# ZrrSkywalker/MonoDETR

Hardware: AMD Instinct MI355X
Metric: training images/sec at B=8 per GPU, KITTI 384x1280 (higher is better)
Workload: dtype bf16; 1 GPU; full MonoDETR training step (ResNet-50 + depth predictor + 3 enc / 3 dec layers, 550 train queries, 4 levels, criterion + AdamW) = BASELINE configs[2] (1 GPU) / configs[3] (DDP); global_batch=8, per_gpu_batch=8, image=3x384x1280, queries=50, precision=bf16, parallelism=dp1, grad_sync=none, prime_steps=12, launch=one hipGraph replay per iteration, cpu_affinity=NUMA node 1 of the GPU

## Files before the change

include/monodetr_amd.h:

```cpp
#ifndef MONODETR_AMD_H
#define MONODETR_AMD_H

#include <stdint.h>

#ifdef __cplusplus
extern "C" {
#endif

#define MDETR_ABI_VERSION 13

#define MDETR_F32 0
#define MDETR_F64 1
#define MDETR_BF16 2

#define MDETR_OK            0
#define MDETR_E_ARG        -1
#define MDETR_E_HIP        -2
#define MDETR_E_ALIGN      -3

int mdetr_abi_version(void);
const char *mdetr_last_error(void);

int mdetr_msda_forward(int dtype,
                       const void *value, const int64_t *spatial_shapes, const int64_t *level_start,
                       const void *loc, const void *attn, void *out,
                       int B, int S, int M, int D, int L, int Lq, int P,
                       int device, void *stream);

int mdetr_msda_backward(int dtype,
                        const void *value, const int64_t *spatial_shapes, const int64_t *level_start,
                        const void *loc, const void *attn, const void *grad_out,
                        void *grad_value, void *grad_loc, void *grad_attn,
                        int B, int S, int M, int D, int L, int Lq, int P,
                        int device, void *stream);

int mdetr_msda_forward_cpu(int dtype,
                           const void *value, const int64_t *spatial_shapes, const int64_t *level_start,
                           const void *loc, const void *attn, void *out,
                           int B, int S, int M, int D, int L, int Lq, int P);
int mdetr_msda_backward_cpu(int dtype,
                            const void *value, const int64_t *spatial_shapes, const int64_t *level_start,
                            const void *loc, const void *attn, const void *grad_out,
                            void *grad_value, void *grad_loc, void *grad_attn,
                            int B, int S, int M, int D, int L, int Lq, int P);

int mdetr_msda_backward_ex(int dtype,
                           const void *value, const int64_t *spatial_shapes, const int64_t *level_start,
                           const void *loc, const void *attn, const void *grad_out,
                           void *grad_value, void *grad_loc, void *grad_attn,
                           int B, int S, int M, int D, int L, int Lq, int P,
                           const int64_t *spatial_shapes_host, const int64_t *level_start_host,
                           void *workspace, int64_t workspace_bytes,
                           int device, void *stream);

int64_t mdetr_msda_backward_workspace_bytes(int dtype, const int64_t *spatial_shapes_host,
                                            const int64_t *level_start_host,
                                            int B, int S, int M, int D, int L, int Lq, int P);

int mdetr_msda_indices(int dtype, const int64_t *spatial_shapes, const void *loc, int32_t *idx,
                       int B, int M, int L, int Lq, int P, int device, void *stream);

int mdetr_msda_variant(int dtype, int M, int D, int L, int P);

int mdetr_attn_forward(int dtype, const void *q, const void *k, const void *v, const uint8_t *key_padding_mask,
                       void *out, float *lse, int B, int H, int Lq, int Lk,
                       int64_t q_bs, int64_t k_bs, int64_t v_bs, int q_rs, int k_rs, int v_rs,
                       float scale, float dropout_p, uint64_t seed, const uint64_t *seed_dev, int device, void *stream);

int mdetr_attn_backward(int dtype, const void *q, const void *k, const void *v, const uint8_t *key_padding_mask,
                        const void *out, const void *d_out, const float *lse, float *dsum,
                        void *dq, void *dk, void *dv, int B, int H, int Lq, int Lk,
                        int64_t q_bs, int64_t k_bs, int64_t v_bs, int q_rs, int k_rs, int v_rs,
                        float scale, float dropout_p, uint64_t seed, const uint64_t *seed_dev, int device, void *stream);

int64_t mdetr_pair_losses_workspace_bytes(int L, int B);
int mdetr_pair_losses_forward(const float *logits, const float *boxes, const float *dims, const float *depths,
                              const float *angles, const int32_t *assign, const int64_t *labels, const float *boxes3d,
                              const float *depth, const float *size3d, const int64_t *heading_bin,
                              const float *heading_res, const uint8_t *valid, const int32_t *num,
                              int L, int B, int Q, int C, int G, int K, float focal_alpha,
                              float num_boxes, const float *num_boxes_dev, float *out, float *comp, void *workspace,
                              int device, void *stream);
int mdetr_pair_losses_backward(const float *logits, const float *boxes, const float *dims, const float *depths,
                               const float *angles, const int32_t *assign, const int64_t *labels, const float *boxes3d,
                               const float *depth, const float *size3d, const int64_t *heading_bin,
                               const float *heading_res, const uint8_t *valid,
                               int L, int B, int Q, int C, int G, int K, float focal_alpha,
                               float num_boxes, const float *num_boxes_dev, const float *grad_out, const float *comp,
                               float *g_logits, float *g_boxes, float *g_dims, float *g_depths, float *g_angles,
                               int device, void *stream);

int mdetr_msda_forward_bf16(const void *value, const int64_t *spatial_shapes, const int64_t *level_start,
                            const float *loc, const float *attn, void *out,
                            int B, int S, int M, int D, int L, int Lq, int P, int device, void *stream);
int mdetr_msda_backward_bf16(const void *value, const int64_t *spatial_shapes, const int64_t *level_start,
                             const float *loc, const float *attn, const void *grad_out,
                             float *grad_value, float *grad_loc, float *grad_attn,
                             int B, int S, int M, int D, int L, int Lq, int P,
                             const int64_t *spatial_shapes_host, const int64_t *level_start_host,
                             void *workspace, int64_t workspace_bytes, int device, void *stream);

int mdetr_msda_prologue_forward(int io_dtype, int ref_dtype, const void *offsets, const void *logits, const void *ref,
                                const int64_t *spatial_shapes, float *sampling_loc, float *attn_weight,
                                int B, int Lq, int M, int L, int P, int R, int64_t ref_sb, int64_t ref_sq, int64_t ref_sl,
                                int device, void *stream);
int mdetr_msda_prologue_backward(int io_dtype, int ref_dtype, const void *offsets, const void *ref, const int64_t *spatial_shapes,
                                 const float *attn_weight, const float *grad_loc, const float *grad_attn,
                                 void *grad_offsets, void *grad_logits, float *grad_ref,
                                 int B, int Lq, int M, int L, int P, int R, int64_t ref_sb, int64_t ref_sq, int64_t ref_sl,
                                 int device, void *stream);
int mdetr_msda_prologue_forward_packed(int io_dtype, int ref_dtype, const void *packed, const void *ref, const int64_t *spatial_shapes,
                                       float *sampling_loc, float *attn_weight, int B, int Lq, int M, int L, int P, int R,
                                       int64_t ref_sb, int64_t ref_sq, int64_t ref_sl, int device, void *stream);
int mdetr_msda_prologue_backward_packed(int io_dtype, int ref_dtype, const void *packed, const void *ref, const int64_t *spatial_shapes,
                                        const float *attn_weight, const float *grad_loc, const float *grad_attn, void *grad_packed,
                                        float *grad_ref, int B, int Lq, int M, int L, int P, int R,
                                        int64_t ref_sb, int64_t ref_sq, int64_t ref_sl, int device, void *stream);

int mdetr_lsa_forward_fused(const float *logits, const float *boxes, const int64_t *labels, const float *boxes3d,
                            const int32_t *num_targets, int32_t *assign, int layers, int images, int groups, int n,
                            int kmax, int num_classes, float w_class, float w_bbox, float w_center, float w_giou,
                            float focal_alpha, int device, void *stream);

int mdetr_ddn_loss_forward(const float *logits, const float *boxes, const float *depth, const uint8_t *valid,
                           int B, int C, int H, int W, int K, int64_t sb, int64_t sc, int64_t sh, int64_t sw,
                           float alpha, float fg_weight, float bg_weight, float depth_min, float depth_max,
                           float *out, void *workspace, int device, void *stream);
int mdetr_ddn_loss_backward(const float *logits, const float *boxes, const float *depth, const uint8_t *valid,
                            int B, int C, int H, int W, int K, int64_t sb, int64_t sc, int64_t sh, int64_t sw,
                            float alpha, float fg_weight, float bg_weight, float depth_min, float depth_max,
                            const float *grad_out, float *grad_logits, int device, void *stream);

int mdetr_adamw_step(int param_dtype, void *param, float *master, const void *grad, float *exp_avg, float *exp_avg_sq,
                     int64_t n, int64_t n_no_decay, float beta1, float beta2, float eps, float weight_decay,
                     float step_size, const float *step_size_dev, int device, void *stream);
int mdetr_adamw_step_counted(int param_dtype, void *param, float *master, const void *grad, float *exp_avg, float *exp_avg_sq,
                             int64_t n, int64_t n_no_decay, float beta1, float beta2, float eps, float weight_decay,
                             const double *step_count_dev, float lr, const double *lr_dev, int device, void *stream);
int mdetr_adamw_step_gathered(int param_dtype, void *param, float *master, const void *const *grad_ptrs, int ntensors,
                              const int *tensor_block_begin, const int64_t *flat_offsets, const int64_t *nbytes, const int *block_tensor,
                              const int64_t *block_start, int chunk_bytes, float *exp_avg, float *exp_avg_sq, int64_t n_no_decay,
                              float beta1, float beta2, float eps, float weight_decay, float step_size, const float *step_size_dev,
                              const double *step_count_dev, float lr, const double *lr_dev, int device, void *stream);

#define MDETR_TGEMM_RELU 1
#define MDETR_TGEMM_NN 2
#define MDETR_TGEMM_BIAS_F32 4
#define MDETR_TGEMM_OUT_F32 8
int mdetr_tgemm(const void *a, const void *w, const void *bias, const void *res, void *y, int64_t T, int N, int K,
                int64_t lda, int64_t ldw, int64_t ldr, int64_t ldy, int flags, float dropout_p, uint64_t seed,
                const void *seed_dev, int device, void *stream);
int mdetr_tgemm_masked(const void *a, const void *w, const void *res, const void *mask, void *y, int64_t T, int N, int K,
                       int64_t lda, int64_t ldw, int64_t ldr, int64_t ldm, int64_t ldy, int device, void *stream);
// ... 33 lines not shown
#define MDETR_KITTI_CONTRAST 16u
#define MDETR_KITTI_SATURATION 32u
#define MDETR_KITTI_HUE 64u
typedef struct MdetrKittiImage {
    int64_t pixel_offset;
    int32_t width, height;
    uint32_t flags;
    uint32_t perm;
    float brightness, contrast, saturation, hue;
    double inv[6];
} MdetrKittiImage;
int mdetr_kitti_preprocess(const uint8_t *pixels, const MdetrKittiImage *images, int n_images, void *out,
                           int out_dtype, int out_h, int out_w, int channels_last, const float *mean, const float *std,
                           int device, void *stream);

int mdetr_rotate_iou_eval(const float *boxes, const float *qboxes, const int64_t *box_start, const int64_t *qbox_start,
                          const int64_t *out_start, int n_frames, int64_t total_pairs, int criterion, float *out,
                          int device, void *stream);
int mdetr_box3d_overlap_eval(const double *boxes, const double *qboxes, const int64_t *box_start, const int64_t *qbox_start,
                             const int64_t *out_start, int n_frames, int64_t total_pairs, int criterion, double *out,
                             int device, void *stream);
int mdetr_kitti_pr_curve(const double *overlaps, const int64_t *ov_start, const double *gt_datas, const double *dt_datas,
                         const int64_t *gt_start, const int64_t *dt_start, const int64_t *ignored_gt,
                         const int64_t *ignored_det, const double *dontcares, const int64_t *dc_start, int n_frames,
                         int metric, double min_overlap, int64_t num_valid_gt, int compute_aos, int max_thresholds,
                         double *pr, double *thresholds, int *n_thresholds);

int mdetr_add_layernorm_forward(int io_dtype, int param_dtype, const void *a, const void *b, const void *gamma, const void *beta, void *y,
                                void *s, float *stats, int64_t rows, int cols, float eps, float dropout_p, uint64_t seed,
                                const uint64_t *seed_dev, int device, void *stream);
int64_t mdetr_add_layernorm_partial_rows(int64_t rows);
int mdetr_add_layernorm_backward(int io_dtype, int param_dtype, const void *dy, const void *s, const void *gamma, const float *stats,
                                 void *da, void *db, float *partial, int64_t rows, int cols, float dropout_p,
                                 uint64_t seed, const uint64_t *seed_dev, int device, void *stream);

int64_t mdetr_column_sum_workspace_bytes(int64_t rows, int cols);
int mdetr_column_sum(int dtype, const void *x, float *out, void *workspace, int64_t workspace_bytes,
                     int64_t rows, int cols, int64_t ld, int device, void *stream);
int mdetr_box_refine(const float *delta, const float *ref, float *out, int64_t rows, int nd, int device, void *stream);
int mdetr_head_tail_forward(const float *delta, const float *init_ref, const float *inter_refs, const float *size3d, const float *depth_reg,
                            const float *depth_map, const float *img_h, const float *focal, float *coord, float *depth_ave,
                            int L, int B, int Q, int nd0, int H, int W, int device, void *stream);
int mdetr_head_tail_backward(const float *init_ref, const float *size3d, const float *depth_reg, const float *img_h, const float *focal,
                             const float *coord, const float *g_coord, const float *g_depth, float *g_delta, float *g_init_ref,
                             float *g_size3d, float *g_depth_reg, float *g_map, int L, int B, int Q, int nd0, int H, int W, int device, void *stream);

typedef struct {
    const float *part;
    void *out;
    int64_t cols;
    int32_t chunks, out_dtype;
} mdetr_chunk_job;
int mdetr_chunk_sums(const mdetr_chunk_job *jobs, int njobs, int device, void *stream);
int mdetr_column_sum_to(int dtype, const void *x, void *out, int out_dtype, void *workspace, int64_t workspace_bytes,
                        int64_t rows, int cols, int64_t ld, int device, void *stream);

int mdetr_conv3x3_forward(const void *x, const void *w, const float *shift, void *y, int B, int H, int W, int C, int N,
                          int relu, int device, void *stream);
int mdetr_conv3x3_plan(int B, int H, int W, int N);
int mdetr_conv3x3_masked(const void *x, const void *w, const float *shift, const void *mask, void *y, int B, int H, int W, int C, int N,
                         int relu, int device, void *stream);

int mdetr_conv_taps(const void *x, const void *w, const float *shift, void *y, const int64_t *dims, int relu, int device, void *stream);

int mdetr_conv_taps_split(const void *x, const void *w, const float *shift, float *partial, int64_t partial_floats, const int64_t *dims,
                          int ksplit, int device, void *stream);

int mdetr_conv_dgrad_s2(const void *dy, const void *wt, void *dx, int B, int OH, int OW, int N, int H, int W, int C, int K, int device, void *stream);

int mdetr_conv_stem(const void *x, const void *w_packed, const float *shift, void *y, int B, int H, int W, int device, void *stream);

int mdetr_conv_wgrad_chunks(int B, int H, int W, int C, int OH, int OW, int N, int K, int SI);
int mdetr_conv_wgrad(const void *x, const void *dy, float *partial, int64_t partial_floats, int B, int H, int W, int C, int OH, int OW, int N,
                     int K, int SI, int device, void *stream);

int mdetr_token_wgrad_chunks(int64_t T, int C, int N);
int mdetr_token_wgrad(const void *x, const void *dy, float *partial, int64_t partial_floats, int64_t T, int C, int N, int with_bias,
                      int device, void *stream);

int mdetr_bias_act_forward(int io_dtype, int bias_dtype, const void *x, const void *bias, const void *skip, void *y,
                           int64_t rows, int cols, int relu, float dropout_p, uint64_t seed, const uint64_t *seed_dev,
                           int device, void *stream);
int mdetr_bias_act_backward(int io_dtype, const void *dy, const void *y, void *dx, int64_t rows, int cols, float scale,
                            int device, void *stream);

int mdetr_fold_weights(int n, const void *const *w, const void *const *scale, void *const *folded, void *const *folded_t,
                       const int *O, const int *C, const int *taps, int device, void *stream);
int mdetr_unfold_grads(int n, const void *const *dfolded, const void *const *scale, void *const *dw,
                       const int *O, const int *C, const int *taps, int device, void *stream);

int mdetr_gather_flat(const void *const *src_ptrs, int ntensors, const int *tensor_block_begin, void *dst, const int64_t *dst_offsets,
                      const int64_t *nbytes, const int *block_tensor, const int64_t *block_start, int chunk_bytes, int device, void *stream);

int mdetr_maxpool3x3s2_bf16(const void *x, void *y, int B, int H, int W, int C, int device, void *stream);
int mdetr_decimate2(int backward, const void *src, void *dst, int B, int H, int W, int64_t pixel_bytes, int device, void *stream);

int64_t mdetr_small_wgrad_workspace_bytes(int64_t rows, int n, int k);
int mdetr_small_wgrad(int io_dtype, const void *dy, const void *x, void *out, int out_dtype, void *workspace, int64_t workspace_bytes,
                      int64_t rows, int n, int k, int64_t ldy, int64_t ldx, int device, void *stream);

int64_t mdetr_group_norm_workspace_bytes(int n, int64_t hw, int c, int groups);
int mdetr_group_norm_forward(int io_dtype, int param_dtype, const void *x, const void *gamma, const void *beta, void *y, float *stats,
                             void *workspace, int64_t workspace_bytes, int n, int64_t hw, int c, int groups, float eps, int relu,
                             int device, void *stream);
int mdetr_group_norm_backward(int io_dtype, int param_dtype, const void *dy, const void *x, const void *gamma, const void *beta,
                              const float *stats, void *dx, void *dparams, void *workspace, int64_t workspace_bytes,
// ... 15 lines not shown
```

monodetr_amd/_capi.py:

```python
import ctypes
import os
import threading

_HERE = os.path.dirname(os.path.abspath(__file__))
LIB_PATH = os.environ.get("MDETR_LIB_PATH") or os.path.join(_HERE, "libmonodetr_amd.so")

MDETR_F32, MDETR_F64, MDETR_BF16 = 0, 1, 2
ABI_VERSION = 13

_c_int, _c_vp = ctypes.c_int, ctypes.c_void_p

SIGNATURES = {
    "mdetr_abi_version": (_c_int, []),
    "mdetr_last_error": (ctypes.c_char_p, []),
    "mdetr_msda_variant": (_c_int, [_c_int] * 5),
    "mdetr_msda_forward": (_c_int, [_c_int] + [_c_vp] * 6 + [_c_int] * 7 + [_c_int, _c_vp]),
    "mdetr_msda_backward": (_c_int, [_c_int] + [_c_vp] * 9 + [_c_int] * 7 + [_c_int, _c_vp]),
    "mdetr_msda_forward_cpu": (_c_int, [_c_int] + [_c_vp] * 6 + [_c_int] * 7),
    "mdetr_msda_backward_cpu": (_c_int, [_c_int] + [_c_vp] * 9 + [_c_int] * 7),
    "mdetr_msda_backward_ex": (_c_int, [_c_int] + [_c_vp] * 9 + [_c_int] * 7 + [_c_vp, _c_vp, _c_vp, ctypes.c_int64] + [_c_int, _c_vp]),
    "mdetr_msda_backward_workspace_bytes": (ctypes.c_int64, [_c_int, _c_vp, _c_vp] + [_c_int] * 7),
    "mdetr_msda_indices": (_c_int, [_c_int] + [_c_vp] * 3 + [_c_int] * 5 + [_c_int, _c_vp]),
    "mdetr_attn_forward": (_c_int, [_c_int] + [_c_vp] * 6 + [_c_int] * 4 + [ctypes.c_int64] * 3 + [_c_int] * 3
                           + [ctypes.c_float, ctypes.c_float, ctypes.c_uint64, _c_vp, _c_int, _c_vp]),
    "mdetr_attn_backward": (_c_int, [_c_int] + [_c_vp] * 11 + [_c_int] * 4 + [ctypes.c_int64] * 3 + [_c_int] * 3
                            + [ctypes.c_float, ctypes.c_float, ctypes.c_uint64, _c_vp, _c_int, _c_vp]),
    "mdetr_lsa_forward": (_c_int, [_c_vp] * 3 + [_c_int] * 5 + [ctypes.c_int64] * 3 + [_c_int, _c_vp]),
    "mdetr_ddn_loss_forward": (_c_int, [_c_vp] * 4 + [_c_int] * 5 + [ctypes.c_int64] * 4 + [ctypes.c_float] * 5 + [_c_vp, _c_vp, _c_int, _c_vp]),
    "mdetr_ddn_loss_backward": (_c_int, [_c_vp] * 4 + [_c_int] * 5 + [ctypes.c_int64] * 4 + [ctypes.c_float] * 5 + [_c_vp, _c_vp, _c_int, _c_vp]),
    "mdetr_pair_losses_workspace_bytes": (ctypes.c_int64, [_c_int, _c_int]),
    "mdetr_pair_losses_forward": (_c_int, [_c_vp] * 14 + [_c_int] * 6 + [ctypes.c_float, ctypes.c_float] + [_c_vp] * 4 + [_c_int, _c_vp]),
    "mdetr_pair_losses_backward": (_c_int, [_c_vp] * 13 + [_c_int] * 6 + [ctypes.c_float, ctypes.c_float] + [_c_vp] * 8 + [_c_int, _c_vp]),
    "mdetr_adamw_step": (_c_int, [_c_int] + [_c_vp] * 5 + [ctypes.c_int64] * 2 + [ctypes.c_float] * 5 + [_c_vp, _c_int, _c_vp]),
    "mdetr_adamw_step_gathered": (_c_int, [_c_int, _c_vp, _c_vp, _c_vp, _c_int] + [_c_vp] * 5 + [_c_int, _c_vp, _c_vp, ctypes.c_int64] + [ctypes.c_float] * 5
                                  + [_c_vp, _c_vp, ctypes.c_float, _c_vp, _c_int, _c_vp]),
    "mdetr_adamw_step_counted": (_c_int, [_c_int] + [_c_vp] * 5 + [ctypes.c_int64] * 2 + [ctypes.c_float] * 4 + [_c_vp, ctypes.c_float, _c_vp, _c_int, _c_vp]),
    "mdetr_tgemm": (_c_int, [_c_vp] * 5 + [ctypes.c_int64, _c_int, _c_int] + [ctypes.c_int64] * 4 + [_c_int, ctypes.c_float, ctypes.c_uint64, _c_vp, _c_int, _c_vp]),
    "mdetr_sgemm_workspace_bytes": (ctypes.c_int64, [_c_int, _c_vp, _c_int]),
    "mdetr_sgemm_grouped": (_c_int, [_c_int, _c_vp, _c_int, _c_vp, ctypes.c_int64, _c_int, _c_vp]),
    "mdetr_tgemm_masked": (_c_int, [_c_vp] * 5 + [ctypes.c_int64, _c_int, _c_int] + [ctypes.c_int64] * 5 + [_c_int, _c_vp]),
    "mdetr_tgemm_f32": (_c_int, [_c_vp] * 5 + [ctypes.c_int64, _c_int, _c_int] + [ctypes.c_int64] * 4 + [_c_int, ctypes.c_float, ctypes.c_uint64, _c_vp, _c_int, _c_vp]),
    "mdetr_tgemm_f32_masked": (_c_int, [_c_vp] * 5 + [ctypes.c_int64, _c_int, _c_int] + [ctypes.c_int64] * 5 + [_c_int, _c_vp]),
    "mdetr_column_sum_workspace_bytes": (ctypes.c_int64, [ctypes.c_int64, _c_int]),
    "mdetr_column_sum": (_c_int, [_c_int, _c_vp, _c_vp, _c_vp, ctypes.c_int64, ctypes.c_int64, _c_int, ctypes.c_int64, _c_int, _c_vp]),
    "mdetr_box_refine": (_c_int, [_c_vp] * 3 + [ctypes.c_int64, _c_int, _c_int, _c_vp]),
    "mdetr_head_tail_forward": (_c_int, [_c_vp] * 10 + [_c_int] * 6 + [_c_int, _c_vp]),
    "mdetr_head_tail_backward": (_c_int, [_c_vp] * 13 + [_c_int] * 6 + [_c_int, _c_vp]),
    "mdetr_chunk_sums": (_c_int, [_c_vp, _c_int, _c_int, _c_vp]),
    "mdetr_column_sum_to": (_c_int, [_c_int, _c_vp, _c_vp, _c_int, _c_vp, ctypes.c_int64, ctypes.c_int64, _c_int, ctypes.c_int64, _c_int, _c_vp]),
    "mdetr_add_layernorm_forward": (_c_int, [_c_int, _c_int] + [_c_vp] * 7 + [ctypes.c_int64, _c_int, ctypes.c_float, ctypes.c_float, ctypes.c_uint64, _c_vp, _c_int, _c_vp]),
    "mdetr_add_layernorm_partial_rows": (ctypes.c_int64, [ctypes.c_int64]),
    "mdetr_add_layernorm_backward": (_c_int, [_c_int, _c_int] + [_c_vp] * 7 + [ctypes.c_int64, _c_int, ctypes.c_float, ctypes.c_uint64, _c_vp, _c_int, _c_vp]),
    "mdetr_conv3x3_forward": (_c_int, [_c_vp] * 4 + [_c_int] * 6 + [_c_int, _c_vp]),
    "mdetr_conv3x3_plan": (_c_int, [_c_int] * 4),
    "mdetr_conv3x3_masked": (_c_int, [_c_vp] * 5 + [_c_int] * 6 + [_c_int, _c_vp]),
    "mdetr_conv_taps": (_c_int, [_c_vp] * 5 + [_c_int, _c_int, _c_vp]),
    "mdetr_conv_taps_split": (_c_int, [_c_vp] * 4 + [ctypes.c_int64, _c_vp, _c_int, _c_int, _c_vp]),
    "mdetr_conv_dgrad_s2": (_c_int, [_c_vp] * 3 + [_c_int] * 8 + [_c_int, _c_vp]),
    "mdetr_conv_stem": (_c_int, [_c_vp] * 4 + [_c_int] * 3 + [_c_int, _c_vp]),
    "mdetr_conv_wgrad_chunks": (_c_int, [_c_int] * 9),
    "mdetr_conv_wgrad": (_c_int, [_c_vp] * 3 + [ctypes.c_int64] + [_c_int] * 9 + [_c_int, _c_vp]),
    "mdetr_token_wgrad_chunks": (_c_int, [ctypes.c_int64, _c_int, _c_int]),
    "mdetr_token_wgrad": (_c_int, [_c_vp, _c_vp, _c_vp, ctypes.c_int64, ctypes.c_int64, _c_int, _c_int, _c_int, _c_int, _c_vp]),
    "mdetr_small_wgrad_workspace_bytes": (ctypes.c_int64, [ctypes.c_int64, _c_int, _c_int]),
    "mdetr_small_wgrad": (_c_int, [_c_int, _c_vp, _c_vp, _c_vp, _c_int, _c_vp, ctypes.c_int64, ctypes.c_int64, _c_int, _c_int, ctypes.c_int64, ctypes.c_int64, _c_int, _c_vp]),
    "mdetr_group_norm_workspace_bytes": (ctypes.c_int64, [_c_int, ctypes.c_int64, _c_int, _c_int]),
    "mdetr_group_norm_forward": (_c_int, [_c_int, _c_int] + [_c_vp] * 6 + [ctypes.c_int64, _c_int, ctypes.c_int64, _c_int, _c_int, ctypes.c_float, _c_int, _c_int, _c_vp]),
    "mdetr_group_norm_backward": (_c_int, [_c_int, _c_int] + [_c_vp] * 8 + [ctypes.c_int64, _c_int, ctypes.c_int64, _c_int, _c_int, _c_int, _c_int, _c_vp]),
    "mdetr_bias_act_forward": (_c_int, [_c_int, _c_int] + [_c_vp] * 4 + [ctypes.c_int64, _c_int, _c_int, ctypes.c_float, ctypes.c_uint64, _c_vp, _c_int, _c_vp]),
    "mdetr_bias_act_backward": (_c_int, [_c_int] + [_c_vp] * 3 + [ctypes.c_int64, _c_int, ctypes.c_float, _c_int, _c_vp]),
    "mdetr_rotate_iou_eval": (_c_int, [_c_vp] * 5 + [_c_int, ctypes.c_int64, _c_int, _c_vp, _c_int, _c_vp]),
    "mdetr_box3d_overlap_eval": (_c_int, [_c_vp] * 5 + [_c_int, ctypes.c_int64, _c_int, _c_vp, _c_int, _c_vp]),
    "mdetr_kitti_pr_curve": (_c_int, [_c_vp] * 10 + [_c_int, _c_int, ctypes.c_double, ctypes.c_int64, _c_int, _c_int, _c_vp, _c_vp, _c_vp]),
    "mdetr_kitti_preprocess": (_c_int, [_c_vp, _c_vp, _c_int, _c_vp, _c_int, _c_int, _c_int, _c_int, _c_vp, _c_vp, _c_int, _c_vp]),
    "mdetr_msda_forward_bf16": (_c_int, [_c_vp] * 6 + [_c_int] * 7 + [_c_int, _c_vp]),
    "mdetr_msda_backward_bf16": (_c_int, [_c_vp] * 9 + [_c_int] * 7 + [_c_vp, _c_vp, _c_vp, ctypes.c_int64, _c_int, _c_vp]),
    "mdetr_msda_prologue_forward": (_c_int, [_c_int, _c_int] + [_c_vp] * 6 + [_c_int] * 6 + [ctypes.c_int64] * 3 + [_c_int, _c_vp]),
    "mdetr_gather_flat": (_c_int, [_c_vp, _c_int] + [_c_vp] * 6 + [_c_int, _c_int, _c_vp]),
    "mdetr_fold_weights": (_c_int, [_c_int] + [_c_vp] * 7 + [_c_int, _c_vp]),
    "mdetr_unfold_grads": (_c_int, [_c_int] + [_c_vp] * 6 + [_c_int, _c_vp]),
    "mdetr_maxpool3x3s2_bf16": (_c_int, [_c_vp, _c_vp, _c_int, _c_int, _c_int, _c_int, _c_int, _c_vp]),
    "mdetr_decimate2": (_c_int, [_c_int, _c_vp, _c_vp, _c_int, _c_int, _c_int, ctypes.c_int64, _c_int, _c_vp]),
    "mdetr_msda_prologue_forward_packed": (_c_int, [_c_int, _c_int] + [_c_vp] * 5 + [_c_int] * 6 + [ctypes.c_int64] * 3 + [_c_int, _c_vp]),
    "mdetr_msda_prologue_backward_packed": (_c_int, [_c_int, _c_int] + [_c_vp] * 8 + [_c_int] * 6 + [ctypes.c_int64] * 3 + [_c_int, _c_vp]),
    "mdetr_msda_prologue_backward": (_c_int, [_c_int, _c_int] + [_c_vp] * 9 + [_c_int] * 6 + [ctypes.c_int64] * 3 + [_c_int, _c_vp]),
    "mdetr_lsa_forward_fused": (_c_int, [_c_vp] * 6 + [_c_int] * 6 + [ctypes.c_float] * 5 + [_c_int, _c_vp]),
    "mdetr_profile_enable": (_c_int, [_c_int]),
    "mdetr_profile_read": (_c_int, [_c_vp, _c_int]),
    "mdetr_profile_read_work": (_c_int, [_c_vp, _c_int]),
}

_lib = None
_lock = threading.Lock()


def lib():
    global _lib
    if _lib is None:
        with _lock:
            if _lib is None:
                if not os.path.exists(LIB_PATH):
                    raise RuntimeError(
                        "monodetr_amd: %s is missing -- the HIP extension is not built. Run "
                        "`python -m monodetr_amd.build` (needs hipcc). There is no CPU/PyTorch fallback." % LIB_PATH)
                handle = ctypes.CDLL(LIB_PATH)
                for name, (res, args) in SIGNATURES.items():
                    fn = getattr(handle, name)
                    fn.restype, fn.argtypes = res, args
                got = handle.mdetr_abi_version()
                if got != ABI_VERSION:
                    raise RuntimeError("monodetr_amd: ABI version mismatch (lib %d, python %d); rebuild" % (got, ABI_VERSION))
                _lib = handle
    return _lib


def check(rc, what):
    if rc != 0:
        msg = lib().mdetr_last_error()
        raise RuntimeError("%s failed (code %d): %s" % (what, rc, msg.decode() if msg else "?"))


def dtype_code(t):
    import torch
    if t.dtype == torch.float32:
        return MDETR_F32
    if t.dtype == torch.float64:
        return MDETR_F64
    raise RuntimeError('"ms_deform_attn" not implemented for \'%s\'' % str(t.dtype).replace("torch.", ""))

# ... 20 lines not shown
```

monodetr_amd/add_ln_ext.py:

```python
import os

import torch
import torch.nn.functional as F

from . import _capi
from .attn_ext import _next_seed

_backend = None
ENABLED = os.environ.get("MDETR_FUSED_LN") == "1"


_seed_counter = None


def _host_seed():
    global _seed_counter
    if _seed_counter is None:
        _seed_counter = int(torch.randint(0, 2 ** 62, (1,), dtype=torch.int64))
    _seed_counter = (_seed_counter + 0x9E3779B97F4A7C15) & 0x7FFFFFFFFFFFFFFF
    return _seed_counter


def _lib():
    return _backend if _backend is not None else _capi.lib()
# ... 14 lines not shown
    cuda = t.is_cuda
    return (t.device.index if cuda else -1), (torch.cuda.current_stream(t.device).cuda_stream if cuda else None)


def _column_sum_f32(x, out_dtype=torch.float32):
    if x.is_cuda and _backend is None:
        from .colsum_ext import column_sum
        return column_sum(x, out_dtype if out_dtype in (torch.float32, torch.bfloat16) else torch.float32)
    return x.sum(0).to(out_dtype)


class _AddLayerNorm(torch.autograd.Function):
    @staticmethod
    def forward(ctx, a, b, gamma, beta, eps, p, seed, seed_dev):
        shape = a.shape
        C = shape[-1]
        a2, b2 = _rows(a, C), _rows(b, C)
        rows = a2.shape[0]
        if gamma.dtype == beta.dtype and gamma.dtype in (torch.float32, torch.bfloat16):
            gp, bp = gamma.contiguous(), beta.contiguous()
        else:
            gp, bp = gamma.float().contiguous(), beta.float().contiguous()
        pcode = _capi.MDETR_BF16 if gp.dtype == torch.bfloat16 else _capi.MDETR_F32
        y, s = torch.empty_like(a2), torch.empty_like(a2)
        stats = torch.empty((rows, 2), dtype=torch.float32, device=a.device)
        io = _capi.MDETR_BF16 if a.dtype == torch.bfloat16 else _capi.MDETR_F32
        dev, stream = _dev(a2)
        rc = _lib().mdetr_add_layernorm_forward(io, pcode, a2.data_ptr(), b2.data_ptr(), gp.data_ptr(), bp.data_ptr(), y.data_ptr(), s.data_ptr(),
                                                stats.data_ptr(), rows, C, float(eps), float(p), int(seed),
                                                seed_dev.data_ptr() if seed_dev is not None else None, dev, stream)
        if rc != 0:
            _capi.check(rc, "mdetr_add_layernorm_forward")
        ctx.save_for_backward(s, gp, stats)
        ctx.seed_dev = seed_dev
        ctx.meta = (io, pcode, rows, C, float(p), int(seed), shape, gamma.dtype, beta.dtype)
        return y.view(shape)

    @staticmethod
    @torch.autograd.function.once_differentiable
    def backward(ctx, dy):
        s, gp, stats = ctx.saved_tensors
        io, pcode, rows, C, p, seed, shape, g_dtype, b_dtype = ctx.meta
        dy2 = _rows(dy, C)
        da, db = torch.empty_like(s), torch.empty_like(s)
        lib = _lib()
        nb = lib.mdetr_add_layernorm_partial_rows(rows)
        partial = torch.empty((nb, 2 * C), dtype=torch.float32, device=s.device)
        dev, stream = _dev(s)
        rc = lib.mdetr_add_layernorm_backward(io, pcode, dy2.data_ptr(), s.data_ptr(), gp.data_ptr(), stats.data_ptr(), da.data_ptr(), db.data_ptr(),
                                              partial.data_ptr(), rows, C, p, seed,
                                              ctx.seed_dev.data_ptr() if ctx.seed_dev is not None else None, dev, stream)
        if rc != 0:
            _capi.check(rc, "mdetr_add_layernorm_backward")
        sums = _column_sum_f32(partial, g_dtype if g_dtype == b_dtype else torch.float32)
        return da.view(shape), db.view(shape), sums[:C].to(g_dtype), sums[C:].to(b_dtype), None, None, None, None


def fused_add_layernorm(a, b, gamma, beta, eps=1e-5, dropout_p=0.0, seed=None):
    seed_dev = None
    if dropout_p > 0.0 and seed is None:
        if a.is_cuda and torch.cuda.is_current_stream_capturing():
            from .attn_ext import site_seed
            seed, seed_dev = site_seed(a.device)
        else:
            seed = _host_seed()
    return _AddLayerNorm.apply(a, b, gamma, beta, eps, dropout_p, seed or 0, seed_dev)


def residual_layernorm(a, b, norm, dropout):
    if ENABLED and supported(a, b, norm):
        p = dropout.p if (dropout is not None and dropout.training) else 0.0
        return fused_add_layernorm(a, b, norm.weight, norm.bias, norm.eps, p)
    return norm(a + (dropout(b) if dropout is not None else b))
```

monodetr_amd/chunk_sums.py:

```python
import ctypes
import os
import threading

import torch

from . import _capi

ENABLED = os.environ.get("MDETR_CHUNK_SUMS") == "1"
POISON = False
IMMEDIATE = False
_backend = None
_lock = threading.RLock()
_depth = 0
_pending = []


class _Job(ctypes.Structure):
    _fields_ = [("part", ctypes.c_void_p), ("out", ctypes.c_void_p), ("cols", ctypes.c_int64), ("chunks", ctypes.c_int32), ("out_dtype", ctypes.c_int32)]


def _lib():
    return _backend if _backend is not None else _capi.lib()


def supported(part, out_dtype):
    return ((part.is_cuda or _backend is not None) and part.dim() == 2 and part.dtype == torch.float32 and part.is_contiguous()
            and part.shape[1] % 4 == 0 and part.shape[0] > 0 and part.data_ptr() % 16 == 0 and out_dtype in (torch.float32, torch.bfloat16))


def _launch(jobs):
    arr = (_Job * len(jobs))()
    for q, (part, out) in zip(arr, jobs):
        q.part, q.out, q.cols, q.chunks = part.data_ptr(), out.data_ptr(), part.shape[1], part.shape[0]
        q.out_dtype = _capi.MDETR_BF16 if out.dtype == torch.bfloat16 else _capi.MDETR_F32
    dev = jobs[0][0].device
    rc = _lib().mdetr_chunk_sums(ctypes.cast(arr, ctypes.c_void_p), len(jobs), dev.index if dev.type == "cuda" else -1,
                                 torch.cuda.current_stream(dev).cuda_stream if dev.type == "cuda" else None)
    if rc != 0:
        msg = _lib().mdetr_last_error()
        raise RuntimeError("mdetr_chunk_sums failed (code %d): %s" % (rc, msg.decode() if msg else "?"))


def chunk_sum(part, out_dtype=torch.float32, defer=True):
    if not supported(part, out_dtype):
        raise RuntimeError("chunk_sum: needs contiguous fp32 partials [chunks, cols], cols a multiple of 4, 16-byte aligned")
    out = torch.empty(part.shape[1], dtype=out_dtype, device=part.device)
    with _lock:
        if defer and ENABLED and _depth > 0 and not IMMEDIATE:
            if POISON:
                out.fill_(float("nan"))
            _pending.append((part, out))
            return out
    _launch([(part, out)])
    return out


def deferring():
    return ENABLED and _depth > 0


def flush():
    with _lock:
        jobs = list(_pending)
        del _pending[:]
    if jobs:
        by_dev = {}
        for j in jobs:
            by_dev.setdefault(j[0].device, []).append(j)
        for group in by_dev.values():
            _launch(group)


def reader_inside_backward(module=None, params=None, held="refuse"):
    if module is not None:
        from torch.nn.parallel import DistributedDataParallel
        if isinstance(module, DistributedDataParallel):
            return "DistributedDataParallel copies each gradient into its bucket during the backward pass"
        if params is None:
            params = module.parameters()
    for p in params or ():
        if not p.requires_grad:
            continue
        if p._backward_hooks or p._post_accumulate_grad_hooks:
            return "a parameter carries a gradient hook"
        if held == "refuse" and p.grad is not None:
            return "a parameter still has a .grad: the new gradient is added to it during the backward pass"
    return None


class deferred:

    def __init__(self, module=None, params=None, held="refuse"):
        self.reason = None
        self._held = ()
        if (module is not None or params is not None) and ENABLED and not IMMEDIATE:
            params = list(module.parameters() if params is None else params)
            self.reason = reader_inside_backward(module, params, held)
            if self.reason is None and held == "verify":
# ... 23 lines not shown
```

monodetr_amd/csrc/capi.hip:

```cpp
#include <hip/hip_runtime.h>
#include <stdarg.h>
#include <stdio.h>

#include <atomic>
#include <map>
#include <mutex>
#include <utility>
#include <vector>

#include "../../include/monodetr_amd.h"
#include "attn.h"
#include "adamw.h"
#include "add_ln.h"
#include "bias_act.h"
#include "colsum.h"
#include "group_norm.h"
#include "small_wgrad.h"
#include "decimate.h"
#include "wfold.h"
#include "conv3x3.h"
#include "conv_stem.h"
#include "conv_taps.h"
#include "conv_wgrad.h"
#include "ddn_loss.h"
// ... 627 lines not shown

int mdetr_box_refine(const float *delta, const float *ref, float *out, int64_t rows, int nd, int device, void *stream)
{
    if (rows < 0 || (nd != 2 && nd != 6)) return fail(MDETR_E_ARG, "mdetr_box_refine: bad sizes rows=%lld nd=%d (2 or 6)", static_cast<long long>(rows), nd);
    if (rows == 0) return MDETR_OK;
    if (!delta || !ref || !out) return fail(MDETR_E_ARG, "mdetr_box_refine: null pointer");
    DeviceScope dev(device);
    if (dev.err != hipSuccess) return fail(MDETR_E_HIP, "mdetr_box_refine: set device %d: %s", device, hipGetErrorString(dev.err));
    const hipError_t e = mdetr::box_refine_launch(delta, ref, out, rows, nd, static_cast<hipStream_t>(stream));
    if (e != hipSuccess) return fail(MDETR_E_HIP, "mdetr_box_refine: launch failed: %s", hipGetErrorString(e));
    return MDETR_OK;
}

static int head_tail_dims(const char *who, int L, int B, int Q, int nd0, int H, int W, mdetr::HeadTailDims *d)
{
    if (L <= 0 || B <= 0 || Q <= 0 || H <= 0 || W <= 0 || (nd0 != 2 && nd0 != 6) || static_cast<int64_t>(L) * B * Q * 6 >= (1ll << 31))
        return fail(MDETR_E_ARG, "%s: bad sizes L=%d B=%d Q=%d nd0=%d H=%d W=%d", who, L, B, Q, nd0, H, W);
    d->L = L; d->B = B; d->Q = Q; d->nd0 = nd0; d->H = H; d->W = W;
    return MDETR_OK;
}

int mdetr_head_tail_forward(const float *delta, const float *init_ref, const float *inter_refs, const float *size3d, const float *depth_reg,
                            const float *depth_map, const float *img_h, const float *focal, float *coord, float *depth_ave,
                            int L, int B, int Q, int nd0, int H, int W, int device, void *stream)
{
    mdetr::HeadTailDims d;
    if (int rc = head_tail_dims("mdetr_head_tail_forward", L, B, Q, nd0, H, W, &d)) return rc;
    if (!delta || !init_ref || (L > 1 && !inter_refs) || !size3d || !depth_reg || !depth_map || !img_h || !focal || !coord || !depth_ave)
        return fail(MDETR_E_ARG, "mdetr_head_tail_forward: null pointer");
    DeviceScope dev(device);
    if (dev.err != hipSuccess) return fail(MDETR_E_HIP, "mdetr_head_tail_forward: set device %d: %s", device, hipGetErrorString(dev.err));
    const hipError_t e = mdetr::head_tail_forward_launch(d, delta, init_ref, inter_refs, size3d, depth_reg, depth_map, img_h, focal, coord, depth_ave,
                                                         static_cast<hipStream_t>(stream));
    if (e != hipSuccess) return fail(MDETR_E_HIP, "mdetr_head_tail_forward: launch failed: %s", hipGetErrorString(e));
    return MDETR_OK;
}

int mdetr_head_tail_backward(const float *init_ref, const float *size3d, const float *depth_reg, const float *img_h, const float *focal,
                             const float *coord, const float *g_coord, const float *g_depth, float *g_delta, float *g_init_ref,
                             float *g_size3d, float *g_depth_reg, float *g_map, int L, int B, int Q, int nd0, int H, int W, int device, void *stream)
{
    mdetr::HeadTailDims d;
    if (int rc = head_tail_dims("mdetr_head_tail_backward", L, B, Q, nd0, H, W, &d)) return rc;
    if (!init_ref || !size3d || !depth_reg || !img_h || !focal || !coord || !g_delta || !g_init_ref || !g_size3d || !g_depth_reg)
        return fail(MDETR_E_ARG, "mdetr_head_tail_backward: null pointer");
    DeviceScope dev(device);
    if (dev.err != hipSuccess) return fail(MDETR_E_HIP, "mdetr_head_tail_backward: set device %d: %s", device, hipGetErrorString(dev.err));
    const hipError_t e = mdetr::head_tail_backward_launch(d, init_ref, size3d, depth_reg, img_h, focal, coord, g_coord, g_depth, g_delta, g_init_ref,
                                                          g_size3d, g_depth_reg, g_map, static_cast<hipStream_t>(stream));
    if (e != hipSuccess) return fail(MDETR_E_HIP, "mdetr_head_tail_backward: launch failed: %s", hipGetErrorString(e));
    return MDETR_OK;
}

int mdetr_chunk_sums(const mdetr_chunk_job *jobs, int njobs, int device, void *stream)
{
    if (njobs == 0) return MDETR_OK;
    const char *why = mdetr::chunk_sums_check(jobs, njobs);
    if (why) return fail(MDETR_E_ARG, "mdetr_chunk_sums: %s (%d jobs)", why, njobs);
    DeviceScope dev(device);
    if (dev.err != hipSuccess) return fail(MDETR_E_HIP, "mdetr_chunk_sums: set device %d: %s", device, hipGetErrorString(dev.err));
    double kb = 0.0;
    for (int i = 0; i < njobs; ++i) kb += (static_cast<double>(jobs[i].chunks) * jobs[i].cols * 4.0 + jobs[i].cols * (jobs[i].out_dtype == 2 ? 2.0 : 4.0)) / 1e3;
    mdetr::ProfileScope prof(12, njobs, static_cast<hipStream_t>(stream), 0.0, kb);
    const hipError_t e = mdetr::chunk_sums_launch(jobs, njobs, static_cast<hipStream_t>(stream));
    if (e != hipSuccess) return fail(MDETR_E_HIP, "mdetr_chunk_sums: launch failed: %s", hipGetErrorString(e));
    return MDETR_OK;
}

static int conv3x3_any(const char *who, const void *x, const void *w, const float *shift, const void *mask, void *y, int B, int H, int W, int C, int N,
                       int relu, int device, void *stream)
{
    if (B < 0 || H < 0 || W < 0 || C <= 0 || N <= 0) return fail(MDETR_E_ARG, "%s: bad sizes B=%d H=%d W=%d C=%d N=%d", who, B, H, W, C, N);
    if (B == 0 || H == 0 || W == 0) return MDETR_OK;
    if (!x || !w || !y) return fail(MDETR_E_ARG, "%s: null pointer", who);
    if (!mdetr::conv3x3_supported(B, H, W, C, N, x, w, y) || (reinterpret_cast<uintptr_t>(mask) & 7) != 0)
        return fail(MDETR_E_ARG, "%s: needs C %% 64 == 0, N %% 32 == 0, 16-byte aligned x / w, 8-byte aligned y / mask (C=%d N=%d)", who, C, N);
    DeviceScope dev(device);
    if (dev.err != hipSuccess) return fail(MDETR_E_HIP, "%s: set device %d: %s", who, device, hipGetErrorString(dev.err));
    const hipError_t e = mdetr::conv3x3_launch(x, w, shift, y, B, H, W, C, N, (relu & 1) != 0, static_cast<hipStream_t>(stream), (relu & 2) != 0, mask);
    if (e != hipSuccess) return fail(MDETR_E_HIP, "%s: launch failed: %s", who, hipGetErrorString(e));
    return MDETR_OK;
}

int mdetr_conv3x3_plan(int B, int H, int W, int N)
{
    if (B <= 0 || H <= 0 || W <= 0 || N <= 0) return fail(MDETR_E_ARG, "mdetr_conv3x3_plan: bad sizes");
    return mdetr::conv3x3_plan(B, H, W, N);
}

int mdetr_conv3x3_forward(const void *x, const void *w, const float *shift, void *y, int B, int H, int W, int C, int N,
                          int relu, int device, void *stream)
{
    return conv3x3_any("mdetr_conv3x3_forward", x, w, shift, nullptr, y, B, H, W, C, N, relu, device, stream);
}

int mdetr_conv3x3_masked(const void *x, const void *w, const float *shift, const void *mask, void *y, int B, int H, int W, int C, int N,
                         int relu, int device, void *stream)
{
    if (!mask) return fail(MDETR_E_ARG, "mdetr_conv3x3_masked: null mask");
    return conv3x3_any("mdetr_conv3x3_masked", x, w, shift, mask, y, B, H, W, C, N, relu, device, stream);
}

int mdetr_conv_taps(const void *x, const void *w, const float *shift, void *y, const int64_t *dims, int relu, int device, void *stream)
{
    if (!dims) return fail(MDETR_E_ARG, "mdetr_conv_taps: null dims");
    mdetr::ConvTapsDims d;
    d.B = static_cast<int>(dims[0]); d.H = static_cast<int>(dims[1]); d.W = static_cast<int>(dims[2]); d.C = static_cast<int>(dims[3]);
    d.OH = static_cast<int>(dims[4]); d.OW = static_cast<int>(dims[5]); d.N = static_cast<int>(dims[6]);
    d.SI = static_cast<int>(dims[7]); d.TR = static_cast<int>(dims[8]); d.TS = static_cast<int>(dims[9]);
    d.PT = static_cast<int>(dims[10]); d.PL = static_cast<int>(dims[11]);
    d.ta0 = static_cast<int>(dims[12]); d.ta_step = static_cast<int>(dims[13]); d.te0 = static_cast<int>(dims[14]); d.te_step = static_cast<int>(dims[15]);
    d.y_off = dims[16]; d.y_sb = dims[17]; d.y_sr = dims[18]; d.y_sc = dims[19];
    d.w_sn = dims[20]; d.w_sa = dims[21]; d.w_se = dims[22];
    for (int i = 0; i < 12; ++i)
        if (dims[i] < 0 || dims[i] > (1ll << 30)) return fail(MDETR_E_ARG, "mdetr_conv_taps: bad size dims[%d] = %lld", i, static_cast<long long>(dims[i]));
    if (d.B == 0 || d.OH == 0 || d.OW == 0) return MDETR_OK;
    if (!x || !w || !y) return fail(MDETR_E_ARG, "mdetr_conv_taps: null pointer");
    if (!mdetr::conv_taps_supported(d, x, w, y))
        return fail(MDETR_E_ARG, "mdetr_conv_taps: unsupported problem (taps %dx%d stride %d, C=%d %% 64, N=%d %% 32, 16-byte aligned x / w, strides in whole "
// ... 454 lines not shown
    if (dev.err != hipSuccess) return fail(MDETR_E_HIP, "mdetr_kitti_preprocess: set device %d: %s", device, hipGetErrorString(dev.err));
    mdetr::KittiNorm norm;
    for (int c = 0; c < 3; ++c) { norm.mean[c] = mean[c]; norm.stdv[c] = std[c]; }
    const hipError_t e = mdetr::kitti_prep_launch(pixels, images, n_images, out, out_dtype, out_h, out_w, norm, channels_last != 0,
                                                  static_cast<hipStream_t>(stream));
    if (e != hipSuccess) return fail(MDETR_E_HIP, "mdetr_kitti_preprocess: launch failed: %s", hipGetErrorString(e));
    return MDETR_OK;
}

int mdetr_msda_forward_bf16(const void *value, const int64_t *spatial_shapes, const int64_t *level_start,
                            const float *loc, const float *attn, void *out,
                            int B, int S, int M, int D, int L, int Lq, int P, int device, void *stream)
{
    if (int rc = check_common("mdetr_msda_forward_bf16", MDETR_F32, B, S, M, D, L, Lq, P)) return rc;
    if (D != 32 || L != 4 || P != 4) return fail(MDETR_E_ARG, "mdetr_msda_forward_bf16: D = 32, L = P = 4 only (D=%d L=%d P=%d)", D, L, P);
    if (B == 0 || Lq == 0) return MDETR_OK;
    if (!value || !spatial_shapes || !level_start || !loc || !attn || !out)
        return fail(MDETR_E_ARG, "mdetr_msda_forward_bf16: null pointer");
    if (!aligned16(value) || !aligned16(loc) || !aligned16(attn) || !aligned16(out))
        return fail(MDETR_E_ALIGN, "mdetr_msda_forward_bf16: value/loc/attn/out must be 16-byte aligned");
    DeviceScope dev(device);
    if (dev.err != hipSuccess) return fail(MDETR_E_HIP, "mdetr_msda_forward_bf16: set device %d: %s", device, hipGetErrorString(dev.err));
    const hipError_t e = mdetr::msda_forward_bf16_launch(value, spatial_shapes, level_start, loc, attn, out,
                                                         B, S, M, D, L, Lq, P, static_cast<hipStream_t>(stream));
    if (e != hipSuccess) return fail(MDETR_E_HIP, "mdetr_msda_forward_bf16: launch failed: %s", hipGetErrorString(e));
    return MDETR_OK;
}

int mdetr_msda_backward_bf16(const void *value, const int64_t *spatial_shapes, const int64_t *level_start,
                             const float *loc, const float *attn, const void *grad_out,
                             float *grad_value, float *grad_loc, float *grad_attn,
                             int B, int S, int M, int D, int L, int Lq, int P,
                             const int64_t *spatial_shapes_host, const int64_t *level_start_host,
                             void *workspace, int64_t workspace_bytes, int device, void *stream)
{
    if (int rc = check_common("mdetr_msda_backward_bf16", MDETR_F32, B, S, M, D, L, Lq, P)) return rc;
    if (D != 32 || L != 4 || P != 4) return fail(MDETR_E_ARG, "mdetr_msda_backward_bf16: D = 32, L = P = 4 only (D=%d L=%d P=%d)", D, L, P);
    if (!grad_value || !grad_loc || !grad_attn) return fail(MDETR_E_ARG, "mdetr_msda_backward_bf16: null output pointer");
    if (B > 0 && Lq > 0 && (!value || !spatial_shapes || !level_start || !loc || !attn || !grad_out))
        return fail(MDETR_E_ARG, "mdetr_msda_backward_bf16: null pointer");
    if (!aligned16(value) || !aligned16(loc) || !aligned16(attn) || !aligned16(grad_out) || !aligned16(grad_value) ||
        !aligned16(grad_loc) || !aligned16(grad_attn))
        return fail(MDETR_E_ALIGN, "mdetr_msda_backward_bf16: all tensors must be 16-byte aligned");
    DeviceScope dev(device);
    if (dev.err != hipSuccess) return fail(MDETR_E_HIP, "mdetr_msda_backward_bf16: set device %d: %s", device, hipGetErrorString(dev.err));
    const hipError_t e = mdetr::msda_backward_bf16_launch(value, spatial_shapes, level_start, loc, attn, grad_out, grad_value,
                                                          grad_loc, grad_attn, B, S, M, D, L, Lq, P, spatial_shapes_host,
                                                          level_start_host, workspace, workspace_bytes,
                                                          static_cast<hipStream_t>(stream));
    if (e != hipSuccess) return fail(MDETR_E_HIP, "mdetr_msda_backward_bf16: launch failed: %s", hipGetErrorString(e));
    return MDETR_OK;
}

static int prologue_args(const char *who, int io_dtype, int B, int Lq, int M, int L, int P, int R)
{
    if (io_dtype != MDETR_F32 && io_dtype != MDETR_BF16) return fail(MDETR_E_ARG, "%s: dtype must be f32 or bf16", who);
    if (B < 0 || Lq < 0 || M <= 0 || L <= 0 || P <= 0 || L * P > mdetr::kPrologueMaxLP || (R != 2 && R != 6))
        return fail(MDETR_E_ARG, "%s: bad shape B=%d Lq=%d M=%d L=%d P=%d R=%d", who, B, Lq, M, L, P, R);
    return MDETR_OK;
}

int mdetr_msda_prologue_forward(int io_dtype, int ref_dtype, const void *offsets, const void *logits, const void *ref,
                                const int64_t *spatial_shapes, float *sampling_loc, float *attn_weight,
                                int B, int Lq, int M, int L, int P, int R, int64_t ref_sb, int64_t ref_sq, int64_t ref_sl,
                                int device, void *stream)
{
    if (int rc = prologue_args("mdetr_msda_prologue_forward", io_dtype, B, Lq, M, L, P, R)) return rc;
    if (ref_dtype != MDETR_F32 && ref_dtype != MDETR_BF16) return fail(MDETR_E_ARG, "mdetr_msda_prologue_forward: ref_dtype %d", ref_dtype);
    if (B == 0 || Lq == 0) return MDETR_OK;
    if (!offsets || !logits || !ref || !spatial_shapes || !sampling_loc || !attn_weight)
        return fail(MDETR_E_ARG, "mdetr_msda_prologue_forward: null pointer");
    DeviceScope dev(device);
    if (dev.err != hipSuccess) return fail(MDETR_E_HIP, "mdetr_msda_prologue_forward: set device %d: %s", device, hipGetErrorString(dev.err));
    const mdetr::PrologueDims d{B, Lq, M, L, P, R, ref_sb, ref_sq, ref_sl};
    const hipError_t e = mdetr::msda_prologue_forward_launch(io_dtype, ref_dtype, d, offsets, logits, ref, spatial_shapes, sampling_loc,
                                                             attn_weight, static_cast<hipStream_t>(stream));
    if (e != hipSuccess) return fail(MDETR_E_HIP, "mdetr_msda_prologue_forward: launch failed: %s", hipGetErrorString(e));
    return MDETR_OK;
}

int mdetr_msda_prologue_backward(int io_dtype, int ref_dtype, const void *offsets, const void *ref, const int64_t *spatial_shapes,
                                 const float *attn_weight, const float *grad_loc, const float *grad_attn,
                                 void *grad_offsets, void *grad_logits, float *grad_ref,
                                 int B, int Lq, int M, int L, int P, int R, int64_t ref_sb, int64_t ref_sq, int64_t ref_sl,
                                 int device, void *stream)
{
    if (int rc = prologue_args("mdetr_msda_prologue_backward", io_dtype, B, Lq, M, L, P, R)) return rc;
    if (ref_dtype != MDETR_F32 && ref_dtype != MDETR_BF16) return fail(MDETR_E_ARG, "mdetr_msda_prologue_backward: ref_dtype %d", ref_dtype);
    if (B == 0 || Lq == 0) return MDETR_OK;
    if (!offsets || !ref || !spatial_shapes || !attn_weight || !grad_loc || !grad_attn || !grad_offsets || !grad_logits)
        return fail(MDETR_E_ARG, "mdetr_msda_prologue_backward: null pointer");
    DeviceScope dev(device);
    if (dev.err != hipSuccess) return fail(MDETR_E_HIP, "mdetr_msda_prologue_backward: set device %d: %s", device, hipGetErrorString(dev.err));
    const mdetr::PrologueDims d{B, Lq, M, L, P, R, ref_sb, ref_sq, ref_sl};
    hipError_t e = hipSuccess;
    if (grad_ref) e = mdetr::zero_fill_launch(grad_ref, static_cast<int64_t>(B) * Lq * L * R * 4, static_cast<hipStream_t>(stream));
    if (e == hipSuccess)
        e = mdetr::msda_prologue_backward_launch(io_dtype, ref_dtype, d, offsets, ref, spatial_shapes, attn_weight, grad_loc, grad_attn,
                                                 grad_offsets, grad_logits, grad_ref, static_cast<hipStream_t>(stream));
    if (e != hipSuccess) return fail(MDETR_E_HIP, "mdetr_msda_prologue_backward: launch failed: %s", hipGetErrorString(e));
    return MDETR_OK;
}

int mdetr_msda_prologue_forward_packed(int io_dtype, int ref_dtype, const void *packed, const void *ref, const int64_t *spatial_shapes,
                                       float *sampling_loc, float *attn_weight, int B, int Lq, int M, int L, int P, int R,
                                       int64_t ref_sb, int64_t ref_sq, int64_t ref_sl, int device, void *stream)
// ... 80 lines not shown
```

monodetr_amd/csrc/colsum.h:

```cpp
#pragma once
#include <hip/hip_runtime.h>
#include <stdint.h>

#include "../../include/monodetr_amd.h"

namespace mdetr {

bool colsum_supported(int dtype, int cols, int64_t ld, const void *x);
int64_t colsum_workspace_bytes(int64_t rows, int cols);
hipError_t colsum_launch(int dtype, const void *x, void *out, void *workspace, int64_t rows, int cols, int64_t ld,
                         hipStream_t st, int out_dtype = 0);

const char *chunk_sums_check(const mdetr_chunk_job *jobs, int njobs);
hipError_t chunk_sums_launch(const mdetr_chunk_job *jobs, int njobs, hipStream_t st);

}
```

monodetr_amd/csrc/colsum.hip:

```cpp
#include <hip/hip_runtime.h>
#include <hip/hip_bf16.h>
#include <stdint.h>

#include "colsum.h"

namespace mdetr {
namespace {

constexpr int kThreads = 256;
constexpr int kRowsPerBlock = 256;

template <typename T> struct Vec16;
template <> struct Vec16<float> {
    static constexpr int N = 4;
    static __device__ __forceinline__ void add(float *acc, const uint4 &v)
    {
        acc[0] += __uint_as_float(v.x); acc[1] += __uint_as_float(v.y);
        acc[2] += __uint_as_float(v.z); acc[3] += __uint_as_float(v.w);
    }
};
template <> struct Vec16<__hip_bfloat16> {
    static constexpr int N = 8;
    static __device__ __forceinline__ void add(float *acc, const uint4 &v)
    {
// ... 22 lines not shown
    for (int i = 0; i < VEC; ++i) acc[i] = 0.f;
    if (cv < cvs) {
        const T *p = x + static_cast<int64_t>(cv) * VEC;
        int64_t r = r0 + lane_r;
        for (; r + 3 * RL < r1; r += 4 * RL) {
            const uint4 a = *reinterpret_cast<const uint4 *>(p + r * ld);
            const uint4 b = *reinterpret_cast<const uint4 *>(p + (r + RL) * ld);
            const uint4 c = *reinterpret_cast<const uint4 *>(p + (r + 2 * RL) * ld);
            const uint4 d = *reinterpret_cast<const uint4 *>(p + (r + 3 * RL) * ld);
            Vec16<T>::add(acc, a); Vec16<T>::add(acc, b); Vec16<T>::add(acc, c); Vec16<T>::add(acc, d);
        }
        for (; r < r1; r += RL) Vec16<T>::add(acc, *reinterpret_cast<const uint4 *>(p + r * ld));
    }
#pragma unroll
    for (int i = 0; i < VEC; ++i) red[(lane_r * CT + lane_c) * VEC + i] = acc[i];
    __syncthreads();
    for (int t = threadIdx.x; t < CT * VEC; t += kThreads) {
        float s = 0.f;
        for (int l = 0; l < RL; ++l) s += red[l * CT * VEC + t];
        const int col = blockIdx.y * CT * VEC + t;
        if (col < cols) partial[static_cast<int64_t>(blockIdx.x) * cols + col] = static_cast<PT>(s);
    }
}

template <typename OT>
__global__ __launch_bounds__(kThreads)
void colsum_final_kernel(const float *__restrict__ partial, OT *__restrict__ out, int nblk, int cols)
{
    __shared__ float red[16][17];
    const int c = threadIdx.x & 15, sl = threadIdx.x >> 4;
    const int col = blockIdx.x * 16 + c;
    float s0 = 0.f, s1 = 0.f, s2 = 0.f, s3 = 0.f;
    if (col < cols) {
        int b = sl;
        for (; b + 48 < nblk; b += 64) {
            s0 += partial[static_cast<int64_t>(b) * cols + col];
            s1 += partial[static_cast<int64_t>(b + 16) * cols + col];
            s2 += partial[static_cast<int64_t>(b + 32) * cols + col];
            s3 += partial[static_cast<int64_t>(b + 48) * cols + col];
        }
        for (; b < nblk; b += 16) s0 += partial[static_cast<int64_t>(b) * cols + col];
    }
    red[sl][c] = (s0 + s1) + (s2 + s3);
    __syncthreads();
    if (sl == 0 && col < cols) {
        float s = 0.f;
#pragma unroll
        for (int l = 0; l < 16; ++l) s += red[l][c];
        out[col] = static_cast<OT>(s);
    }
}

constexpr int kChunkJobs = 48, kChunkCols = 4 * kThreads;
struct ChunkJob {
    const float *part;
    void *out;
    int64_t cols;
    int chunks, out_bf16;
    int block0, pad_;
};
struct ChunkArgs {
    ChunkJob j[kChunkJobs];
    int njobs, pad_;
};

__global__ __launch_bounds__(kThreads)
void chunk_sums_kernel(const ChunkArgs a)
{
    __shared__ __attribute__((aligned(16))) ChunkArgs la;
    {
        const unsigned *src = reinterpret_cast<const unsigned *>(&a);
        unsigned *dst = reinterpret_cast<unsigned *>(&la);
        for (unsigned i = threadIdx.x; i < sizeof(ChunkArgs) / 4; i += kThreads) dst[i] = src[i];
        __syncthreads();
    }
    int ji = 0;
    for (int i = 1; i < la.njobs; ++i)
        if (static_cast<int>(blockIdx.x) >= la.j[i].block0) ji = i;
    const ChunkJob &J = la.j[ji];
    const int64_t cols = J.cols, c = static_cast<int64_t>(static_cast<int>(blockIdx.x) - J.block0) * kChunkCols + 4 * threadIdx.x;
    if (c >= cols) return;
    const float *p = J.part + c;
    const int chunks = J.chunks;
    float4 s = make_float4(0.f, 0.f, 0.f, 0.f);
    int k = 0;
    for (; k + 3 < chunks; k += 4) {
        const float4 v0 = *reinterpret_cast<const float4 *>(p + static_cast<int64_t>(k) * cols);
        const float4 v1 = *reinterpret_cast<const float4 *>(p + static_cast<int64_t>(k + 1) * cols);
        const float4 v2 = *reinterpret_cast<const float4 *>(p + static_cast<int64_t>(k + 2) * cols);
        const float4 v3 = *reinterpret_cast<const float4 *>(p + static_cast<int64_t>(k + 3) * cols);
        s.x = (((s.x + v0.x) + v1.x) + v2.x) + v3.x; s.y = (((s.y + v0.y) + v1.y) + v2.y) + v3.y;
        s.z = (((s.z + v0.z) + v1.z) + v2.z) + v3.z; s.w = (((s.w + v0.w) + v1.w) + v2.w) + v3.w;
    }
    for (; k < chunks; ++k) {
        const float4 v = *reinterpret_cast<const float4 *>(p + static_cast<int64_t>(k) * cols);
        s.x += v.x; s.y += v.y; s.z += v.z; s.w += v.w;
    }
    if (J.out_bf16) {
        __hip_bfloat16 *o = static_cast<__hip_bfloat16 *>(J.out) + c;
        o[0] = __float2bfloat16(s.x); o[1] = __float2bfloat16(s.y); o[2] = __float2bfloat16(s.z); o[3] = __float2bfloat16(s.w);
    } else {
        *reinterpret_cast<float4 *>(static_cast<float *>(J.out) + c) = s;
    }
}

}

const char *chunk_sums_check(const mdetr_chunk_job *jobs, int njobs)
{
    if (!jobs || njobs <= 0) return "no jobs";
    for (int i = 0; i < njobs; ++i) {
        const mdetr_chunk_job &q = jobs[i];
        if (!q.part || !q.out || q.cols <= 0 || q.chunks <= 0) return "null pointer or empty job";
        if (q.cols % 4 != 0 || (reinterpret_cast<uintptr_t>(q.part) & 15) != 0) return "cols must be a multiple of 4 and the partials 16-byte aligned";
        if (q.out_dtype != 0 && q.out_dtype != 2) return "out_dtype must be MDETR_F32 or MDETR_BF16";
        if ((reinterpret_cast<uintptr_t>(q.out) & (q.out_dtype == 2 ? 7 : 15)) != 0) return "result not aligned (16 bytes fp32, 8 bytes bf16)";
        if ((q.cols + kChunkCols - 1) / kChunkCols > (1 << 24)) return "job too wide";
    }
    return nullptr;
}

hipError_t chunk_sums_launch(const mdetr_chunk_job *jobs, int njobs, hipStream_t st)
{
    for (int first = 0; first < njobs; first += kChunkJobs) {
        ChunkArgs a;
        const int n = njobs - first < kChunkJobs ? njobs - first : kChunkJobs;
        int blocks = 0;
        for (int i = 0; i < n; ++i) {
            const mdetr_chunk_job &q = jobs[first + i];
            ChunkJob &J = a.j[i];
            J.part = q.part; J.out = q.out; J.cols = q.cols; J.chunks = q.chunks; J.out_bf16 = q.out_dtype == 2; J.block0 = blocks; J.pad_ = 0;
            blocks += static_cast<int>((q.cols + kChunkCols - 1) / kChunkCols);
        }
        a.njobs = n; a.pad_ = 0;
        hipLaunchKernelGGL(chunk_sums_kernel, dim3(blocks), dim3(kThreads), 0, st, a);
        const hipError_t e = hipGetLastError();
        if (e != hipSuccess) return e;
    }
    return hipSuccess;
}

int64_t colsum_workspace_bytes(int64_t rows, int cols)
{
    const int64_t nblk = (rows + kRowsPerBlock - 1) / kRowsPerBlock;
    return nblk * cols * static_cast<int64_t>(sizeof(float));
}

bool colsum_supported(int dtype, int cols, int64_t ld, const void *x)
{
    const int vec = dtype == 2 ? 8 : 4, esz = dtype == 2 ? 2 : 4;
    return (dtype == 0 || dtype == 2) && cols > 0 && cols % vec == 0 && (ld * esz) % 16 == 0 &&
           (reinterpret_cast<uintptr_t>(x) & 15) == 0;
}

hipError_t colsum_launch(int dtype, const void *x, void *out, void *workspace, int64_t rows, int cols, int64_t ld,
                         hipStream_t st, int out_dtype)
{
    if (cols == 0) return hipSuccess;
    const int64_t nblk = (rows + kRowsPerBlock - 1) / kRowsPerBlock;
    float *partial = nblk == 1 ? static_cast<float *>(out) : static_cast<float *>(workspace);
    if (nblk > 0) {
        const int vec = dtype == 2 ? 8 : 4;
        const int cvs = cols / vec;
        int CT = 1;
        while (CT * 2 <= cvs && CT * 2 <= kThreads) CT *= 2;
        while (CT > 8 && nblk * ((cvs + CT - 1) / CT) < 512 && kThreads / (CT / 2) <= (rows < kRowsPerBlock ? rows : kRowsPerBlock)) CT /= 2;
        const dim3 grid(static_cast<unsigned>(nblk), static_cast<unsigned>((cvs + CT - 1) / CT));
        if (nblk == 1 && out_dtype == 2) {
            __hip_bfloat16 *o = static_cast<__hip_bfloat16 *>(out);
            if (dtype == 2)
                hipLaunchKernelGGL((colsum_partial_kernel<__hip_bfloat16, __hip_bfloat16>), grid, dim3(kThreads), 0, st,
                                   static_cast<const __hip_bfloat16 *>(x), o, rows, cols, ld, CT);
            else
                hipLaunchKernelGGL((colsum_partial_kernel<float, __hip_bfloat16>), grid, dim3(kThreads), 0, st,
                                   static_cast<const float *>(x), o, rows, cols, ld, CT);
        } else if (dtype == 2) {
            hipLaunchKernelGGL((colsum_partial_kernel<__hip_bfloat16, float>), grid, dim3(kThreads), 0, st,
                               static_cast<const __hip_bfloat16 *>(x), partial, rows, cols, ld, CT);
        } else {
            hipLaunchKernelGGL((colsum_partial_kernel<float, float>), grid, dim3(kThreads), 0, st,
                               static_cast<const float *>(x), partial, rows, cols, ld, CT);
        }
    }
    if (nblk == 1) return hipGetLastError();
    if (out_dtype == 2)
// ... 10 lines not shown
```

monodetr_amd/csrc/msda.h:

```cpp
#pragma once
#include <hip/hip_runtime.h>
#include <hip/hip_bf16.h>
#include <stdint.h>

namespace mdetr {

template <typename E> struct Elem;
template <> struct Elem<float> {
    static constexpr int kBytes = 4;
    typedef float4 Raw;
    static __device__ __forceinline__ Raw loadr(const char *p) { return *reinterpret_cast<const float4 *>(p); }
    static __device__ __forceinline__ float4 widen(const Raw &r) { return r; }
    static __device__ __forceinline__ float load1(const float *p) { return *p; }
    static __device__ __forceinline__ float4 load4(const char *p) { return *reinterpret_cast<const float4 *>(p); }
    static __device__ __forceinline__ void store4(char *p, const float4 &v) { *reinterpret_cast<float4 *>(p) = v; }
};
template <> struct Elem<__hip_bfloat16> {
    static constexpr int kBytes = 2;
    typedef uint2 Raw;
    static __device__ __forceinline__ Raw loadr(const char *p) { return *reinterpret_cast<const uint2 *>(p); }
    static __device__ __forceinline__ float4 widen(const Raw &u)
    {
        return make_float4(__uint_as_float(u.x << 16), __uint_as_float(u.x & 0xFFFF0000u),
                           __uint_as_float(u.y << 16), __uint_as_float(u.y & 0xFFFF0000u));
    }
    static __device__ __forceinline__ float load1(const __hip_bfloat16 *p) { return __bfloat162float(*p); }
    static __device__ __forceinline__ float4 load4(const char *p)
    {
        const uint2 u = *reinterpret_cast<const uint2 *>(p);
        return make_float4(__uint_as_float(u.x << 16), __uint_as_float(u.x & 0xFFFF0000u),
                           __uint_as_float(u.y << 16), __uint_as_float(u.y & 0xFFFF0000u));
    }
    static __device__ __forceinline__ void store4(char *p, const float4 &v)
    {
        __hip_bfloat16 h[4] = {__float2bfloat16(v.x), __float2bfloat16(v.y), __float2bfloat16(v.z), __float2bfloat16(v.w)};
        *reinterpret_cast<uint2 *>(p) = *reinterpret_cast<const uint2 *>(h);
    }
};

bool msda_fast_path(int dtype, int D, int L, int P);

hipError_t msda_forward_launch(int dtype, const void *value, const int64_t *shapes, const int64_t *lstart,
                               const void *loc, const void *attn, void *out,
                               int B, int S, int M, int D, int L, int Lq, int P, hipStream_t st);

hipError_t msda_backward_launch(int dtype, const void *value, const int64_t *shapes, const int64_t *lstart,
                                const void *loc, const void *attn, const void *grad_out,
                                void *grad_value, void *grad_loc, void *grad_attn,
                                int B, int S, int M, int D, int L, int Lq, int P, hipStream_t st);

hipError_t msda_backward_launch_ex(int dtype, const void *value, const int64_t *shapes, const int64_t *lstart,
                                   const void *loc, const void *attn, const void *grad_out,
                                   void *grad_value, void *grad_loc, void *grad_attn,
                                   int B, int S, int M, int D, int L, int Lq, int P,
                                   const int64_t *shapes_host, const int64_t *lstart_host,
                                   void *workspace, int64_t workspace_bytes, hipStream_t st);

hipError_t msda_forward_bf16_launch(const void *value, const int64_t *shapes, const int64_t *lstart,
                                    const float *loc, const float *attn, void *out,
                                    int B, int S, int M, int D, int L, int Lq, int P, hipStream_t st);
hipError_t msda_backward_bf16_launch(const void *value, const int64_t *shapes, const int64_t *lstart,
                                     const float *loc, const float *attn, const void *grad_out,
                                     float *grad_value, float *grad_loc, float *grad_attn,
                                     int B, int S, int M, int D, int L, int Lq, int P,
                                     const int64_t *shapes_host, const int64_t *lstart_host,
                                     void *workspace, int64_t workspace_bytes, hipStream_t st);

int64_t msda_tiled_workspace_bytes(const int64_t *shapes_h, const int64_t *start_h, int B, int S, int M, int D, int L, int Lq, int P);

hipError_t msda_tiled_grad_value_launch(const int64_t *shapes_h, const int64_t *start_h,
                                        const float *loc, const float *attn, const void *grad_out, float *grad_value,
                                        void *workspace, int64_t workspace_bytes,
                                        int B, int S, int M, int D, int L, int Lq, int P, bool absmax_ready, hipStream_t st,
                                        int grad_out_dtype = 0 );

int64_t msda_fused_workspace_bytes(const int64_t *shapes_h, const int64_t *start_h, int B, int S, int M, int D, int L, int Lq, int P);
hipError_t msda_backward_fused_launch(const int64_t *shapes_h, const int64_t *start_h, const void *value, const float *loc,
                                      const float *attn, const void *grad_out, float *grad_value, float *grad_loc, float *grad_attn,
                                      void *workspace, int64_t workspace_bytes, int B, int S, int M, int D, int L, int Lq, int P,
                                      int elem_dtype, hipStream_t st);

void msda_forward_cpu(int dtype, const void *value, const int64_t *shapes, const int64_t *lstart, const void *loc,
                      const void *attn, void *out, int B, int S, int M, int D, int L, int Lq, int P);
void msda_backward_cpu(int dtype, const void *value, const int64_t *shapes, const int64_t *lstart, const void *loc,
                       const void *attn, const void *grad_out, void *grad_value, void *grad_loc, void *grad_attn,
                       int B, int S, int M, int D, int L, int Lq, int P);

hipError_t msda_indices_launch(int dtype, const int64_t *shapes, const void *loc, int32_t *idx,
                               int B, int M, int L, int Lq, int P, hipStream_t st);

hipError_t zero_fill_launch(void *p, int64_t bytes, hipStream_t st);

void profile_begin(int kind, int Lq, hipStream_t st);
void profile_end(hipStream_t st);
void profile_work(double mflop, double kbytes);
struct ProfileScope {
    hipStream_t s;
    ProfileScope(int kind, int64_t key, hipStream_t st) : s(st) { profile_begin(kind, static_cast<int>(key > 0x7fffffff ? 0x7fffffff : key), st); }
    ProfileScope(int kind, int64_t key, hipStream_t st, double mflop, double kbytes) : s(st)
    {
        profile_begin(kind, static_cast<int>(key > 0x7fffffff ? 0x7fffffff : key), st);
        profile_work(mflop, kbytes);
    }
    ~ProfileScope() { profile_end(s); }
};
inline int64_t conv_mflop(int64_t out_pixels, int64_t macs_per_pixel) { return (2 * out_pixels * macs_per_pixel + 500000) / 1000000; }

}
```

monodetr_amd/csrc/msda.hip:

```cpp
#include <hip/hip_runtime.h>
#include <stdint.h>
#include <stdlib.h>

#include <mdetr_wave.h>

#include "msda.h"
#include "mdetr_tune.h"

namespace mdetr {
namespace {

template <typename T>
__device__ __forceinline__ T pix_coord(T loc, int size)
{
#pragma clang fp contract(off)
    const T prod = loc * static_cast<T>(size);
    return prod - static_cast<T>(0.5);
}

template <typename T>
struct Foot {
    int h_low, w_low;
    T lh, lw, hh, hw;
    bool ok1, ok2, ok3, ok4;
// ... 749 lines not shown
    struct Scope { hipStream_t s; Scope(int Lq_, hipStream_t s_) : s(s_) { profile_begin(0, Lq_, s_); } ~Scope() { profile_end(s); } } scope(Lq, st);
    const int npairs = Lq * M, iters = rounds_per_block(B, npairs);
    const int chunks = (npairs + 32 * iters - 1) / (32 * iters);
    hipLaunchKernelGGL((msda_fwd_rec<4, 4, __hip_bfloat16, __hip_bfloat16>), dim3(static_cast<unsigned>(B) * chunks), dim3(kWaves * 64), 0, st,
                       static_cast<const __hip_bfloat16 *>(value), shapes, lstart, loc, attn,
                       static_cast<__hip_bfloat16 *>(out), B, S, M, npairs, iters);
    return hipGetLastError();
}

hipError_t msda_backward_bf16_launch(const void *value, const int64_t *shapes, const int64_t *lstart,
                                     const float *loc, const float *attn, const void *grad_out,
                                     float *grad_value, float *grad_loc, float *grad_attn,
                                     int B, int S, int M, int D, int L, int Lq, int P,
                                     const int64_t *shapes_host, const int64_t *lstart_host,
                                     void *workspace, int64_t workspace_bytes, hipStream_t st)
{
    if (D != 32 || L != 4 || P != 4) return hipErrorNotSupported;
    const int64_t nv = static_cast<int64_t>(B) * S * M * D;
    hipError_t err;
    const int bwd_env = [] { char tb[16]; const char *ev = tune_str("msda_bwd", tb, sizeof(tb)); return !ev || !*ev || ev[0] == 'f' ? 0 : (ev[0] == 't' ? 1 : 2); }();
    if (bwd_env == 0 && static_cast<int64_t>(B) * Lq * M && shapes_host && lstart_host && workspace) {
        err = msda_backward_fused_launch(shapes_host, lstart_host, value, loc, attn, grad_out, grad_value, grad_loc, grad_attn,
                                         workspace, workspace_bytes, B, S, M, D, L, Lq, P, 2, st);
        if (err != hipErrorNotSupported) return err;
    }
    if (nv && (err = zero_fill_launch(grad_value, nv * 4, st)) != hipSuccess) return err;
    if (static_cast<int64_t>(B) * Lq * M == 0) return hipSuccess;
    const bool try_tiled = shapes_host && lstart_host && workspace && bwd_env != 2 &&
                           msda_tiled_workspace_bytes(shapes_host, lstart_host, B, S, M, D, L, Lq, P) > 0 &&
                           msda_tiled_workspace_bytes(shapes_host, lstart_host, B, S, M, D, L, Lq, P) <= workspace_bytes;
    unsigned *absmax2 = try_tiled ? static_cast<unsigned *>(workspace) : nullptr;
    if (try_tiled && (err = zero_fill_launch(absmax2, 8, st)) != hipSuccess) return err;
    const int npairs = Lq * M, iters = rounds_per_block(B, npairs);
    const int chunks = (npairs + 32 * iters - 1) / (32 * iters);
    const dim3 grid(static_cast<unsigned>(B) * chunks), block(kWaves * 64);
    const size_t lds = sizeof(float) * kWaves * slab_floats(L * P);
    auto a = [&](auto kern) {
        hipLaunchKernelGGL(kern, grid, block, lds, st, static_cast<const __hip_bfloat16 *>(value), shapes, lstart, loc, attn,
                           static_cast<const __hip_bfloat16 *>(grad_out), grad_value, grad_loc, grad_attn,
                           B, S, M, L, P, npairs, iters, absmax2);
    };
    profile_begin(1, Lq, st);
    if (try_tiled) a(msda_bwd_d32<4, 4, 2, __hip_bfloat16, __hip_bfloat16>);
    else a(msda_bwd_d32<4, 4, 1, __hip_bfloat16, __hip_bfloat16>);
    profile_end(st);
    if (try_tiled) {
        err = msda_tiled_grad_value_launch(shapes_host, lstart_host, loc, attn, grad_out, grad_value, workspace, workspace_bytes,
                                           B, S, M, D, L, Lq, P, true, st, 2);
        if (err != hipSuccess) return err;
    }
    return hipGetLastError();
}

hipError_t msda_backward_launch(int dtype, const void *value, const int64_t *shapes, const int64_t *lstart,
                                const void *loc, const void *attn, const void *grad_out,
                                void *grad_value, void *grad_loc, void *grad_attn,
                                int B, int S, int M, int D, int L, int Lq, int P, hipStream_t st)
{
    return msda_backward_launch_ex(dtype, value, shapes, lstart, loc, attn, grad_out, grad_value, grad_loc, grad_attn,
                                   B, S, M, D, L, Lq, P, nullptr, nullptr, nullptr, 0, st);
}

hipError_t msda_indices_launch(int dtype, const int64_t *shapes, const void *loc, int32_t *idx,
                               int B, int M, int L, int Lq, int P, hipStream_t st)
{
    const int64_t n = static_cast<int64_t>(B) * Lq * M * L * P;
    if (n == 0) return hipSuccess;
    if (dtype == 0)
        hipLaunchKernelGGL(msda_indices_kernel<float>, dim3(grid_for(n, 256)), dim3(256), 0, st, shapes,
                           static_cast<const float *>(loc), idx, L, P, n);
    else
        hipLaunchKernelGGL(msda_indices_kernel<double>, dim3(grid_for(n, 256)), dim3(256), 0, st, shapes,
                           static_cast<const double *>(loc), idx, L, P, n);
    return hipGetLastError();
}

}
```

monodetr_amd/csrc/msda_fused.hip:

```cpp
#include <hip/hip_runtime.h>
#include <stdint.h>
#include <stdlib.h>
#include <string.h>

#include <type_traits>

#include <mdetr_wave.h>

#include "msda.h"
#include "mdetr_tune.h"

namespace mdetr {
namespace {

constexpr int kMaxLevels = 4;
constexpr int kCH = 32;
constexpr int kRecDw = 12;
constexpr int kCellU64 = kCH / 2;
constexpr int kCellStride = kCellU64 + 1;
constexpr int kTrash = 8;
constexpr int kMaxCells = 1024;
constexpr unsigned long long kCookie = 0x6d64657472667573ull;

constexpr int kMaxPre = 1024;
constexpr int kHdrBytes = 256 + kMaxPre * 2 * 4;
struct Header {
    unsigned npre, pad0;
    unsigned far;
    unsigned pad;
    unsigned long long cookie;
    unsigned long long far_elems;
};

struct FusedPlan {
    int B, S, M, L, P, Lq;
    int H[kMaxLevels], W[kMaxLevels], start[kMaxLevels];
    int mode[kMaxLevels];
    int owner;
    int TH[kMaxLevels], TW[kMaxLevels], nty[kMaxLevels], ntx[kMaxLevels], R[kMaxLevels];
    int nchunk[kMaxLevels];
    int blk0[kMaxLevels], nblk[kMaxLevels], bstride[kMaxLevels], nblocks;
    long long scr0[kMaxLevels];
    long long scr_per_bm;
    int max_cells;
    int max_tab;
    int npre;
    int small;
};

__host__ __device__ inline int ceil_div_ll(long long a, long long b)
{
    return static_cast<int>(a >= 0 ? (a + b - 1) / b : -((-a) / b));
}

__host__ __device__ inline int row_pad(int tw) { return tw % 16 == 0 ? 1 : 0; }

__host__ __device__ inline int centre_cell(int y, int n_l, int n_q)
{
    return static_cast<int>((static_cast<unsigned>(2 * y + 1) * static_cast<unsigned>(n_l)) / (2u * static_cast<unsigned>(n_q)));
}

__host__ __device__ inline int first_at_or_after(int t, int n_l, int n_q)
{
    const int y = ceil_div_ll(2LL * t * n_q - n_l, 2LL * n_l);
    return y < 0 ? 0 : (y > n_q ? n_q : y);
}

__host__ __device__ inline int first_at_or_after_small(int t, int n_l, int n_q)
{
    const int a = 2 * t * n_q - n_l, b = 2 * n_l;
    const int y = a >= 0 ? static_cast<int>((static_cast<unsigned>(a) + static_cast<unsigned>(b) - 1u) / static_cast<unsigned>(b))
                         : -static_cast<int>(static_cast<unsigned>(-a) / static_cast<unsigned>(b));
    return y < 0 ? 0 : (y > n_q ? n_q : y);
}

__device__ __forceinline__ float pix_coord_f(float loc, int size)
{
#pragma clang fp contract(off)
    const float prod = loc * static_cast<float>(size);
    return prod - 0.5f;
}

__device__ __forceinline__ float sum8f(float v)
{
    v += __builtin_bit_cast(float, __builtin_amdgcn_update_dpp(0, __builtin_bit_cast(int, v), 0xB1, 0xF, 0xF, true));
    v += __builtin_bit_cast(float, __builtin_amdgcn_update_dpp(0, __builtin_bit_cast(int, v), 0x4E, 0xF, 0xF, true));
    v += __builtin_bit_cast(float, __builtin_amdgcn_update_dpp(0, __builtin_bit_cast(int, v), 0x141, 0xF, 0xF, true));
    return v;
}

__device__ __forceinline__ float sum4f(float v)
{
    v += __builtin_bit_cast(float, __builtin_amdgcn_update_dpp(0, __builtin_bit_cast(int, v), 0xB1, 0xF, 0xF, true));
    v += __builtin_bit_cast(float, __builtin_amdgcn_update_dpp(0, __builtin_bit_cast(int, v), 0x4E, 0xF, 0xF, true));
    return v;
}
__device__ __forceinline__ float sum2f(float v)
{
    v += __builtin_bit_cast(float, __builtin_amdgcn_update_dpp(0, __builtin_bit_cast(int, v), 0xB1, 0xF, 0xF, true));
    return v;
}
// ... 603 lines not shown
                typename RG::T rg[NG];
                const int h0 = 64 - nh;
#pragma unroll
                for (int t = 0; t < NG; ++t) {
                    const int r = h0 + min(i0 + SPG * t + j, nh - 1);
                    rg[t] = RG::load(gbase + (pair0u + wrec[r * kRecDw] * static_cast<unsigned>(M)) * static_cast<unsigned>(kCH * Elem<GT>::kBytes));
                }
#pragma unroll
                for (int t = 0; t < NG; ++t) {
                    if (i0 + SPG * t + j < nh) {
                        const unsigned *rr = wrec + (h0 + i0 + SPG * t + j) * kRecDw;
                        const uint4 r0 = *reinterpret_cast<const uint4 *>(rr);
                        const uint4 r1 = *reinterpret_cast<const uint4 *>(rr + 4);
                        const float wt[4] = {__builtin_bit_cast(float, r1.x), __builtin_bit_cast(float, r1.y),
                                             __builtin_bit_cast(float, r1.z), __builtin_bit_cast(float, r1.w)};
                        const float as = __builtin_bit_cast(float, rr[8]) * scale;
                        float ag[CPL];
                        RG::widen(rg[t], ag);
#pragma unroll
                        for (int i = 0; i < CPL; ++i) ag[i] *= as;
                        accumulate<CPL>(win, r0.z, r0.w, wt, ag, k, magic);
                    }
                }
            };
            constexpr int HG = LPS == 2 ? 2 : 4;
            for (int i0 = 0; i0 < nh; i0 += HG * SPG) {
                const int ng = min(HG, (nh - i0 + SPG - 1) / SPG);
                if (ng == 1) halo_batch(std::integral_constant<int, 1>(), i0);
                else if (HG == 2 || ng == 2) halo_batch(std::integral_constant<int, 2>(), i0);
                else if constexpr (HG >= 4) {
                    if (ng == 3) halo_batch(std::integral_constant<int, 3>(), i0);
                    else halo_batch(std::integral_constant<int, 4>(), i0);
                }
            }
            wave_sync();
            base = next_base;
        }
        __syncthreads();

        if (OWNER) {
            unsigned mc = 0u;
            for (int i = threadIdx.x; i < w.ncell; i += THREADS) mc = max(mc, cnt[i]);
            for (int o = 32; o > 0; o >>= 1) mc = max(mc, __shfl_xor(mc, o));
            if (lane == 0) atomicMax(blk, mc);
            __syncthreads();
            const unsigned maxcnt0 = blk[0];
            __syncthreads();
            if (finite && maxcnt0 >= (512u << shift) && shift < 12) continue;
        }
        {
            const unsigned long long cbits = static_cast<unsigned long long>(__builtin_bit_cast(unsigned, magic)) * 0x100000001ull;
            const float inv = finite ? ldexpf(1.0f, -(22 - shift - e)) : 0.f;
            float *dst1 = scratch + (static_cast<int64_t>(b) * M + m) * pl.scr_per_bm + pl.scr0[l] + static_cast<int64_t>(w.slot) * w.ncell * kCH;
            float *dst0 = grad_value + ((static_cast<int64_t>(b) * pl.S + pl.start[l]) * M + m) * kCH;
            unsigned mc = 0u;
            for (int i = threadIdx.x; i < w.ncell * kCellU64; i += THREADS) {
                const int cell = i / kCellU64, pr = i % kCellU64;
                const unsigned n = cnt[cell];
                mc = max(mc, n);
                const unsigned long long s = win[cell * kCellStride + pr] - static_cast<unsigned long long>(n) * cbits;
                const int lo = static_cast<int>(static_cast<unsigned>(s));
                const int hi = static_cast<int>((static_cast<long long>(s) - static_cast<long long>(lo)) >> 32);
                const float2 out = make_float2(static_cast<float>(lo) * inv, static_cast<float>(hi) * inv);
                if (OWNER) {
                    const int yy = w.cy0 + cell / w.tstride, xx = w.cx0 + cell % w.tstride;
                    if (n != 0u && yy >= 0 && yy < H && xx >= 0 && xx < W) {
                        float *dst = dst0 + static_cast<int64_t>(yy * W + xx) * (M * kCH) + 2 * pr;
                        unsafeAtomicAdd(dst, out.x);
                        unsafeAtomicAdd(dst + 1, out.y);
                    }
                } else if (w.mode == 1) {
                    *reinterpret_cast<float2 *>(dst1 + static_cast<int64_t>(cell) * kCH + 2 * pr) = out;
                } else {
                    const int wxx = cell % w.tstride;
                    const int yy = w.cy0 + cell / w.tstride, xx = w.cx0 + wxx;
                    if (yy < H && xx < W && wxx < pl.TW[l])
                        *reinterpret_cast<float2 *>(dst0 + static_cast<int64_t>(yy * W + xx) * (M * kCH) + 2 * pr) = out;
                }
            }
            if (OWNER) break;
            for (int o = 32; o > 0; o >>= 1) mc = max(mc, __shfl_xor(mc, o));
            if (lane == 0) atomicMax(blk + 2 + (shift & 1), mc);
            __syncthreads();
            const unsigned maxcnt = blk[2 + (shift & 1)];
            if (!(finite && maxcnt >= (512u << shift) && shift < 12)) {
                break;
            }
        }
    }
}

__device__ __forceinline__ void finalize_row(const FusedPlan &pl, const float *__restrict__ scratch, float *__restrict__ far,
                                             float *__restrict__ grad_value, int l, int b, int pix, int m, int c4, bool use_far)
{
    const bool chunks = pl.mode[l] == 1;
    const int64_t row = (static_cast<int64_t>(b) * pl.S + pix) * pl.M + m;
    float4 acc = make_float4(0.f, 0.f, 0.f, 0.f);
    if (chunks) {
        const int ncell = pl.H[l] * pl.W[l];
        const float *base = scratch + (static_cast<int64_t>(b) * pl.M + m) * pl.scr_per_bm + pl.scr0[l] +
                            static_cast<int64_t>(pix - pl.start[l]) * kCH + c4;
        const int64_t cs = static_cast<int64_t>(ncell) * kCH;
        const int nch = pl.nchunk[l];
        constexpr int kFlight = 12;
        for (int t0 = 0; t0 < nch; t0 += kFlight) {
            float4 v[kFlight];
#pragma unroll
            for (int u = 0; u < kFlight; ++u)
                if (t0 + u < nch) v[u] = *reinterpret_cast<const float4 *>(base + (t0 + u) * cs);
#pragma unroll
            for (int u = 0; u < kFlight; ++u)
                if (t0 + u < nch) { acc.x += v[u].x; acc.y += v[u].y; acc.z += v[u].z; acc.w += v[u].w; }
        }
    } else {
        acc = *reinterpret_cast<const float4 *>(grad_value + row * kCH + c4);
    }
    if (use_far) {
        float4 *f = reinterpret_cast<float4 *>(far + row * kCH + c4);
        const float4 v = *f;
        acc.x += v.x; acc.y += v.y; acc.z += v.z; acc.w += v.w;
        *f = make_float4(0.f, 0.f, 0.f, 0.f);
    }
    *reinterpret_cast<float4 *>(grad_value + row * kCH + c4) = acc;
}

__global__ __launch_bounds__(256)
void msda_finalize_kernel(const FusedPlan pl, const float *__restrict__ scratch, float *__restrict__ far,
                          float *__restrict__ grad_value, Header *__restrict__ hdr)
{
    const int64_t gid = blockIdx.x * static_cast<int64_t>(blockDim.x) + threadIdx.x;
    const int64_t stride = static_cast<int64_t>(gridDim.x) * blockDim.x;
    if (gid == 0) {
        hdr->cookie = kCookie;
        hdr->far_elems = static_cast<unsigned long long>(pl.B) * pl.S * pl.M * kCH;
    }
    const bool use_far = hdr->far != 0u;
    if (use_far) {
        const int64_t n = static_cast<int64_t>(pl.B) * pl.S * pl.M * 8;
        const bool narrow = n < (1LL << 34);
        for (int64_t i = gid; i < n; i += stride) {
            const int64_t row = i >> 3;
            int m, pix, b;
            if (narrow) {
                const unsigned r = static_cast<unsigned>(row), bp = r / static_cast<unsigned>(pl.M);
                m = static_cast<int>(r - bp * static_cast<unsigned>(pl.M));
                b = static_cast<int>(bp / static_cast<unsigned>(pl.S));
                pix = static_cast<int>(bp - static_cast<unsigned>(b) * static_cast<unsigned>(pl.S));
            } else {
                m = static_cast<int>(row % pl.M);
                const int64_t bp = row / pl.M;
                pix = static_cast<int>(bp % pl.S); b = static_cast<int>(bp / pl.S);
            }
            int l = 0;
            while (l + 1 < pl.L && pix >= pl.start[l + 1]) ++l;
            finalize_row(pl, scratch, far, grad_value, l, b, pix, m, static_cast<int>(i & 7) * 4, true);
        }
        return;
    }
    int64_t cum[kMaxLevels + 1];
    cum[0] = 0;
#pragma unroll
    for (int l = 0; l < kMaxLevels; ++l)
        cum[l + 1] = cum[l] + ((l < pl.L && pl.mode[l] == 1) ? static_cast<int64_t>(pl.B) * pl.H[l] * pl.W[l] * pl.M * 8 : 0);
    const bool narrow = cum[kMaxLevels] < (1LL << 34);
    for (int64_t i = gid; i < cum[kMaxLevels]; i += stride) {
        int l = 0;
#pragma unroll
        for (int t = 1; t < kMaxLevels; ++t) l += i >= cum[t] ? 1 : 0;
        const int hw = pl.H[l] * pl.W[l];
        const int64_t row = (i - cum[l]) >> 3;
        int cell, b, m;
        if (narrow) {
            const unsigned r = static_cast<unsigned>(row), bm = r / static_cast<unsigned>(hw);
            cell = static_cast<int>(r - bm * static_cast<unsigned>(hw));
            b = static_cast<int>(bm / static_cast<unsigned>(pl.M));
            m = static_cast<int>(bm - static_cast<unsigned>(b) * static_cast<unsigned>(pl.M));
// ... 71 lines not shown
            pl.nblk[l] = pl.nty[l] * pl.ntx[l];
            cells = TH * (TW + row_pad(TW));
            if (self) {
                int tab = 0;
                for (int lq = 0; lq < L; ++lq)
                    tab += ((TH + 2 * reach) * pl.H[lq] + H - 1) / H + ((TW + 2 * reach) * pl.W[lq] + W - 1) / W + 4;
                pl.max_tab = tab > pl.max_tab ? tab : pl.max_tab;
                if (static_cast<long long>(Lq) * P >= (1 << 22)) return false;
            }
        }
        if (cells > kMaxCells || cells >= 0xFFF0) return false;
        pl.max_cells = cells > pl.max_cells ? cells : pl.max_cells;
        pl.bstride[l] = 1;
    }
    for (int l = 0; l < L; ++l) {
        if (pl.mode[l] == 1) continue;
        pl.blk0[l] = blk;
        blk += pl.nblk[l];
    }
    int n1 = 0, first_chunks = 0;
    for (int l = L - 1; l >= 0; --l)
        if (pl.mode[l] == 1) { if (!n1) first_chunks = pl.nchunk[l]; if (pl.nchunk[l] == first_chunks) ++n1; }
    int j = 0;
    for (int l = L - 1; l >= 0; --l) {
        if (pl.mode[l] == 1 && pl.nchunk[l] == first_chunks) { pl.blk0[l] = blk + j; pl.bstride[l] = n1; ++j; }
    }
    blk += n1 * first_chunks;
    for (int l = L - 1; l >= 0; --l) {
        if (pl.mode[l] != 1 || pl.nchunk[l] == first_chunks) continue;
        pl.blk0[l] = blk;
        blk += pl.nblk[l];
    }
    pl.nblocks = blk;
    pl.scr_per_bm = scr;
    return true;
}

int64_t plan_workspace_bytes(const FusedPlan &pl)
{
    if (pl.owner) return kHdrBytes;
    return kHdrBytes + (static_cast<int64_t>(pl.B) * pl.M * pl.scr_per_bm + static_cast<int64_t>(pl.B) * pl.S * pl.M * kCH) * 4;
}

}

int64_t msda_fused_workspace_bytes(const int64_t *shapes_h, const int64_t *start_h, int B, int S, int M, int D, int L, int Lq, int P)
{
    FusedPlan pl;
    if (D != kCH || !shapes_h || !start_h || !build_plan(pl, shapes_h, start_h, B, S, M, L, Lq, P)) return 0;
    return plan_workspace_bytes(pl);
}

hipError_t msda_backward_fused_launch(const int64_t *shapes_h, const int64_t *start_h, const void *value, const float *loc,
                                      const float *attn, const void *grad_out, float *grad_value, float *grad_loc, float *grad_attn,
                                      void *workspace, int64_t workspace_bytes, int B, int S, int M, int D, int L, int Lq, int P,
                                      int elem_dtype, hipStream_t st)
{
    FusedPlan pl;
    if (D != kCH || !shapes_h || !start_h || !build_plan(pl, shapes_h, start_h, B, S, M, L, Lq, P, elem_dtype)) return hipErrorNotSupported;
    if (!workspace || workspace_bytes < plan_workspace_bytes(pl)) return hipErrorNotSupported;
    if (elem_dtype != 0 && elem_dtype != 2) return hipErrorNotSupported;
    Header *hdr = static_cast<Header *>(workspace);
    const int64_t nfar = static_cast<int64_t>(B) * S * M * kCH;
    float *far = pl.owner ? grad_value : reinterpret_cast<float *>(static_cast<unsigned char *>(workspace) + kHdrBytes);
    float *scratch = pl.owner ? nullptr : far + nfar;
    hipError_t err;
    const int64_t n_go = static_cast<int64_t>(B) * Lq * M * D, n_at = static_cast<int64_t>(B) * Lq * M * L * P;
    if ((L * P) % 4 != 0) return hipErrorNotSupported;
    const int64_t pre_items = (n_go + n_at) / 4 + (pl.owner ? nfar / 4 : nfar / 4 / 64);
    const unsigned pre_blocks = static_cast<unsigned>(pre_items / (256 * 4) < kMaxPre ? (pre_items / (256 * 4) > 0 ? pre_items / (256 * 4) : 1) : kMaxPre);
    pl.npre = static_cast<int>(pre_blocks);
    profile_begin(7, Lq, st);
    if (elem_dtype == 2)
        hipLaunchKernelGGL(msda_absmax_kernel<__hip_bfloat16>, dim3(pre_blocks), dim3(256), 0, st, static_cast<const __hip_bfloat16 *>(grad_out), n_go, attn, n_at, hdr, far, nfar, pl.owner);
    else
        hipLaunchKernelGGL(msda_absmax_kernel<float>, dim3(pre_blocks), dim3(256), 0, st, static_cast<const float *>(grad_out), n_go, attn, n_at, hdr, far, nfar, pl.owner);
    profile_end(st);
    int threads = env_int("msda_threads", 1024);
    threads = (threads >= 1024 && elem_dtype == 2) ? 1024 : ((threads == 768 && elem_dtype == 2) ? 768 : 512);
    auto lds_bytes = [&](int thr) {
        return lds_win_bytes(pl.max_cells) + lds_cnt_bytes(pl.max_cells) + static_cast<size_t>(thr / 64) * 64 * kRecDw * 4 +
               static_cast<size_t>(pl.max_tab) * 4 + 128 + 16 + 128;
    };
    size_t lds = lds_bytes(threads);
    if (lds > 160 * 1024 && threads > 512) {
        threads = 512;
        lds = lds_bytes(threads);
    }
    if (lds > 160 * 1024) return hipErrorNotSupported;
    int dev = 0;
    if ((err = hipGetDevice(&dev)) != hipSuccess) return err;
    int lps = env_int("msda_lps", 4);
    lps = ((lps == 4 || lps == 2) && elem_dtype == 2 && threads > 512) ? lps : 8;
    if (lps == 2 && threads != 1024) lps = 4;
    const int groups = env_int("msda_groups", 2);
    static bool attr_set[10][64] = {};
    int which = elem_dtype != 2 ? 0 : (threads == 512 ? 1 : (threads == 768 ? (groups >= 4 ? 5 : 4) : (lps == 8 ? 2 : (lps == 2 ? 9 : 3))));
    typedef __hip_bfloat16 bf;
    const void *kern = which == 0 ? reinterpret_cast<const void *>(msda_bwd_fused<float, float, 512, 4, 8>)
                     : which == 1 ? reinterpret_cast<const void *>(msda_bwd_fused<bf, bf, 512, 4, 8>)
                     : which == 2 ? reinterpret_cast<const void *>(msda_bwd_fused<bf, bf, 1024, 4, 8>)
                     : which == 3 ? reinterpret_cast<const void *>(msda_bwd_fused<bf, bf, 1024, 2, 4>)
                     : which == 4 ? reinterpret_cast<const void *>(msda_bwd_fused<bf, bf, 768, 2, 4>)
                     : which == 9 ? reinterpret_cast<const void *>(msda_bwd_fused<bf, bf, 1024, 1, 2>)
                                  : reinterpret_cast<const void *>(msda_bwd_fused<bf, bf, 768, 4, 4>);
    const int slot_ = which;
    if (dev < 0 || dev >= 64 || !attr_set[slot_][dev]) {
        if ((err = hipFuncSetAttribute(kern, hipFuncAttributeMaxDynamicSharedMemorySize, 160 * 1024)) != hipSuccess) return err;
        if (dev >= 0 && dev < 64) attr_set[slot_][dev] = true;
    }
    const unsigned nblocks = static_cast<unsigned>(B) * M * pl.nblocks;
    profile_begin(6, Lq, st);
    auto go = [&](auto k, auto vt, auto gt) {
        using VT = decltype(vt); using GT = decltype(gt);
// ... 22 lines not shown
```

monodetr_amd/kernel_families.py:

```python
import os

AUTOTUNE_SWITCHES = ("MDETR_FUSED_LOSSES", "MDETR_FUSED_ADAMW", "MDETR_MSDA_PROLOGUE", "MDETR_FUSED_LN", "MDETR_MSDA_BF16",
                     "MDETR_FUSED_EPILOGUE", "MDETR_GEMM_RELU", "MDETR_CONV3X3", "MDETR_GROUP_NORM", "MDETR_SMALL_WGRAD",
                     "MDETR_CONV_STRIDED", "MDETR_CONV_WGRAD", "MDETR_CONV_STEM", "MDETR_TGEMM", "MDETR_WFOLD", "MDETR_RELU_PREMASK",
                     "MDETR_HEADS", "MDETR_CHUNK_SUMS", "MDETR_HEAD_TAIL", "MDETR_TGEMM_F32")
ALL_SWITCHES = AUTOTUNE_SWITCHES
SWITCH_TESTS = {
    "MDETR_FUSED_LOSSES": "test_fused_pair_losses_*, test_fused_ddn_loss_*, test_fused_cost_solver_*, test_training_step_with_fused_criterion_*",
    "MDETR_FUSED_ADAMW": "test_fused_adamw_kernel_*, test_fused_adamw_vs_recorded_reference_steps, test_training_step_with_fused_adamw_*",
    "MDETR_FUSED_LN": "test_fused_add_layernorm_*, test_training_step_with_fused_layernorm_*",
    "MDETR_MSDA_PROLOGUE": "test_msda_prologue_kernel_*",
    "MDETR_MSDA_BF16": "test_msda_bf16_kernels_*, test_msda_function_with_native_bf16_*, test_training_step_with_bf16_msda_*, test_msda_gpu.py::test_bf16_native_full_encoder_shape_vs_oracle",
    "MDETR_FUSED_EPILOGUE": "test_bias_act_kernel_*, test_training_step_with_fused_tails_*",
    "MDETR_GEMM_RELU": "test_library_gemm_relu_epilogue_*, test_training_step_with_fused_tails_*",
    "MDETR_SMALL_WGRAD": "test_small_wgrad_kernel_*, test_training_step_with_the_small_wgrad_kernel_*, test_exact_products_gpu.py::test_exact_small_wgrad",
    "MDETR_GROUP_NORM": "test_group_norm_kernel_*, test_training_step_with_the_group_norm_kernel_*",
    "MDETR_CONV_STRIDED": "test_conv_strided_kernel_matches_the_library_convolution, test_training_step_with_the_convolution_kernels_*, test_exact_products_gpu.py::test_exact_conv_strided_*",
    "MDETR_CONV_WGRAD": "test_conv_wgrad_kernel_matches_the_library_weight_gradient, test_conv_strided_kernel_*, test_training_step_with_the_convolution_kernels_*, test_exact_products_gpu.py::test_exact_conv_wgrad_*, test_exact_products_gpu.py::test_exact_token_weight_gradient",
    "MDETR_CONV_STEM": "test_conv_stem_kernel_matches_the_library_convolution, test_training_step_with_the_convolution_kernels_*, test_exact_products_gpu.py::test_exact_conv_stem",
    "MDETR_TGEMM": "test_tgemm_gpu.py::test_tgemm_*, test_training_step_with_the_token_gemm_kernel_*, test_bottleneck_with_fused_tails_*, test_exact_products_gpu.py::test_exact_tgemm_bf16_*, test_exact_products_gpu.py::test_exact_decimate_and_pointwise_conv",
    "MDETR_WFOLD": "test_fold_kernel_*, test_training_step_with_the_fold_kernel_*",
    "MDETR_TGEMM_F32": "test_tgemm_f32_gpu.py::test_tgemm_f32_*, test_tgemm_f32_gpu.py::test_fp32_modules_with_the_switch_*, test_exact_products_gpu.py::test_exact_tgemm_f32_*",
    "MDETR_RELU_PREMASK": "test_tgemm_gpu.py::test_masked_input_gradient_*, test_tgemm_gpu.py::test_bottleneck_stage_with_premasked_relu_*, test_exact_products_gpu.py::test_exact_tgemm_masked_*",
    "MDETR_HEADS": "test_sgemm_gpu.py::test_sgemm_*, test_sgemm_gpu.py::test_heads_level_*, test_training_step_with_the_grouped_heads_*, test_exact_products_gpu.py::test_exact_sgemm_grouped_*",
    "MDETR_HEAD_TAIL": "test_sgemm_gpu.py::test_head_tail_*, test_sgemm_gpu.py::test_training_step_with_the_head_tail_*",
    "MDETR_CHUNK_SUMS": "test_colsum_gpu.py::test_chunk_sums_*, test_colsum_gpu.py::test_deferred_chunk_sums_*",
    "MDETR_CONV3X3": "test_conv3x3_kernel_matches_the_library_convolution, test_training_step_with_the_conv3x3_kernel_*, test_conv3x3_module_with_a_trainable_bias_*, test_exact_products_gpu.py::test_exact_conv3x3_*",
}
COMMITTED_SWITCHES = {
    "bf16": ("MDETR_FUSED_LOSSES", "MDETR_FUSED_ADAMW", "MDETR_FUSED_LN", "MDETR_MSDA_PROLOGUE", "MDETR_MSDA_BF16",
             "MDETR_FUSED_EPILOGUE", "MDETR_GEMM_RELU", "MDETR_CONV3X3", "MDETR_GROUP_NORM", "MDETR_SMALL_WGRAD",
             "MDETR_CONV_WGRAD", "MDETR_CONV_STRIDED", "MDETR_CONV_STEM", "MDETR_TGEMM", "MDETR_WFOLD", "MDETR_RELU_PREMASK", "MDETR_HEADS",
             "MDETR_CHUNK_SUMS", "MDETR_HEAD_TAIL"),
    "fp32": ("MDETR_FUSED_LOSSES", "MDETR_FUSED_ADAMW", "MDETR_FUSED_LN", "MDETR_MSDA_PROLOGUE",
             "MDETR_FUSED_EPILOGUE", "MDETR_GEMM_RELU", "MDETR_GROUP_NORM", "MDETR_SMALL_WGRAD", "MDETR_HEADS",
             "MDETR_HEAD_TAIL"),
}
COMMITTED_SWITCHES["bf16-autocast"] = COMMITTED_SWITCHES["fp32"]


def committed_switches(precision):
    env = env_switches()
    if env or os.environ.get("MDETR_BENCH_DEFAULT_PATH") == "1":
        return env, "environment"
    return set(COMMITTED_SWITCHES[precision]), "bench.COMMITTED_SWITCHES"


def env_switches():
    return {k for k in ALL_SWITCHES if os.environ.get(k) == "1"}


def apply_switches(names):
    from monodetr_amd import chunk_sums, head_tail_ext
    chunk_sums.ENABLED = "MDETR_CHUNK_SUMS" in names
    head_tail_ext.ENABLED = "MDETR_HEAD_TAIL" in names
    from monodetr_amd import add_ln_ext, bias_act_ext, conv3x3_ext, conv_stem_ext, conv_taps_ext, conv_wgrad_ext, group_norm_ext, small_wgrad_ext, wfold_ext
    from monodetr_amd.monodetr import heads, linear
    from monodetr_amd.monodetr.ops.functions import ms_deform_attn_func
    from monodetr_amd.monodetr.ops.modules import ms_deform_attn
    ms_deform_attn._FUSED_PROLOGUE = "MDETR_MSDA_PROLOGUE" in names
    add_ln_ext.ENABLED = "MDETR_FUSED_LN" in names
    linear._TGEMM = "MDETR_TGEMM" in names
    linear._TGEMM_F32 = "MDETR_TGEMM_F32" in names
    heads.ENABLED = "MDETR_HEADS" in names
    wfold_ext.ENABLED = "MDETR_WFOLD" in names
    linear._PREMASK = "MDETR_RELU_PREMASK" in names
    linear._GEMM_RELU = "MDETR_GEMM_RELU" in names
    bias_act_ext.ENABLED = "MDETR_FUSED_EPILOGUE" in names
    conv3x3_ext.ENABLED = "MDETR_CONV3X3" in names
    conv_taps_ext.ENABLED = "MDETR_CONV_STRIDED" in names
    conv_wgrad_ext.ENABLED = "MDETR_CONV_WGRAD" in names
    conv_stem_ext.ENABLED = "MDETR_CONV_STEM" in names
    group_norm_ext.ENABLED = "MDETR_GROUP_NORM" in names
    small_wgrad_ext.ENABLED = "MDETR_SMALL_WGRAD" in names
    ms_deform_attn_func._NATIVE_BF16 = "MDETR_MSDA_BF16" in names


def enable_for_training(model, criterion, optimizer_cfg, precision="fp32", choice="committed"):
    names, _ = (set(), "default") if choice == "default" else committed_switches("bf16" if precision == "bf16" else "fp32")
# ... 4 lines not shown
```

monodetr_amd/monodetr/linear.py:

```python
import os

import torch
import torch.nn.functional as F
from torch import nn

from .. import colsum_ext, small_wgrad_ext

_MIN_TOKENS = 4096
_GEMM_RELU = os.environ.get("MDETR_GEMM_RELU") == "1"
_TGEMM = os.environ.get("MDETR_TGEMM") == "1"
_TGEMM_F32 = os.environ.get("MDETR_TGEMM_F32") == "1"


_TWGRAD_MIN_ROWS = 1024


_PREMASK = os.environ.get("MDETR_RELU_PREMASK") == "1"


class ReluToken:
    __slots__ = ("premasked",)

    def __init__(self):
        self.premasked = False


def relu_token_of(t):
    return getattr(t, "_mdetr_relu_token", None) if _PREMASK else None


def _kernel_dtype(dtype):
    return (_TGEMM and dtype == torch.bfloat16) or (_TGEMM_F32 and dtype == torch.float32)


_F32_NN_MIN_TOKENS = 8192


def _tgemm_ok(x2, weight, bias=None, res2=None, nn=False):
    if not _kernel_dtype(x2.dtype):
        return False
    if nn and x2.dtype == torch.float32 and x2.shape[0] < _F32_NN_MIN_TOKENS:
        return False
    from .. import tgemm_ext
    return tgemm_ext.supported(x2, weight, nn=nn, res=res2, bias=bias)


def _drop_seed(x, p):
    if p <= 0.0:
        return 0, None
    if x.is_cuda and torch.cuda.is_current_stream_capturing():
        from ..attn_ext import site_seed
        return site_seed(x.device)
    from ..add_ln_ext import _host_seed
    return _host_seed(), None


def _act_backward(dy, y, scale=1.0):
    if scale == 1.0:
        return torch.ops.aten.threshold_backward(dy, y, 0.0)
    from .. import bias_act_ext
    if bias_act_ext.supported(y):
        return bias_act_ext.act_backward(dy, y, scale)
    return torch.where(y > 0, dy * scale, torch.zeros_like(dy))


def _split_count(T):
    best = 0
    for c in (64, 48, 80, 96, 60, 50, 40, 32, 128, 30, 24, 20, 16):
        if T % c == 0 and T // c >= 256:
            best = c
# ... 37 lines not shown
            db = colsum_ext.column_sum(dy2, dt)
        else:
            db = (dy2.view(C, T // C, -1).sum(1).sum(0) if C else dy2.sum(0)).to(dt)
    return dw, db


def _fwd_product(x2, weight, bias, relu=False, res2=None, dropout_p=0.0, seed=0, seed_dev=None, out_dtype=None):
    from .. import tgemm_ext
    return tgemm_ext.tgemm(x2, weight, bias, res2, relu=relu, out_dtype=out_dtype, dropout_p=dropout_p, seed=seed, seed_dev=seed_dev)


def _input_gradient(dy2, weight, dskip2=None, mask2=None):
    if dy2.is_contiguous() and _tgemm_ok(dy2, weight, res2=dskip2, nn=True):
        from .. import tgemm_ext
        if mask2 is not None and tgemm_ext.masked_supported(dy2, weight, mask2, dskip2):
            return tgemm_ext.tgemm_masked(dy2, weight, mask2, dskip2)
        dx = tgemm_ext.tgemm(dy2, weight, None, dskip2, nn=True)
    elif dskip2 is None:
        dx = dy2 @ weight
    elif dskip2.dtype == dy2.dtype:
        dx = torch.addmm(dskip2, dy2, weight)
    else:
        dx = dskip2 + dy2 @ weight
    return dx if mask2 is None else torch.ops.aten.threshold_backward(dx, mask2, 0.0)


class _TokenLinearSkip(torch.autograd.Function):

    @staticmethod
    def forward(ctx, x, weight, bias, pos, relu=False, dropout_p=0.0, premask=False, wide_out=False, out_token=None):
        ctx.premask = bool(premask) and pos is None
        ctx.out_token = out_token
        ctx.wide_out = bool(wide_out)
        q = x if pos is None else x + pos
        q2 = q.reshape(-1, q.shape[-1])
        ctx.has_bias = bias is not None
        ctx.bias_dtype = bias.dtype if bias is not None else None
        ctx.relu = bool(relu)
        ctx.scale = 1.0 / (1.0 - dropout_p) if dropout_p > 0.0 else 1.0
        if _tgemm_ok(q2, weight, bias):
            seed, seed_dev = _drop_seed(q, dropout_p)
            y = _fwd_product(q2, weight, bias, relu, None, dropout_p, seed, seed_dev,
                             torch.float32 if wide_out else q2.dtype).view(q.shape[:-1] + (weight.shape[0],))
        elif dropout_p > 0.0 or wide_out:
            raise RuntimeError("token_linear_skip: dropout and the fp32 result exist in csrc/tgemm.hip's epilogue only")
        elif relu:
            y = torch._addmm_activation(bias, q2, weight.t()).view(q.shape[:-1] + (weight.shape[0],))
        else:
            y = F.linear(q, weight, bias)
        if relu:
            ctx.save_for_backward(q, weight, y)
        else:
            ctx.save_for_backward(q, weight)
        return y, x.view_as(x)

    @staticmethod
    @torch.autograd.function.once_differentiable
    def backward(ctx, dy, dskip):
        q, weight = ctx.saved_tensors[:2]
        if ctx.relu and not (ctx.out_token is not None and ctx.out_token.premasked and ctx.scale == 1.0):
            dy = _act_backward(dy.contiguous(), ctx.saved_tensors[2], ctx.scale)
        if ctx.wide_out:
            dy = dy.to(q.dtype)
        q2, dy2 = q.reshape(-1, q.shape[-1]), dy.reshape(-1, dy.shape[-1])
        dx = None
        if ctx.needs_input_grad[0]:
            ds2 = dskip.reshape(-1, q.shape[-1]) if dskip is not None else None
            dx = _input_gradient(dy2, weight, ds2, q2 if ctx.premask else None).view_as(q)
        dw, db = _weight_bias_grads(q2, dy2, weight, ctx.needs_input_grad[1], ctx.has_bias and ctx.needs_input_grad[2], ctx.bias_dtype)
        return dx, dw, db, None, None, None, None, None, None


def token_linear_skip(x, weight, bias=None, pos=None, relu=False, dropout_p=0.0, relu_token=None, wide_out=False, out_token=None):
    if (x.is_cuda or _tgemm_backend()) and x.dtype == weight.dtype and x.numel() // x.shape[-1] >= _MIN_TOKENS and torch.is_grad_enabled() and x.requires_grad \
            and not torch.is_autocast_enabled() and (pos is None or not pos.requires_grad) \
            and (not relu or skip_relu_fusable(bias, x, weight)) and (dropout_p <= 0.0 or skip_dropout_fusable(x, weight, bias)) \
            and (not wide_out or (not relu and x.is_cuda and x.dtype == torch.bfloat16 and _tgemm_ok(x.reshape(-1, x.shape[-1]), weight, bias))):
        premask = relu_token is not None and pos is None and _kernel_dtype(x.dtype) and _tgemm_ok(x.reshape(-1, x.shape[-1]), weight, bias) \
            and (x.dtype != torch.float32 or x.numel() // x.shape[-1] >= _F32_NN_MIN_TOKENS)
        if premask:
            relu_token.premasked = True
        return _TokenLinearSkip.apply(x, weight, bias, pos, relu, dropout_p, premask, wide_out, out_token if relu else None)
    if dropout_p > 0.0:
        raise RuntimeError("token_linear_skip: ask skip_dropout_fusable before passing dropout_p")
    return token_linear(x if pos is None else x + pos, weight, bias, relu=relu, wide_out=wide_out), x


def skip_relu_fusable(bias, x=None, weight=None):
    if x is not None and weight is not None and _tgemm_ok(x.reshape(-1, x.shape[-1]), weight, bias):
        return True
    return _GEMM_RELU and bias is not None and bias.dim() == 1 and bias.is_contiguous()


def skip_dropout_fusable(x, weight, bias):
    return (x.is_cuda or _tgemm_backend()) and x.dtype == weight.dtype and x.numel() // x.shape[-1] >= _MIN_TOKENS \
        and not torch.is_autocast_enabled() and _tgemm_ok(x.reshape(-1, x.shape[-1]), weight, bias)


class _TokenLinear(torch.autograd.Function):
    @staticmethod
    def forward(ctx, x, weight, bias, fused_relu=False, wide_out=False, dropout_p=0.0):
        ctx.has_bias = bias is not None
        ctx.bias_dtype = bias.dtype if bias is not None else None
        ctx.fused_relu = False
        ctx.wide_out = bool(wide_out)
        ctx.scale = 1.0 / (1.0 - dropout_p) if dropout_p > 0.0 else 1.0
        x2 = x.reshape(-1, x.shape[-1])
        if _tgemm_ok(x2, weight, bias):
            seed, seed_dev = _drop_seed(x, dropout_p)
            y = _fwd_product(x2, weight, bias, fused_relu, None, dropout_p, seed, seed_dev, torch.float32 if wide_out else x2.dtype)
            y = y.view(x.shape[:-1] + (weight.shape[0],))
            ctx.fused_relu = bool(fused_relu)
            if fused_relu:
                ctx.save_for_backward(x, weight, y)
            else:
                ctx.save_for_backward(x, weight)
            return y
        if dropout_p > 0.0:
            raise RuntimeError("token_linear: dropout is only fused into csrc/tgemm.hip's epilogue")
        if wide_out:
            y = torch.mm(x2, weight.t(), out_dtype=torch.float32)
            if bias is not None:
                y += bias.float()
            ctx.save_for_backward(x, weight)
            return y.view(x.shape[:-1] + (weight.shape[0],))
        if fused_relu:
            y = torch._addmm_activation(bias, x2, weight.t()).view(x.shape[:-1] + (weight.shape[0],))
            ctx.fused_relu = True
            ctx.save_for_backward(x, weight, y)
            return y
        ctx.save_for_backward(x, weight)
        return F.linear(x, weight, bias)

    @staticmethod
    @torch.autograd.function.once_differentiable
    def backward(ctx, dy):
        if ctx.fused_relu:
            x, weight, y = ctx.saved_tensors
            dy = _act_backward(dy.contiguous(), y, ctx.scale)
        else:
            x, weight = ctx.saved_tensors
        if ctx.wide_out:
            dy = dy.to(x.dtype)
        dx = dw = db = None
        x2 = x.reshape(-1, x.shape[-1])
        dy2 = dy.reshape(-1, dy.shape[-1])
        if ctx.needs_input_grad[0]:
            dx = _input_gradient(dy2, weight).view_as(x)
        dw, db = _weight_bias_grads(x2, dy2, weight, ctx.needs_input_grad[1], ctx.has_bias and ctx.needs_input_grad[2], ctx.bias_dtype)
        return dx, dw, db, None, None, None


class _TokenLinearResidualRelu(torch.autograd.Function):

    @staticmethod
    def forward(ctx, x2, weight, bias, res2, out_token=None, in_premask=False):
        out = _fwd_product(x2, weight, bias, True, res2)
        ctx.has_bias = bias is not None
        ctx.bias_dtype = bias.dtype if bias is not None else None
        ctx.out_token = out_token
        ctx.in_premask = bool(in_premask)
        ctx.save_for_backward(x2, weight, out)
        return out

    @staticmethod
    @torch.autograd.function.once_differentiable
    def backward(ctx, dout):
        x2, weight, out = ctx.saved_tensors
        if ctx.out_token is not None and ctx.out_token.premasked:
            g = dout.contiguous()
        else:
            g = torch.ops.aten.threshold_backward(dout.contiguous(), out, 0.0)
        dx = _input_gradient(g, weight, None, x2 if ctx.in_premask else None) if ctx.needs_input_grad[0] else None
        dw, db = _weight_bias_grads(x2, g, weight, ctx.needs_input_grad[1], ctx.has_bias and ctx.needs_input_grad[2], ctx.bias_dtype)
        return dx, dw, db, (g if ctx.needs_input_grad[3] else None), None, None


class _SplitRows(torch.autograd.Function):

    @staticmethod
    def forward(ctx, packed, *sizes):
        ctx.sizes = sizes
        ctx.meta = (packed.shape[1:], packed.dtype, packed.device)
        return tuple(p.view_as(p) for p in packed.split(list(sizes), 0))

    @staticmethod
    @torch.autograd.function.once_differentiable
    def backward(ctx, *grads):
        tail, dtype, device = ctx.meta
        from .. import chunk_sums
        chunk_sums.flush()
        parts = [g if g is not None else torch.zeros((n,) + tuple(tail), dtype=dtype, device=device) for g, n in zip(grads, ctx.sizes)]
        return (torch.cat(parts, 0),) + (None,) * len(ctx.sizes)


def split_rows(packed, *sizes):
# ... 145 lines not shown
```

monodetr_amd/monodetr/ops/functions/ms_deform_attn_func.py:

```python
import os

import torch
import torch.nn.functional as F
from torch.autograd import Function
from torch.autograd.function import once_differentiable

from .... import msda_ext as MSDA


_LOW = (torch.bfloat16, torch.float16)
_NATIVE_BF16 = os.environ.get("MDETR_MSDA_BF16") == "1"


class MSDeformAttnFunction(Function):
    @staticmethod
    def forward(ctx, value, value_spatial_shapes, value_level_start_index, sampling_locations,
                attention_weights, im2col_step):
        ctx.im2col_step = im2col_step
        ctx.in_dtypes = (value.dtype, sampling_locations.dtype, attention_weights.dtype)
        ctx.native_bf16 = _NATIVE_BF16 and value.dtype == torch.bfloat16 and MSDA.bf16_supported(value, sampling_locations)
        if ctx.native_bf16:
            value, sampling_locations, attention_weights = value.contiguous(), sampling_locations.float(), attention_weights.float()
            out = MSDA.ms_deform_attn_forward_bf16(value, value_spatial_shapes, value_level_start_index,
                                                   sampling_locations, attention_weights)
            ctx.save_for_backward(value, value_spatial_shapes, value_level_start_index,
                                  sampling_locations, attention_weights)
            return out
        if value.dtype in _LOW or sampling_locations.dtype in _LOW or attention_weights.dtype in _LOW:
            value, sampling_locations, attention_weights = value.float(), sampling_locations.float(), attention_weights.float()
        elif not (value.dtype == sampling_locations.dtype == attention_weights.dtype):
            wide = torch.promote_types(torch.promote_types(value.dtype, sampling_locations.dtype), attention_weights.dtype)
            value, sampling_locations, attention_weights = value.to(wide), sampling_locations.to(wide), attention_weights.to(wide)
        out = MSDA.ms_deform_attn_forward(value, value_spatial_shapes, value_level_start_index,
                                          sampling_locations, attention_weights, im2col_step)
        ctx.save_for_backward(value, value_spatial_shapes, value_level_start_index,
                              sampling_locations, attention_weights)
        return out.to(ctx.in_dtypes[0]) if ctx.in_dtypes[0] in _LOW else out

    @staticmethod
    @once_differentiable
    def backward(ctx, grad_output):
        value, shapes, level_start, loc, attn = ctx.saved_tensors
        dv, dl, da = ctx.in_dtypes
        if ctx.native_bf16:
            g_value, g_loc, g_attn = MSDA.ms_deform_attn_backward_bf16(
                value, shapes, level_start, loc, attn, grad_output.to(torch.bfloat16).contiguous())
            return g_value.to(dv), None, None, g_loc.to(dl), g_attn.to(da), None
        g_value, g_loc, g_attn = MSDA.ms_deform_attn_backward(
            value, shapes, level_start, loc, attn, grad_output.to(value.dtype).contiguous(), ctx.im2col_step)
        return g_value.to(dv), None, None, g_loc.to(dl), g_attn.to(da), None


def ms_deform_attn_core_pytorch(value, value_spatial_shapes, sampling_locations, attention_weights):
    N, S, M, D = value.shape
    Lq, L, P = sampling_locations.shape[1], sampling_locations.shape[3], sampling_locations.shape[4]
    sizes = [(int(h), int(w)) for h, w in value_spatial_shapes]
    levels = value.split([h * w for h, w in sizes], dim=1)
    grid = 2 * sampling_locations - 1
    sampled = []
    for lvl, (h, w) in enumerate(sizes):
        image = levels[lvl].flatten(2).transpose(1, 2).reshape(N * M, D, h, w)
        where = grid[:, :, :, lvl].transpose(1, 2).flatten(0, 1)
        sampled.append(F.grid_sample(image, where, mode='bilinear', padding_mode='zeros', align_corners=False))
    weights = attention_weights.transpose(1, 2).reshape(N * M, 1, Lq, L * P)
    out = (torch.stack(sampled, dim=-2).flatten(-2) * weights).sum(-1).view(N, M * D, Lq)
    return out.transpose(1, 2).contiguous()
```

monodetr_amd/monodetr/ops/modules/ms_deform_attn.py:

```python
import math
import os
import warnings

import torch
import torch.nn.functional as F
from torch import nn

from ..functions import MSDeformAttnFunction
from ... import _cut
from ...linear import Linear, token_linear, token_linear_skip
from .... import msda_prologue_ext


_FUSED_PROLOGUE = os.environ.get("MDETR_MSDA_PROLOGUE") == "1"
_PACKED_PROJECTION = True
_WIDE_CROSS_VALUE = True



def _check_token_count(spatial_shapes, S):
    seen = getattr(spatial_shapes, "_mdetr_token_count", None)
    if seen != (spatial_shapes._version, S):
        assert int((spatial_shapes[:, 0] * spatial_shapes[:, 1]).sum()) == S
        try:
# ... 7 lines not shown
        raise ValueError("invalid input for _is_power_of_2: {} (type: {})".format(n, type(n)))
    return n != 0 and (n & (n - 1)) == 0


def _star_offsets(n_heads, n_levels, n_points):
    theta = torch.arange(n_heads, dtype=torch.float32) * (2.0 * math.pi / n_heads)
    d = torch.stack([theta.cos(), theta.sin()], -1)
    d = d / d.abs().max(-1, keepdim=True)[0]
    scale = torch.arange(1, n_points + 1, dtype=torch.float32).view(1, 1, n_points, 1)
    return (d.view(n_heads, 1, 1, 2) * scale).expand(n_heads, n_levels, n_points, 2).reshape(-1)


class MSDeformAttn(nn.Module):
    def __init__(self, d_model=256, n_levels=4, n_heads=8, n_points=4, conditional=False):
        super().__init__()
        if d_model % n_heads != 0:
            raise ValueError("d_model must be divisible by n_heads, but got {} and {}".format(d_model, n_heads))
        if not _is_power_of_2(d_model // n_heads):
            warnings.warn("MSDeformAttn: head dimension %d is not a power of 2; the gfx950 fast path "
                          "needs 32 channels per head, other sizes take the generic kernel." % (d_model // n_heads))
        self.im2col_step = 64
        self.d_model, self.n_levels, self.n_heads, self.n_points = d_model, n_levels, n_heads, n_points
        self.conditional = conditional
        d_value = d_model // 2 if conditional else d_model
        self.sampling_offsets = Linear(d_model, n_heads * n_levels * n_points * 2)
        self.attention_weights = Linear(d_model, n_heads * n_levels * n_points)
        self.value_proj = Linear(d_value, d_value)
        self.output_proj = Linear(d_value, d_value)
        self._reset_parameters()

    def _reset_parameters(self):
        with torch.no_grad():
            self.sampling_offsets.weight.zero_()
            self.sampling_offsets.bias = nn.Parameter(_star_offsets(self.n_heads, self.n_levels, self.n_points))
            self.attention_weights.weight.zero_()
            self.attention_weights.bias.zero_()
            nn.init.xavier_uniform_(self.value_proj.weight)
            self.value_proj.bias.zero_()
            nn.init.xavier_uniform_(self.output_proj.weight)
            self.output_proj.bias.zero_()

    def forward(self, query, reference_points, input_flatten, input_spatial_shapes,
                input_level_start_index, input_padding_mask=None, chain_input=False):
        N, Lq, _ = query.shape
        S = input_flatten.shape[1]
        M, L, P = self.n_heads, self.n_levels, self.n_points
        _check_token_count(input_spatial_shapes, S)

        wide = _WIDE_CROSS_VALUE and input_flatten.is_cuda and input_flatten.dtype == torch.bfloat16 and Lq * 8 <= S
        if chain_input:
            value, input_next = token_linear_skip(input_flatten, self.value_proj.weight, self.value_proj.bias, wide_out=wide)
        else:
            value, input_next = token_linear(input_flatten, self.value_proj.weight, self.value_proj.bias, wide_out=wide), input_flatten
        if input_padding_mask is not None:
            value = value.masked_fill(input_padding_mask[..., None], 0.0)
        value = value.view(N, S, M, -1)

        if reference_points.shape[-1] not in (2, 6):
            raise ValueError("Last dim of reference_points must be 2 or 4, but get {} instead.".format(
                reference_points.shape[-1]))
        packed = offsets = logits = None
        if _FUSED_PROLOGUE and _PACKED_PROJECTION and not torch.is_autocast_enabled():
            packed = token_linear(query, *self._packed_projection())
        else:
            offsets = token_linear(query, self.sampling_offsets.weight, self.sampling_offsets.bias).view(N, Lq, M, L, P, 2)
            logits = token_linear(query, self.attention_weights.weight, self.attention_weights.bias).view(N, Lq, M, L * P)
        out = self._attend(value, packed, offsets, logits, reference_points, input_spatial_shapes, input_level_start_index, query.dtype)
        return (out, input_next) if chain_input else out

    def _packed_projection(self):
        return (torch.cat((self.sampling_offsets.weight, self.attention_weights.weight), 0),
                torch.cat((self.sampling_offsets.bias, self.attention_weights.bias), 0))

    def _attend(self, value, packed, offsets, logits, reference_points, input_spatial_shapes, input_level_start_index, out_dtype):
        N, S = value.shape[:2]
        M, L, P = self.n_heads, self.n_levels, self.n_points
        Lq = (packed if packed is not None else offsets).shape[1]
        if packed is not None and not msda_prologue_ext.packed_supported(packed, reference_points, L, P):
            offsets, logits = packed[..., :M * L * P * 2].reshape(N, Lq, M, L, P, 2), packed[..., M * L * P * 2:].reshape(N, Lq, M, L * P)
            packed = None
        if packed is not None:
            locations, weights = msda_prologue_ext.msda_prologue_packed(packed, reference_points, input_spatial_shapes, M, L, P)
        elif _FUSED_PROLOGUE and msda_prologue_ext.supported(offsets, logits, reference_points):
            locations, weights = msda_prologue_ext.msda_prologue(offsets, logits, reference_points, input_spatial_shapes)
        else:
            weights = F.softmax(logits, -1).view(N, Lq, M, L, P)
            ref = reference_points[:, :, None, :, None, :]
            if reference_points.shape[-1] == 2:
                wh = input_spatial_shapes.flip(-1)
                locations = ref + offsets / wh[None, None, None, :, None, :]
            else:
                extent = ref[..., 2::2] + ref[..., 3::2]
                locations = ref[..., :2] + offsets / P * extent * 0.5

        out = MSDeformAttnFunction.apply(value, input_spatial_shapes, input_level_start_index,
                                         locations, weights, self.im2col_step)
        out = _cut.at("msda", out, when_armed=True)
        if out.dtype != out_dtype and out_dtype == torch.bfloat16:
            out = out.to(out_dtype)
        return token_linear(out, self.output_proj.weight, self.output_proj.bias)

    def forward_self(self, src, pos, reference_points, input_spatial_shapes, input_level_start_index, input_padding_mask=None):
        if not (_FUSED_PROLOGUE and _PACKED_PROJECTION and src.is_cuda and not torch.is_autocast_enabled()
                and reference_points.shape[-1] in (2, 6)):
            return self.forward(src if pos is None else src + pos, reference_points, src, input_spatial_shapes,
                                input_level_start_index, input_padding_mask), _cut.at("msda", src, when_armed=True)
        N, S, _ = src.shape
        _check_token_count(input_spatial_shapes, S)
        value, src1 = token_linear_skip(src, self.value_proj.weight, self.value_proj.bias)
        if input_padding_mask is not None:
            value = value.masked_fill(input_padding_mask[..., None], 0.0)
        packed, src2 = token_linear_skip(src1, *self._packed_projection(), pos=pos)
        out = self._attend(value.view(N, S, self.n_heads, -1), packed, None, None, reference_points, input_spatial_shapes,
                           input_level_start_index, src.dtype)
        return out, _cut.at("msda", src2, when_armed=True)


class MSDeformAttn_cross(MSDeformAttn):

    def __init__(self, d_model=256, n_levels=4, n_heads=8, n_points=4):
        super().__init__(d_model, n_levels, n_heads, n_points, conditional=True)


MultiheadAttention = nn.MultiheadAttention
```

monodetr_amd/msda_ext.py:

```python
import os

import torch

from . import _capi

_NAMES5 = ("value", "spatial_shapes", "level_start_index", "sampling_loc", "attn_weight")

_ALLOW_CPU = False


def allow_cpu(on=True):
    global _ALLOW_CPU
    _ALLOW_CPU = bool(on)


def _check_inputs(tensors, names):
    if not tensors[0].is_cuda:
        raise RuntimeError("Not implemented on the CPU")
    for t, n in zip(tensors, names):
        if not t.is_contiguous():
            raise RuntimeError("%s tensor has to be contiguous" % n)
        if not t.is_cuda:
            raise RuntimeError("%s must be a CUDA tensor" % n)
        if t.device != tensors[0].device:
            raise RuntimeError("%s is on %s but value is on %s" % (n, t.device, tensors[0].device))


def _dims(value, spatial_shapes, level_start_index, sampling_loc, attn_weight, im2col_step):
    if value.dim() != 4 or sampling_loc.dim() != 6 or attn_weight.dim() != 5:
        raise RuntimeError("expected value[B,S,M,D], sampling_loc[B,Lq,M,L,P,2], attn_weight[B,Lq,M,L,P]")
    B, S, M, D = value.shape
    L = spatial_shapes.shape[0]
    Lq, P = sampling_loc.shape[1], sampling_loc.shape[4]
    if tuple(sampling_loc.shape) != (B, Lq, M, L, P, 2) or tuple(attn_weight.shape) != (B, Lq, M, L, P):
        raise RuntimeError("sampling_loc / attn_weight shapes do not match value / spatial_shapes")
    if spatial_shapes.dtype != torch.int64 or level_start_index.dtype != torch.int64:
        raise RuntimeError("spatial_shapes and level_start_index must be int64 (ms_deform_attn_cuda.cu:67-68)")
    if tuple(spatial_shapes.shape) != (L, 2) or tuple(level_start_index.shape) != (L,):
        raise RuntimeError("spatial_shapes must be [L,2] and level_start_index [L]")
    if sampling_loc.dtype != value.dtype or attn_weight.dtype != value.dtype:
        raise RuntimeError("value, sampling_loc and attn_weight must share one dtype")
    step = min(B, int(im2col_step))
    if B > 0 and (step <= 0 or B % step != 0):
        raise RuntimeError("batch(%d) must divide im2col_step(%d)" % (B, step))
    return B, S, M, D, L, Lq, P


def _aligned(t):
    return t if t.data_ptr() % 16 == 0 else t.clone(memory_format=torch.contiguous_format)


def _stream(device):
    return torch.cuda.current_stream(device).cuda_stream




def _geometry_on_host(spatial_shapes, level_start_index):
    hit = getattr(spatial_shapes, "_mdetr_host", None)
    if hit is None or hit[0] != spatial_shapes._version or hit[1] is not level_start_index or hit[2] != level_start_index._version:
        host = (spatial_shapes.cpu().contiguous(), level_start_index.cpu().contiguous())
        hit = (spatial_shapes._version, level_start_index, level_start_index._version, host)
        try:
            spatial_shapes._mdetr_host = hit
        except AttributeError:
            pass
    return hit[3]


def _workspace(device, nbytes):
    from . import _workspace as W
    return W.get("msda", device, nbytes, zero=True)


def ms_deform_attn_forward(value, spatial_shapes, level_start_index, sampling_loc, attn_weight, im2col_step):
    args = (value, spatial_shapes, level_start_index, sampling_loc, attn_weight)
    if _ALLOW_CPU and not value.is_cuda:
        return _forward_cpu(*args, im2col_step)
    _check_inputs(args, _NAMES5)
    B, S, M, D, L, Lq, P = _dims(*args, im2col_step)
    code = _capi.dtype_code(value)
    value, sampling_loc, attn_weight = _aligned(value), _aligned(sampling_loc), _aligned(attn_weight)
    out = torch.empty((B, Lq, M * D), dtype=value.dtype, device=value.device)
    dev = value.device.index
    rc = _capi.lib().mdetr_msda_forward(
        code, value.data_ptr(), spatial_shapes.data_ptr(), level_start_index.data_ptr(),
        sampling_loc.data_ptr(), attn_weight.data_ptr(), out.data_ptr(),
        B, S, M, D, L, Lq, P, dev, _stream(value.device))
    _capi.check(rc, "mdetr_msda_forward")
    return out


def ms_deform_attn_backward(value, spatial_shapes, level_start_index, sampling_loc, attn_weight, grad_output, im2col_step):
    args = (value, spatial_shapes, level_start_index, sampling_loc, attn_weight)
    if _ALLOW_CPU and not value.is_cuda:
        return _backward_cpu(*args, grad_output, im2col_step)
    _check_inputs(args + (grad_output,), _NAMES5 + ("grad_output",))
    B, S, M, D, L, Lq, P = _dims(*args, im2col_step)
    if grad_output.dtype != value.dtype or grad_output.numel() != B * Lq * M * D:
        raise RuntimeError("grad_output must be [B,Lq,M*D] of value's dtype")
    code = _capi.dtype_code(value)
    value, sampling_loc, attn_weight, grad_output = (_aligned(t) for t in (value, sampling_loc, attn_weight, grad_output))
    grad_value = torch.empty_like(value)
    grad_loc = torch.empty_like(sampling_loc)
    grad_attn = torch.empty_like(attn_weight)
    dev = value.device.index
    lib = _capi.lib()
    ws_bytes = 0
    if code == _capi.MDETR_F32 and D == 32 and B * Lq > 0:
        sh_h, st_h = _geometry_on_host(spatial_shapes, level_start_index)
        ws_bytes = lib.mdetr_msda_backward_workspace_bytes(code, sh_h.data_ptr(), st_h.data_ptr(), B, S, M, D, L, Lq, P)
    if ws_bytes > 0:
        ws = _workspace(value.device, ws_bytes)
        rc = lib.mdetr_msda_backward_ex(
            code, value.data_ptr(), spatial_shapes.data_ptr(), level_start_index.data_ptr(),
            sampling_loc.data_ptr(), attn_weight.data_ptr(), grad_output.data_ptr(),
            grad_value.data_ptr(), grad_loc.data_ptr(), grad_attn.data_ptr(),
            B, S, M, D, L, Lq, P, sh_h.data_ptr(), st_h.data_ptr(), ws.data_ptr(), ws_bytes,
            dev, _stream(value.device))
        _capi.check(rc, "mdetr_msda_backward_ex")
    else:
        rc = lib.mdetr_msda_backward(
            code, value.data_ptr(), spatial_shapes.data_ptr(), level_start_index.data_ptr(),
            sampling_loc.data_ptr(), attn_weight.data_ptr(), grad_output.data_ptr(),
            grad_value.data_ptr(), grad_loc.data_ptr(), grad_attn.data_ptr(),
            B, S, M, D, L, Lq, P, dev, _stream(value.device))
        _capi.check(rc, "mdetr_msda_backward")
    return [grad_value, grad_loc, grad_attn]


def _host_args(tensors, names):
    for t, n in zip(tensors, names):
        if t.is_cuda:
            raise RuntimeError("%s must be a CPU tensor (value is)" % n)
        if not t.is_contiguous():
            raise RuntimeError("%s tensor has to be contiguous" % n)


def _forward_cpu(value, spatial_shapes, level_start_index, sampling_loc, attn_weight, im2col_step):
    args = (value, spatial_shapes, level_start_index, sampling_loc, attn_weight)
    _host_args(args, _NAMES5)
    B, S, M, D, L, Lq, P = _dims(*args, im2col_step)
    out = torch.empty((B, Lq, M * D), dtype=value.dtype)
    rc = _capi.lib().mdetr_msda_forward_cpu(_capi.dtype_code(value), value.data_ptr(), spatial_shapes.data_ptr(), level_start_index.data_ptr(),
                                            sampling_loc.data_ptr(), attn_weight.data_ptr(), out.data_ptr(), B, S, M, D, L, Lq, P)
    _capi.check(rc, "mdetr_msda_forward_cpu")
    return out


def _backward_cpu(value, spatial_shapes, level_start_index, sampling_loc, attn_weight, grad_output, im2col_step):
    args = (value, spatial_shapes, level_start_index, sampling_loc, attn_weight)
    _host_args(args + (grad_output,), _NAMES5 + ("grad_output",))
    B, S, M, D, L, Lq, P = _dims(*args, im2col_step)
    if grad_output.dtype != value.dtype or grad_output.numel() != B * Lq * M * D:
        raise RuntimeError("grad_output must be [B,Lq,M*D] of value's dtype")
    gv, gl, ga = torch.empty_like(value), torch.empty_like(sampling_loc), torch.empty_like(attn_weight)
    rc = _capi.lib().mdetr_msda_backward_cpu(_capi.dtype_code(value), value.data_ptr(), spatial_shapes.data_ptr(), level_start_index.data_ptr(),
                                             sampling_loc.data_ptr(), attn_weight.data_ptr(), grad_output.data_ptr(),
                                             gv.data_ptr(), gl.data_ptr(), ga.data_ptr(), B, S, M, D, L, Lq, P)
    _capi.check(rc, "mdetr_msda_backward_cpu")
    return [gv, gl, ga]


def _dims_mixed(value, spatial_shapes, level_start_index, sampling_loc, attn_weight):
    if value.dtype != torch.bfloat16 or sampling_loc.dtype != torch.float32 or attn_weight.dtype != torch.float32:
        raise RuntimeError("bf16 variant: value must be bfloat16, sampling_loc and attn_weight float32")
    if value.dim() != 4 or sampling_loc.dim() != 6 or attn_weight.dim() != 5:
        raise RuntimeError("expected value[B,S,M,D], sampling_loc[B,Lq,M,L,P,2], attn_weight[B,Lq,M,L,P]")
    B, S, M, D = value.shape
    L = spatial_shapes.shape[0]
    Lq, P = sampling_loc.shape[1], sampling_loc.shape[4]
    if tuple(sampling_loc.shape) != (B, Lq, M, L, P, 2) or tuple(attn_weight.shape) != (B, Lq, M, L, P):
        raise RuntimeError("sampling_loc / attn_weight shapes do not match value / spatial_shapes")
    if spatial_shapes.dtype != torch.int64 or level_start_index.dtype != torch.int64:
        raise RuntimeError("spatial_shapes and level_start_index must be int64 (ms_deform_attn_cuda.cu:67-68)")
    if tuple(spatial_shapes.shape) != (L, 2) or tuple(level_start_index.shape) != (L,):
        raise RuntimeError("spatial_shapes must be [L,2] and level_start_index [L]")
    return B, S, M, D, L, Lq, P


def bf16_supported(value, sampling_loc):
    return (value.is_cuda and value.dtype == torch.bfloat16 and value.dim() == 4 and value.shape[3] == 32
            and sampling_loc.dim() == 6 and sampling_loc.shape[3] == 4 and sampling_loc.shape[4] == 4)


def ms_deform_attn_forward_bf16(value, spatial_shapes, level_start_index, sampling_loc, attn_weight):
    args = (value, spatial_shapes, level_start_index, sampling_loc, attn_weight)
    _check_inputs(args, _NAMES5)
    B, S, M, D, L, Lq, P = _dims_mixed(*args)
    value, sampling_loc, attn_weight = _aligned(value), _aligned(sampling_loc), _aligned(attn_weight)
    out = torch.empty((B, Lq, M * D), dtype=torch.bfloat16, device=value.device)
    rc = _capi.lib().mdetr_msda_forward_bf16(
        value.data_ptr(), spatial_shapes.data_ptr(), level_start_index.data_ptr(),
        sampling_loc.data_ptr(), attn_weight.data_ptr(), out.data_ptr(),
        B, S, M, D, L, Lq, P, value.device.index, _stream(value.device))
    _capi.check(rc, "mdetr_msda_forward_bf16")
    return out


def ms_deform_attn_backward_bf16(value, spatial_shapes, level_start_index, sampling_loc, attn_weight, grad_output):
    args = (value, spatial_shapes, level_start_index, sampling_loc, attn_weight)
    _check_inputs(args + (grad_output,), _NAMES5 + ("grad_output",))
    B, S, M, D, L, Lq, P = _dims_mixed(*args)
    if grad_output.dtype != torch.bfloat16 or grad_output.numel() != B * Lq * M * D:
        raise RuntimeError("grad_output must be bfloat16 [B,Lq,M*D]")
    value, sampling_loc, attn_weight, grad_output = (_aligned(t) for t in (value, sampling_loc, attn_weight, grad_output))
    grad_value = torch.empty(value.shape, dtype=torch.float32, device=value.device)
    grad_loc = torch.empty_like(sampling_loc)
    grad_attn = torch.empty_like(attn_weight)
    lib = _capi.lib()
    ws_bytes, ws_ptr, sh_ptr, st_ptr = 0, 0, 0, 0
    if B * Lq > 0:
        sh_h, st_h = _geometry_on_host(spatial_shapes, level_start_index)
        ws_bytes = lib.mdetr_msda_backward_workspace_bytes(_capi.MDETR_F32, sh_h.data_ptr(), st_h.data_ptr(),
                                                           B, S, M, D, L, Lq, P)
        if ws_bytes > 0:
            ws_ptr, sh_ptr, st_ptr = _workspace(value.device, ws_bytes).data_ptr(), sh_h.data_ptr(), st_h.data_ptr()
    rc = lib.mdetr_msda_backward_bf16(
        value.data_ptr(), spatial_shapes.data_ptr(), level_start_index.data_ptr(),
        sampling_loc.data_ptr(), attn_weight.data_ptr(), grad_output.data_ptr(),
        grad_value.data_ptr(), grad_loc.data_ptr(), grad_attn.data_ptr(),
        B, S, M, D, L, Lq, P, sh_ptr, st_ptr, ws_ptr, ws_bytes, value.device.index, _stream(value.device))
    _capi.check(rc, "mdetr_msda_backward_bf16")
    return [grad_value, grad_loc, grad_attn]


def ms_deform_attn_indices(spatial_shapes, sampling_loc):
    if not sampling_loc.is_cuda:
        raise RuntimeError("Not implemented on the CPU")
    if not sampling_loc.is_contiguous() or not spatial_shapes.is_contiguous():
        raise RuntimeError("sampling_loc tensor has to be contiguous")
    B, Lq, M, L, P, _ = sampling_loc.shape
    idx = torch.empty((B, Lq, M, L, P, 4), dtype=torch.int32, device=sampling_loc.device)
    rc = _capi.lib().mdetr_msda_indices(
        _capi.dtype_code(sampling_loc), spatial_shapes.data_ptr(), _aligned(sampling_loc).data_ptr(),
        idx.data_ptr(), B, M, L, Lq, P, sampling_loc.device.index, _stream(sampling_loc.device))
    _capi.check(rc, "mdetr_msda_indices")
    return idx
```

Baseline: 489.7 images/sec.

## Emit bf16 value gradient directly from MSDA backward and defer LayerNorm column sums

Adds a one-pass MSDA backward entry point that writes grad_value straight to bf16 and hands it to the wide value token. This avoids a separate fp32 grad buffer and a later cast or copy. Chunk sums gain a pitched variant and a tall-reduction path, so add+LayerNorm backward can defer its gamma/beta column sums into the batched chunk-sum launch instead of running a separate column-sum kernel. The cost is more code paths and bf16 rounding of the value gradient, with a fallback when the kernel does not support the geometry.

```diff
diff --git a/include/monodetr_amd.h b/include/monodetr_amd.h
--- a/include/monodetr_amd.h
+++ b/include/monodetr_amd.h
@@ -7,7 +7,7 @@
 extern "C" {
 #endif
 
-#define MDETR_ABI_VERSION 13
+#define MDETR_ABI_VERSION 14
 
 #define MDETR_F32 0
 #define MDETR_F64 1
@@ -17,6 +17,7 @@
 #define MDETR_E_ARG        -1
 #define MDETR_E_HIP        -2
 #define MDETR_E_ALIGN      -3
+#define MDETR_E_UNSUPPORTED -4
 
 int mdetr_abi_version(void);
 const char *mdetr_last_error(void);
@@ -99,6 +100,11 @@
                              int B, int S, int M, int D, int L, int Lq, int P,
                              const int64_t *spatial_shapes_host, const int64_t *level_start_host,
                              void *workspace, int64_t workspace_bytes, int device, void *stream);
+int mdetr_msda_backward_to(int dtype, int grad_value_dtype, const void *value, const float *loc, const float *attn,
+                           const void *grad_out, void *grad_value, float *grad_loc, float *grad_attn,
+                           int B, int S, int M, int D, int L, int Lq, int P,
+                           const int64_t *spatial_shapes_host, const int64_t *level_start_host,
+                           void *workspace, int64_t workspace_bytes, int device, void *stream);
 
 int mdetr_msda_prologue_forward(int io_dtype, int ref_dtype, const void *offsets, const void *logits, const void *ref,
                                 const int64_t *spatial_shapes, float *sampling_loc, float *attn_weight,
@@ -238,6 +244,13 @@
     int32_t chunks, out_dtype;
 } mdetr_chunk_job;
 int mdetr_chunk_sums(const mdetr_chunk_job *jobs, int njobs, int device, void *stream);
+typedef struct {
+    const float *part;
+    void *out;
+    int64_t cols, pitch;
+    int32_t chunks, out_dtype;
+} mdetr_chunk_job_pitched;
+int mdetr_chunk_sums_pitched(const mdetr_chunk_job_pitched *jobs, int njobs, int device, void *stream);
 int mdetr_column_sum_to(int dtype, const void *x, void *out, int out_dtype, void *workspace, int64_t workspace_bytes,
                         int64_t rows, int cols, int64_t ld, int device, void *stream);
 
diff --git a/monodetr_amd/_capi.py b/monodetr_amd/_capi.py
--- a/monodetr_amd/_capi.py
+++ b/monodetr_amd/_capi.py
@@ -6,7 +6,8 @@
 LIB_PATH = os.environ.get("MDETR_LIB_PATH") or os.path.join(_HERE, "libmonodetr_amd.so")
 
 MDETR_F32, MDETR_F64, MDETR_BF16 = 0, 1, 2
-ABI_VERSION = 13
+MDETR_E_UNSUPPORTED = -4
+ABI_VERSION = 14
 
 _c_int, _c_vp = ctypes.c_int, ctypes.c_void_p
 
@@ -47,6 +48,7 @@
     "mdetr_head_tail_forward": (_c_int, [_c_vp] * 10 + [_c_int] * 6 + [_c_int, _c_vp]),
     "mdetr_head_tail_backward": (_c_int, [_c_vp] * 13 + [_c_int] * 6 + [_c_int, _c_vp]),
     "mdetr_chunk_sums": (_c_int, [_c_vp, _c_int, _c_int, _c_vp]),
+    "mdetr_chunk_sums_pitched": (_c_int, [_c_vp, _c_int, _c_int, _c_vp]),
     "mdetr_column_sum_to": (_c_int, [_c_int, _c_vp, _c_vp, _c_int, _c_vp, ctypes.c_int64, ctypes.c_int64, _c_int, ctypes.c_int64, _c_int, _c_vp]),
     "mdetr_add_layernorm_forward": (_c_int, [_c_int, _c_int] + [_c_vp] * 7 + [ctypes.c_int64, _c_int, ctypes.c_float, ctypes.c_float, ctypes.c_uint64, _c_vp, _c_int, _c_vp]),
     "mdetr_add_layernorm_partial_rows": (ctypes.c_int64, [ctypes.c_int64]),
@@ -75,6 +77,7 @@
     "mdetr_kitti_preprocess": (_c_int, [_c_vp, _c_vp, _c_int, _c_vp, _c_int, _c_int, _c_int, _c_int, _c_vp, _c_vp, _c_int, _c_vp]),
     "mdetr_msda_forward_bf16": (_c_int, [_c_vp] * 6 + [_c_int] * 7 + [_c_int, _c_vp]),
     "mdetr_msda_backward_bf16": (_c_int, [_c_vp] * 9 + [_c_int] * 7 + [_c_vp, _c_vp, _c_vp, ctypes.c_int64, _c_int, _c_vp]),
+    "mdetr_msda_backward_to": (_c_int, [_c_int, _c_int] + [_c_vp] * 7 + [_c_int] * 7 + [_c_vp, _c_vp, _c_vp, ctypes.c_int64, _c_int, _c_vp]),
     "mdetr_msda_prologue_forward": (_c_int, [_c_int, _c_int] + [_c_vp] * 6 + [_c_int] * 6 + [ctypes.c_int64] * 3 + [_c_int, _c_vp]),
     "mdetr_gather_flat": (_c_int, [_c_vp, _c_int] + [_c_vp] * 6 + [_c_int, _c_int, _c_vp]),
     "mdetr_fold_weights": (_c_int, [_c_int] + [_c_vp] * 7 + [_c_int, _c_vp]),
diff --git a/monodetr_amd/add_ln_ext.py b/monodetr_amd/add_ln_ext.py
--- a/monodetr_amd/add_ln_ext.py
+++ b/monodetr_amd/add_ln_ext.py
@@ -90,6 +90,11 @@
                                               ctx.seed_dev.data_ptr() if ctx.seed_dev is not None else None, dev, stream)
         if rc != 0:
             _capi.check(rc, "mdetr_add_layernorm_backward")
+        from . import chunk_sums
+        if (chunk_sums.deferring() and (s.is_cuda or chunk_sums._backend is not None) and g_dtype in (torch.float32, torch.bfloat16)
+                and b_dtype in (torch.float32, torch.bfloat16) and chunk_sums.supported(partial[:, :C], g_dtype)):
+            return (da.view(shape), db.view(shape), chunk_sums.chunk_sum(partial[:, :C], g_dtype).view(C),
+                    chunk_sums.chunk_sum(partial[:, C:], b_dtype).view(C), None, None, None, None)
         sums = _column_sum_f32(partial, g_dtype if g_dtype == b_dtype else torch.float32)
         return da.view(shape), db.view(shape), sums[:C].to(g_dtype), sums[C:].to(b_dtype), None, None, None, None
 
diff --git a/monodetr_amd/chunk_sums.py b/monodetr_amd/chunk_sums.py
--- a/monodetr_amd/chunk_sums.py
+++ b/monodetr_amd/chunk_sums.py
@@ -19,23 +19,37 @@
     _fields_ = [("part", ctypes.c_void_p), ("out", ctypes.c_void_p), ("cols", ctypes.c_int64), ("chunks", ctypes.c_int32), ("out_dtype", ctypes.c_int32)]
 
 
+class _PitchedJob(ctypes.Structure):
+    _fields_ = [("part", ctypes.c_void_p), ("out", ctypes.c_void_p), ("cols", ctypes.c_int64), ("pitch", ctypes.c_int64), ("chunks", ctypes.c_int32),
+                ("out_dtype", ctypes.c_int32)]
+
+
+def _pitch(part):
+    return part.stride(0) if part.shape[0] > 1 else part.shape[1]
+
+
 def _lib():
     return _backend if _backend is not None else _capi.lib()
 
 
 def supported(part, out_dtype):
-    return ((part.is_cuda or _backend is not None) and part.dim() == 2 and part.dtype == torch.float32 and part.is_contiguous()
-            and part.shape[1] % 4 == 0 and part.shape[0] > 0 and part.data_ptr() % 16 == 0 and out_dtype in (torch.float32, torch.bfloat16))
+    return ((part.is_cuda or _backend is not None) and part.dim() == 2 and part.dtype == torch.float32 and part.shape[0] > 0
+            and part.shape[1] > 0 and part.shape[1] % 4 == 0 and part.stride(1) == 1 and _pitch(part) % 4 == 0 and _pitch(part) >= part.shape[1]
+            and part.data_ptr() % 16 == 0 and out_dtype in (torch.float32, torch.bfloat16))
 
 
 def _launch(jobs):
-    arr = (_Job * len(jobs))()
+    pitched = any(_pitch(part) != part.shape[1] for part, _ in jobs)
+    arr = ((_PitchedJob if pitched else _Job) * len(jobs))()
     for q, (part, out) in zip(arr, jobs):
         q.part, q.out, q.cols, q.chunks = part.data_ptr(), out.data_ptr(), part.shape[1], part.shape[0]
         q.out_dtype = _capi.MDETR_BF16 if out.dtype == torch.bfloat16 else _capi.MDETR_F32
+        if pitched:
+            q.pitch = _pitch(part)
     dev = jobs[0][0].device
-    rc = _lib().mdetr_chunk_sums(ctypes.cast(arr, ctypes.c_void_p), len(jobs), dev.index if dev.type == "cuda" else -1,
-                                 torch.cuda.current_stream(dev).cuda_stream if dev.type == "cuda" else None)
+    entry = _lib().mdetr_chunk_sums_pitched if pitched else _lib().mdetr_chunk_sums
+    rc = entry(ctypes.cast(arr, ctypes.c_void_p), len(jobs), dev.index if dev.type == "cuda" else -1,
+               torch.cuda.current_stream(dev).cuda_stream if dev.type == "cuda" else None)
     if rc != 0:
         msg = _lib().mdetr_last_error()
         raise RuntimeError("mdetr_chunk_sums failed (code %d): %s" % (rc, msg.decode() if msg else "?"))
@@ -43,7 +57,7 @@
 
 def chunk_sum(part, out_dtype=torch.float32, defer=True):
     if not supported(part, out_dtype):
-        raise RuntimeError("chunk_sum: needs contiguous fp32 partials [chunks, cols], cols a multiple of 4, 16-byte aligned")
+        raise RuntimeError("chunk_sum: needs fp32 partials [chunks, cols] (contiguous, or a column range of such), cols a multiple of 4, 16-byte aligned")
     out = torch.empty(part.shape[1], dtype=out_dtype, device=part.device)
     with _lock:
         if defer and ENABLED and _depth > 0 and not IMMEDIATE:
diff --git a/monodetr_amd/csrc/capi.hip b/monodetr_amd/csrc/capi.hip
--- a/monodetr_amd/csrc/capi.hip
+++ b/monodetr_amd/csrc/capi.hip
@@ -703,7 +703,7 @@
     return MDETR_OK;
 }
 
-int mdetr_chunk_sums(const mdetr_chunk_job *jobs, int njobs, int device, void *stream)
+int mdetr_chunk_sums_pitched(const mdetr_chunk_job_pitched *jobs, int njobs, int device, void *stream)
 {
     if (njobs == 0) return MDETR_OK;
     const char *why = mdetr::chunk_sums_check(jobs, njobs);
@@ -716,6 +716,18 @@
     const hipError_t e = mdetr::chunk_sums_launch(jobs, njobs, static_cast<hipStream_t>(stream));
     if (e != hipSuccess) return fail(MDETR_E_HIP, "mdetr_chunk_sums: launch failed: %s", hipGetErrorString(e));
     return MDETR_OK;
+}
+
+int mdetr_chunk_sums(const mdetr_chunk_job *jobs, int njobs, int device, void *stream)
+{
+    if (njobs == 0) return MDETR_OK;
+    if (!jobs || njobs < 0) return fail(MDETR_E_ARG, "mdetr_chunk_sums: no jobs (%d jobs)", njobs);
+    std::vector<mdetr_chunk_job_pitched> wide(static_cast<size_t>(njobs));
+    for (int i = 0; i < njobs; ++i) {
+        const mdetr_chunk_job &q = jobs[i];
+        wide[i] = mdetr_chunk_job_pitched{q.part, q.out, q.cols, q.cols, q.chunks, q.out_dtype};
+    }
+    return mdetr_chunk_sums_pitched(wide.data(), njobs, device, stream);
 }
 
 static int conv3x3_any(const char *who, const void *x, const void *w, const float *shift, const void *mask, void *y, int B, int H, int W, int C, int N,
@@ -1276,6 +1288,31 @@
     return MDETR_OK;
 }
 
+int mdetr_msda_backward_to(int dtype, int grad_value_dtype, const void *value, const float *loc, const float *attn,
+                           const void *grad_out, void *grad_value, float *grad_loc, float *grad_attn,
+                           int B, int S, int M, int D, int L, int Lq, int P,
+                           const int64_t *spatial_shapes_host, const int64_t *level_start_host,
+                           void *workspace, int64_t workspace_bytes, int device, void *stream)
+{
+    if (int rc = check_common("mdetr_msda_backward_to", MDETR_F32, B, S, M, D, L, Lq, P)) return rc;
+    if ((dtype != MDETR_F32 && dtype != MDETR_BF16) || (grad_value_dtype != MDETR_F32 && grad_value_dtype != MDETR_BF16))
+        return fail(MDETR_E_ARG, "mdetr_msda_backward_to: dtype / grad_value_dtype must be MDETR_F32 or MDETR_BF16 (%d, %d)", dtype, grad_value_dtype);
+    if (!value || !loc || !attn || !grad_out || !grad_value || !grad_loc || !grad_attn)
+        return fail(MDETR_E_ARG, "mdetr_msda_backward_to: null pointer");
+    if (!aligned16(value) || !aligned16(loc) || !aligned16(attn) || !aligned16(grad_out) || !aligned16(grad_value) ||
+        !aligned16(grad_loc) || !aligned16(grad_attn) || !aligned16(workspace))
+        return fail(MDETR_E_ALIGN, "mdetr_msda_backward_to: all tensors must be 16-byte aligned");
+    DeviceScope dev(device);
+    if (dev.err != hipSuccess) return fail(MDETR_E_HIP, "mdetr_msda_backward_to: set device %d: %s", device, hipGetErrorString(dev.err));
+    const hipError_t e = mdetr::msda_backward_to_launch(dtype, grad_value_dtype, value, loc, attn, grad_out, grad_value, grad_loc, grad_attn,
+                                                        B, S, M, D, L, Lq, P, spatial_shapes_host, level_start_host, workspace,
+                                                        workspace_bytes, static_cast<hipStream_t>(stream));
+    if (e == hipErrorNotSupported)
+        return fail(MDETR_E_UNSUPPORTED, "mdetr_msda_backward_to: the one-pass kernel does not take this geometry (B=%d S=%d M=%d D=%d L=%d Lq=%d P=%d)", B, S, M, D, L, Lq, P);
+    if (e != hipSuccess) return fail(MDETR_E_HIP, "mdetr_msda_backward_to: launch failed: %s", hipGetErrorString(e));
+    return MDETR_OK;
+}
+
 static int prologue_args(const char *who, int io_dtype, int B, int Lq, int M, int L, int P, int R)
 {
     if (io_dtype != MDETR_F32 && io_dtype != MDETR_BF16) return fail(MDETR_E_ARG, "%s: dtype must be f32 or bf16", who);
diff --git a/monodetr_amd/csrc/colsum.h b/monodetr_amd/csrc/colsum.h
--- a/monodetr_amd/csrc/colsum.h
+++ b/monodetr_amd/csrc/colsum.h
@@ -11,7 +11,7 @@
 hipError_t colsum_launch(int dtype, const void *x, void *out, void *workspace, int64_t rows, int cols, int64_t ld,
                          hipStream_t st, int out_dtype = 0);
 
-const char *chunk_sums_check(const mdetr_chunk_job *jobs, int njobs);
-hipError_t chunk_sums_launch(const mdetr_chunk_job *jobs, int njobs, hipStream_t st);
+const char *chunk_sums_check(const mdetr_chunk_job_pitched *jobs, int njobs);
+hipError_t chunk_sums_launch(const mdetr_chunk_job_pitched *jobs, int njobs, hipStream_t st);
 
 }
diff --git a/monodetr_amd/csrc/colsum.hip b/monodetr_amd/csrc/colsum.hip
--- a/monodetr_amd/csrc/colsum.hip
+++ b/monodetr_amd/csrc/colsum.hip
@@ -98,12 +98,13 @@
 }
 
 constexpr int kChunkJobs = 48, kChunkCols = 4 * kThreads;
+constexpr int kTallChunks = 128, kTallLanes = 32, kTallCols = 4 * (kThreads / kTallLanes);
 struct ChunkJob {
     const float *part;
     void *out;
-    int64_t cols;
+    int64_t cols, pitch;
     int chunks, out_bf16;
-    int block0, pad_;
+    int block0, tall;
 };
 struct ChunkArgs {
     ChunkJob j[kChunkJobs];
@@ -114,6 +115,7 @@
 void chunk_sums_kernel(const ChunkArgs a)
 {
     __shared__ __attribute__((aligned(16))) ChunkArgs la;
+    __shared__ __attribute__((aligned(16))) float red[kTallLanes][kTallCols];
     {
         const unsigned *src = reinterpret_cast<const unsigned *>(&a);
         unsigned *dst = reinterpret_cast<unsigned *>(&la);
@@ -124,22 +126,54 @@
     for (int i = 1; i < la.njobs; ++i)
         if (static_cast<int>(blockIdx.x) >= la.j[i].block0) ji = i;
     const ChunkJob &J = la.j[ji];
-    const int64_t cols = J.cols, c = static_cast<int64_t>(static_cast<int>(blockIdx.x) - J.block0) * kChunkCols + 4 * threadIdx.x;
+    const int64_t cols = J.cols, pitch = J.pitch;
+    const int chunks = J.chunks;
+    if (J.tall) {
+        const int tc = threadIdx.x % (kTallCols / 4), r = threadIdx.x / (kTallCols / 4);
+        const int64_t c0 = static_cast<int64_t>(static_cast<int>(blockIdx.x) - J.block0) * kTallCols, c = c0 + 4 * tc;
+        float4 s = make_float4(0.f, 0.f, 0.f, 0.f);
+        if (c < cols) {
+            const float *p = J.part + c;
+            int k = r;
+            for (; k + 3 * kTallLanes < chunks; k += 4 * kTallLanes) {
+                const float4 v0 = *reinterpret_cast<const float4 *>(p + static_cast<int64_t>(k) * pitch);
+                const float4 v1 = *reinterpret_cast<const float4 *>(p + static_cast<int64_t>(k + kTallLanes) * pitch);
+                const float4 v2 = *reinterpret_cast<const float4 *>(p + static_cast<int64_t>(k + 2 * kTallLanes) * pitch);
+                const float4 v3 = *reinterpret_cast<const float4 *>(p + static_cast<int64_t>(k + 3 * kTallLanes) * pitch);
+                s.x = (((s.x + v0.x) + v1.x) + v2.x) + v3.x; s.y = (((s.y + v0.y) + v1.y) + v2.y) + v3.y;
+                s.z = (((s.z + v0.z) + v1.z) + v2.z) + v3.z; s.w = (((s.w + v0.w) + v1.w) + v2.w) + v3.w;
+            }
+            for (; k < chunks; k += kTallLanes) {
+                const float4 v = *reinterpret_cast<const float4 *>(p + static_cast<int64_t>(k) * pitch);
+                s.x += v.x; s.y += v.y; s.z += v.z; s.w += v.w;
+            }
+        }
+        *reinterpret_cast<float4 *>(&red[r][4 * tc]) = s;
+        __syncthreads();
+        if (threadIdx.x < kTallCols && c0 + threadIdx.x < cols) {
+            float t = 0.f;
+#pragma unroll
+            for (int l = 0; l < kTallLanes; ++l) t += red[l][threadIdx.x];
+            if (J.out_bf16) static_cast<__hip_bfloat16 *>(J.out)[c0 + threadIdx.x] = __float2bfloat16(t);
+            else static_cast<float *>(J.out)[c0 + threadIdx.x] = t;
+        }
+        return;
+    }
+    const int64_t c = static_cast<int64_t>(static_cast<int>(blockIdx.x) - J.block0) * kChunkCols + 4 * threadIdx.x;
     if (c >= cols) return;
     const float *p = J.part + c;
-    const int chunks = J.chunks;
     float4 s = make_float4(0.f, 0.f, 0.f, 0.f);
     int k = 0;
     for (; k + 3 < chunks; k += 4) {
-        const float4 v0 = *reinterpret_cast<const float4 *>(p + static_cast<int64_t>(k) * cols);
-        const float4 v1 = *reinterpret_cast<const float4 *>(p + static_cast<int64_t>(k + 1) * cols);
-        const float4 v2 = *reinterpret_cast<const float4 *>(p + static_cast<int64_t>(k + 2) * cols);
-        const float4 v3 = *reinterpret_cast<const float4 *>(p + static_cast<int64_t>(k + 3) * cols);
+        const float4 v0 = *reinterpret_cast<const float4 *>(p + static_cast<int64_t>(k) * pitch);
+        const float4 v1 = *reinterpret_cast<const float4 *>(p + static_cast<int64_t>(k + 1) * pitch);
+        const float4 v2 = *reinterpret_cast<const float4 *>(p + static_cast<int64_t>(k + 2) * pitch);
+        const float4 v3 = *reinterpret_cast<const float4 *>(p + static_cast<int64_t>(k + 3) * pitch);
         s.x = (((s.x + v0.x) + v1.x) + v2.x) + v3.x; s.y = (((s.y + v0.y) + v1.y) + v2.y) + v3.y;
         s.z = (((s.z + v0.z) + v1.z) + v2.z) + v3.z; s.w = (((s.w + v0.w) + v1.w) + v2.w) + v3.w;
     }
     for (; k < chunks; ++k) {
-        const float4 v = *reinterpret_cast<const float4 *>(p + static_cast<int64_t>(k) * cols);
+        const float4 v = *reinterpret_cast<const float4 *>(p + static_cast<int64_t>(k) * pitch);
         s.x += v.x; s.y += v.y; s.z += v.z; s.w += v.w;
     }
     if (J.out_bf16) {
@@ -150,33 +184,41 @@
     }
 }
 
-}
-
-const char *chunk_sums_check(const mdetr_chunk_job *jobs, int njobs)
+inline int64_t chunk_job_blocks(const mdetr_chunk_job_pitched &q)
+{
+    const int64_t per = q.chunks > kTallChunks ? kTallCols : kChunkCols;
+    return (q.cols + per - 1) / per;
+}
+
+}
+
+const char *chunk_sums_check(const mdetr_chunk_job_pitched *jobs, int njobs)
 {
     if (!jobs || njobs <= 0) return "no jobs";
     for (int i = 0; i < njobs; ++i) {
-        const mdetr_chunk_job &q = jobs[i];
+        const mdetr_chunk_job_pitched &q = jobs[i];
         if (!q.part || !q.out || q.cols <= 0 || q.chunks <= 0) return "null pointer or empty job";
         if (q.cols % 4 != 0 || (reinterpret_cast<uintptr_t>(q.part) & 15) != 0) return "cols must be a multiple of 4 and the partials 16-byte aligned";
+        if (q.pitch < q.cols || q.pitch % 4 != 0) return "pitch must be a multiple of 4 and at least cols";
         if (q.out_dtype != 0 && q.out_dtype != 2) return "out_dtype must be MDETR_F32 or MDETR_BF16";
         if ((reinterpret_cast<uintptr_t>(q.out) & (q.out_dtype == 2 ? 7 : 15)) != 0) return "result not aligned (16 bytes fp32, 8 bytes bf16)";
-        if ((q.cols + kChunkCols - 1) / kChunkCols > (1 << 24)) return "job too wide";
+        if (chunk_job_blocks(q) > (1 << 24)) return "job too wide";
     }
     return nullptr;
 }
 
-hipError_t chunk_sums_launch(const mdetr_chunk_job *jobs, int njobs, hipStream_t st)
+hipError_t chunk_sums_launch(const mdetr_chunk_job_pitched *jobs, int njobs, hipStream_t st)
 {
     for (int first = 0; first < njobs; first += kChunkJobs) {
         ChunkArgs a;
         const int n = njobs - first < kChunkJobs ? njobs - first : kChunkJobs;
         int blocks = 0;
         for (int i = 0; i < n; ++i) {
-            const mdetr_chunk_job &q = jobs[first + i];
+            const mdetr_chunk_job_pitched &q = jobs[first + i];
             ChunkJob &J = a.j[i];
-            J.part = q.part; J.out = q.out; J.cols = q.cols; J.chunks = q.chunks; J.out_bf16 = q.out_dtype == 2; J.block0 = blocks; J.pad_ = 0;
-            blocks += static_cast<int>((q.cols + kChunkCols - 1) / kChunkCols);
+            J.part = q.part; J.out = q.out; J.cols = q.cols; J.pitch = q.pitch; J.chunks = q.chunks; J.out_bf16 = q.out_dtype == 2; J.block0 = blocks;
+            J.tall = q.chunks > kTallChunks;
+            blocks += static_cast<int>(chunk_job_blocks(q));
         }
         a.njobs = n; a.pad_ = 0;
         hipLaunchKernelGGL(chunk_sums_kernel, dim3(blocks), dim3(kThreads), 0, st, a);
diff --git a/monodetr_amd/csrc/msda.h b/monodetr_amd/csrc/msda.h
--- a/monodetr_amd/csrc/msda.h
+++ b/monodetr_amd/csrc/msda.h
@@ -76,9 +76,14 @@
 
 int64_t msda_fused_workspace_bytes(const int64_t *shapes_h, const int64_t *start_h, int B, int S, int M, int D, int L, int Lq, int P);
 hipError_t msda_backward_fused_launch(const int64_t *shapes_h, const int64_t *start_h, const void *value, const float *loc,
-                                      const float *attn, const void *grad_out, float *grad_value, float *grad_loc, float *grad_attn,
+                                      const float *attn, const void *grad_out, void *grad_value, float *grad_loc, float *grad_attn,
                                       void *workspace, int64_t workspace_bytes, int B, int S, int M, int D, int L, int Lq, int P,
-                                      int elem_dtype, hipStream_t st);
+                                      int elem_dtype, hipStream_t st, int gv_dtype = 0 );
+hipError_t msda_backward_to_launch(int elem_dtype, int gv_dtype, const void *value, const float *loc, const float *attn,
+                                   const void *grad_out, void *grad_value, float *grad_loc, float *grad_attn,
+                                   int B, int S, int M, int D, int L, int Lq, int P,
+                                   const int64_t *shapes_host, const int64_t *lstart_host,
+                                   void *workspace, int64_t workspace_bytes, hipStream_t st);
 
 void msda_forward_cpu(int dtype, const void *value, const int64_t *shapes, const int64_t *lstart, const void *loc,
                       const void *attn, void *out, int B, int S, int M, int D, int L, int Lq, int P);
diff --git a/monodetr_amd/csrc/msda.hip b/monodetr_amd/csrc/msda.hip
--- a/monodetr_amd/csrc/msda.hip
+++ b/monodetr_amd/csrc/msda.hip
@@ -825,6 +825,20 @@
     return hipGetLastError();
 }
 
+hipError_t msda_backward_to_launch(int elem_dtype, int gv_dtype, const void *value, const float *loc, const float *attn,
+                                   const void *grad_out, void *grad_value, float *grad_loc, float *grad_attn,
+                                   int B, int S, int M, int D, int L, int Lq, int P,
+                                   const int64_t *shapes_host, const int64_t *lstart_host,
+                                   void *workspace, int64_t workspace_bytes, hipStream_t st)
+{
+    const int bwd_env = [] { char tb[16]; const char *ev = tune_str("msda_bwd", tb, sizeof(tb)); return !ev || !*ev || ev[0] == 'f' ? 0 : (ev[0] == 't' ? 1 : 2); }();
+    if (bwd_env != 0 || (elem_dtype != 0 && elem_dtype != 2) || !msda_fast_path(0, D, L, P) || (elem_dtype == 2 && (L != 4 || P != 4)) ||
+        static_cast<int64_t>(B) * Lq * M == 0 || !shapes_host || !lstart_host || !workspace)
+        return hipErrorNotSupported;
+    return msda_backward_fused_launch(shapes_host, lstart_host, value, loc, attn, grad_out, grad_value, grad_loc, grad_attn,
+                                      workspace, workspace_bytes, B, S, M, D, L, Lq, P, elem_dtype, st, gv_dtype);
+}
+
 hipError_t msda_backward_launch(int dtype, const void *value, const int64_t *shapes, const int64_t *lstart,
                                 const void *loc, const void *attn, const void *grad_out,
                                 void *grad_value, void *grad_loc, void *grad_attn,
diff --git a/monodetr_amd/csrc/msda_fused.hip b/monodetr_amd/csrc/msda_fused.hip
--- a/monodetr_amd/csrc/msda_fused.hip
+++ b/monodetr_amd/csrc/msda_fused.hip
@@ -46,7 +46,17 @@
     int max_tab;
     int npre;
     int small;
+    int gv_bf16;
 };
+
+__device__ __forceinline__ unsigned bf16x2_rne(float a, float b)
+{
+    const __hip_bfloat16 x = __float2bfloat16(a), y = __float2bfloat16(b);
+    unsigned short ux, uy;
+    __builtin_memcpy(&ux, &x, 2);
+    __builtin_memcpy(&uy, &y, 2);
+    return static_cast<unsigned>(ux) | (static_cast<unsigned>(uy) << 16);
+}
 
 __host__ __device__ inline int ceil_div_ll(long long a, long long b)
 {
@@ -756,7 +766,7 @@
             const unsigned long long cbits = static_cast<unsigned long long>(__builtin_bit_cast(unsigned, magic)) * 0x100000001ull;
             const float inv = finite ? ldexpf(1.0f, -(22 - shift - e)) : 0.f;
             float *dst1 = scratch + (static_cast<int64_t>(b) * M + m) * pl.scr_per_bm + pl.scr0[l] + static_cast<int64_t>(w.slot) * w.ncell * kCH;
-            float *dst0 = grad_value + ((static_cast<int64_t>(b) * pl.S + pl.start[l]) * M + m) * kCH;
+            float *dst0 = grad_value + ((static_cast<int64_t>(b) * pl.S + pl.start[l]) * M + m) * (pl.gv_bf16 ? kCH / 2 : kCH);
             unsigned mc = 0u;
             for (int i = threadIdx.x; i < w.ncell * kCellU64; i += THREADS) {
                 const int cell = i / kCellU64, pr = i % kCellU64;
@@ -778,8 +788,10 @@
                 } else {
                     const int wxx = cell % w.tstride;
                     const int yy = w.cy0 + cell / w.tstride, xx = w.cx0 + wxx;
-                    if (yy < H && xx < W && wxx < pl.TW[l])
-                        *reinterpret_cast<float2 *>(dst0 + static_cast<int64_t>(yy * W + xx) * (M * kCH) + 2 * pr) = out;
+                    if (yy < H && xx < W && wxx < pl.TW[l]) {
+                        if (pl.gv_bf16) dst0[static_cast<int64_t>(yy * W + xx) * (M * kCH / 2) + pr] = __uint_as_float(bf16x2_rne(out.x, out.y));
+                        else *reinterpret_cast<float2 *>(dst0 + static_cast<int64_t>(yy * W + xx) * (M * kCH) + 2 * pr) = out;
+                    }
                 }
             }
             if (OWNER) break;
@@ -816,6 +828,9 @@
             for (int u = 0; u < kFlight; ++u)
                 if (t0 + u < nch) { acc.x += v[u].x; acc.y += v[u].y; acc.z += v[u].z; acc.w += v[u].w; }
         }
+    } else if (pl.gv_bf16) {
+        const uint2 h = *reinterpret_cast<const uint2 *>(reinterpret_cast<const unsigned short *>(grad_value) + row * kCH + c4);
+        acc = make_float4(__uint_as_float(h.x << 16), __uint_as_float(h.x & 0xFFFF0000u), __uint_as_float(h.y << 16), __uint_as_float(h.y & 0xFFFF0000u));
     } else {
         acc = *reinterpret_cast<const float4 *>(grad_value + row * kCH + c4);
     }
@@ -825,7 +840,10 @@
         acc.x += v.x; acc.y += v.y; acc.z += v.z; acc.w += v.w;
         *f = make_float4(0.f, 0.f, 0.f, 0.f);
     }
-    *reinterpret_cast<float4 *>(grad_value + row * kCH + c4) = acc;
+    if (pl.gv_bf16)
+        *reinterpret_cast<uint2 *>(reinterpret_cast<unsigned short *>(grad_value) + row * kCH + c4) = make_uint2(bf16x2_rne(acc.x, acc.y), bf16x2_rne(acc.z, acc.w));
+    else
+        *reinterpret_cast<float4 *>(grad_value + row * kCH + c4) = acc;
 }
 
 __global__ __launch_bounds__(256)
@@ -1003,14 +1021,17 @@
 }
 
 hipError_t msda_backward_fused_launch(const int64_t *shapes_h, const int64_t *start_h, const void *value, const float *loc,
-                                      const float *attn, const void *grad_out, float *grad_value, float *grad_loc, float *grad_attn,
+                                      const float *attn, const void *grad_out, void *grad_value_any, float *grad_loc, float *grad_attn,
                                       void *workspace, int64_t workspace_bytes, int B, int S, int M, int D, int L, int Lq, int P,
-                                      int elem_dtype, hipStream_t st)
+                                      int elem_dtype, hipStream_t st, int gv_dtype)
 {
     FusedPlan pl;
     if (D != kCH || !shapes_h || !start_h || !build_plan(pl, shapes_h, start_h, B, S, M, L, Lq, P, elem_dtype)) return hipErrorNotSupported;
     if (!workspace || workspace_bytes < plan_workspace_bytes(pl)) return hipErrorNotSupported;
     if (elem_dtype != 0 && elem_dtype != 2) return hipErrorNotSupported;
+    if (gv_dtype != 0 && gv_dtype != 2) return hipErrorNotSupported;
+    pl.gv_bf16 = gv_dtype == 2;
+    float *grad_value = static_cast<float *>(grad_value_any);
     Header *hdr = static_cast<Header *>(workspace);
     const int64_t nfar = static_cast<int64_t>(B) * S * M * kCH;
     float *far = pl.owner ? grad_value : reinterpret_cast<float *>(static_cast<unsigned char *>(workspace) + kHdrBytes);
diff --git a/monodetr_amd/kernel_families.py b/monodetr_amd/kernel_families.py
--- a/monodetr_amd/kernel_families.py
+++ b/monodetr_amd/kernel_families.py
@@ -8,7 +8,7 @@
 SWITCH_TESTS = {
     "MDETR_FUSED_LOSSES": "test_fused_pair_losses_*, test_fused_ddn_loss_*, test_fused_cost_solver_*, test_training_step_with_fused_criterion_*",
     "MDETR_FUSED_ADAMW": "test_fused_adamw_kernel_*, test_fused_adamw_vs_recorded_reference_steps, test_training_step_with_fused_adamw_*",
-    "MDETR_FUSED_LN": "test_fused_add_layernorm_*, test_training_step_with_fused_layernorm_*",
+    "MDETR_FUSED_LN": "test_fused_add_layernorm_*, test_training_step_with_fused_layernorm_*, test_chunk_sums_tall_gpu.py::test_fused_add_layernorm_*",
     "MDETR_MSDA_PROLOGUE": "test_msda_prologue_kernel_*",
     "MDETR_MSDA_BF16": "test_msda_bf16_kernels_*, test_msda_function_with_native_bf16_*, test_training_step_with_bf16_msda_*, test_msda_gpu.py::test_bf16_native_full_encoder_shape_vs_oracle",
     "MDETR_FUSED_EPILOGUE": "test_bias_act_kernel_*, test_training_step_with_fused_tails_*",
@@ -24,7 +24,7 @@
     "MDETR_RELU_PREMASK": "test_tgemm_gpu.py::test_masked_input_gradient_*, test_tgemm_gpu.py::test_bottleneck_stage_with_premasked_relu_*, test_exact_products_gpu.py::test_exact_tgemm_masked_*",
     "MDETR_HEADS": "test_sgemm_gpu.py::test_sgemm_*, test_sgemm_gpu.py::test_heads_level_*, test_training_step_with_the_grouped_heads_*, test_exact_products_gpu.py::test_exact_sgemm_grouped_*",
     "MDETR_HEAD_TAIL": "test_sgemm_gpu.py::test_head_tail_*, test_sgemm_gpu.py::test_training_step_with_the_head_tail_*",
-    "MDETR_CHUNK_SUMS": "test_colsum_gpu.py::test_chunk_sums_*, test_colsum_gpu.py::test_deferred_chunk_sums_*",
+    "MDETR_CHUNK_SUMS": "test_colsum_gpu.py::test_chunk_sums_*, test_colsum_gpu.py::test_deferred_chunk_sums_*, test_chunk_sums_tall_gpu.py::test_chunk_sums_*",
     "MDETR_CONV3X3": "test_conv3x3_kernel_matches_the_library_convolution, test_training_step_with_the_conv3x3_kernel_*, test_conv3x3_module_with_a_trainable_bias_*, test_exact_products_gpu.py::test_exact_conv3x3_*",
 }
 COMMITTED_SWITCHES = {
diff --git a/monodetr_amd/monodetr/linear.py b/monodetr_amd/monodetr/linear.py
--- a/monodetr_amd/monodetr/linear.py
+++ b/monodetr_amd/monodetr/linear.py
@@ -16,6 +16,20 @@
 
 
 _PREMASK = os.environ.get("MDETR_RELU_PREMASK") == "1"
+
+
+class WideGradToken:
+    __slots__ = ("grad",)
+
+    def __init__(self):
+        self.grad = None
+
+    def take(self, dy, shape, dtype):
+        g, self.grad = self.grad, None
+        if g is None:
+            return dy.to(dtype) if dy is not None else None
+        g = g.view(shape)
+        return g.to(dtype) if dy is None else (dy + g.float()).to(dtype)
 
 
 class ReluToken:
@@ -159,16 +173,22 @@
             ctx.save_for_backward(q, weight, y)
         else:
             ctx.save_for_backward(q, weight)
+        ctx.wide_token = None
+        if ctx.wide_out:
+            ctx.wide_token = y._mdetr_wide_token = WideGradToken()
+            ctx.set_materialize_grads(False)
         return y, x.view_as(x)
 
     @staticmethod
     @torch.autograd.function.once_differentiable
     def backward(ctx, dy, dskip):
         q, weight = ctx.saved_tensors[:2]
+        if ctx.wide_out:
+            dy = ctx.wide_token.take(dy, q.shape[:-1] + (weight.shape[0],), q.dtype)
+            if dy is None:
+                return (dskip if ctx.needs_input_grad[0] else None), None, None, None, None, None, None, None, None
         if ctx.relu and not (ctx.out_token is not None and ctx.out_token.premasked and ctx.scale == 1.0):
             dy = _act_backward(dy.contiguous(), ctx.saved_tensors[2], ctx.scale)
-        if ctx.wide_out:
-            dy = dy.to(q.dtype)
         q2, dy2 = q.reshape(-1, q.shape[-1]), dy.reshape(-1, dy.shape[-1])
         dx = None
         if ctx.needs_input_grad[0]:
@@ -211,6 +231,7 @@
         ctx.bias_dtype = bias.dtype if bias is not None else None
         ctx.fused_relu = False
         ctx.wide_out = bool(wide_out)
+        ctx.wide_token = None
         ctx.scale = 1.0 / (1.0 - dropout_p) if dropout_p > 0.0 else 1.0
         x2 = x.reshape(-1, x.shape[-1])
         if _tgemm_ok(x2, weight, bias):
@@ -222,6 +243,9 @@
                 ctx.save_for_backward(x, weight, y)
             else:
                 ctx.save_for_backward(x, weight)
+            if ctx.wide_out:
+                ctx.wide_token = y._mdetr_wide_token = WideGradToken()
+                ctx.set_materialize_grads(False)
             return y
         if dropout_p > 0.0:
             raise RuntimeError("token_linear: dropout is only fused into csrc/tgemm.hip's epilogue")
@@ -248,7 +272,9 @@
         else:
             x, weight = ctx.saved_tensors
         if ctx.wide_out:
-            dy = dy.to(x.dtype)
+            dy = ctx.wide_token.take(dy, x.shape[:-1] + (weight.shape[0],), x.dtype) if ctx.wide_token is not None else dy.to(x.dtype)
+            if dy is None:
+                return None, None, None, None, None, None
         dx = dw = db = None
         x2 = x.reshape(-1, x.shape[-1])
         dy2 = dy.reshape(-1, dy.shape[-1])
diff --git a/monodetr_amd/monodetr/ops/functions/ms_deform_attn_func.py b/monodetr_amd/monodetr/ops/functions/ms_deform_attn_func.py
--- a/monodetr_amd/monodetr/ops/functions/ms_deform_attn_func.py
+++ b/monodetr_amd/monodetr/ops/functions/ms_deform_attn_func.py
@@ -10,13 +10,19 @@
 
 _LOW = (torch.bfloat16, torch.float16)
 _NATIVE_BF16 = os.environ.get("MDETR_MSDA_BF16") == "1"
+_BF16_GRAD_VALUE = True
+
+
+def _takes_grad_value_dtype():
+    return bool(getattr(MSDA, "GRAD_VALUE_DTYPE", False))
 
 
 class MSDeformAttnFunction(Function):
     @staticmethod
     def forward(ctx, value, value_spatial_shapes, value_level_start_index, sampling_locations,
-                attention_weights, im2col_step):
+                attention_weights, im2col_step, value_token=None):
         ctx.im2col_step = im2col_step
+        ctx.value_token = value_token if (_BF16_GRAD_VALUE and _takes_grad_value_dtype() and value.dtype == torch.float32) else None
         ctx.in_dtypes = (value.dtype, sampling_locations.dtype, attention_weights.dtype)
         ctx.native_bf16 = _NATIVE_BF16 and value.dtype == torch.bfloat16 and MSDA.bf16_supported(value, sampling_locations)
         if ctx.native_bf16:
@@ -43,12 +49,18 @@
         value, shapes, level_start, loc, attn = ctx.saved_tensors
         dv, dl, da = ctx.in_dtypes
         if ctx.native_bf16:
+            kw = {"grad_value_dtype": dv} if _BF16_GRAD_VALUE and _takes_grad_value_dtype() else {}
             g_value, g_loc, g_attn = MSDA.ms_deform_attn_backward_bf16(
-                value, shapes, level_start, loc, attn, grad_output.to(torch.bfloat16).contiguous())
-            return g_value.to(dv), None, None, g_loc.to(dl), g_attn.to(da), None
+                value, shapes, level_start, loc, attn, grad_output.to(torch.bfloat16).contiguous(), **kw)
+            return g_value.to(dv), None, None, g_loc.to(dl), g_attn.to(da), None, None
+        if ctx.value_token is not None and not ctx.native_bf16 and value.dtype == torch.float32 and dv == torch.float32:
+            g_value, g_loc, g_attn = MSDA.ms_deform_attn_backward(
+                value, shapes, level_start, loc, attn, grad_output.to(value.dtype).contiguous(), ctx.im2col_step, grad_value_dtype=torch.bfloat16)
+            ctx.value_token.grad = g_value
+            return None, None, None, g_loc.to(dl), g_attn.to(da), None, None
         g_value, g_loc, g_attn = MSDA.ms_deform_attn_backward(
             value, shapes, level_start, loc, attn, grad_output.to(value.dtype).contiguous(), ctx.im2col_step)
-        return g_value.to(dv), None, None, g_loc.to(dl), g_attn.to(da), None
+        return g_value.to(dv), None, None, g_loc.to(dl), g_attn.to(da), None, None
 
 
 def ms_deform_attn_core_pytorch(value, value_spatial_shapes, sampling_locations, attention_weights):
diff --git a/monodetr_amd/monodetr/ops/modules/ms_deform_attn.py b/monodetr_amd/monodetr/ops/modules/ms_deform_attn.py
--- a/monodetr_amd/monodetr/ops/modules/ms_deform_attn.py
+++ b/monodetr_amd/monodetr/ops/modules/ms_deform_attn.py
@@ -83,6 +83,7 @@
             value, input_next = token_linear_skip(input_flatten, self.value_proj.weight, self.value_proj.bias, wide_out=wide)
         else:
             value, input_next = token_linear(input_flatten, self.value_proj.weight, self.value_proj.bias, wide_out=wide), input_flatten
+        value_token = getattr(value, "_mdetr_wide_token", None) if wide and input_padding_mask is None else None
         if input_padding_mask is not None:
             value = value.masked_fill(input_padding_mask[..., None], 0.0)
         value = value.view(N, S, M, -1)
@@ -96,14 +97,16 @@
         else:
             offsets = token_linear(query, self.sampling_offsets.weight, self.sampling_offsets.bias).view(N, Lq, M, L, P, 2)
             logits = token_linear(query, self.attention_weights.weight, self.attention_weights.bias).view(N, Lq, M, L * P)
-        out = self._attend(value, packed, offsets, logits, reference_points, input_spatial_shapes, input_level_start_index, query.dtype)
+        out = self._attend(value, packed, offsets, logits, reference_points, input_spatial_shapes, input_level_start_index, query.dtype,
+                           value_token)
         return (out, input_next) if chain_input else out
 
     def _packed_projection(self):
         return (torch.cat((self.sampling_offsets.weight, self.attention_weights.weight), 0),
                 torch.cat((self.sampling_offsets.bias, self.attention_weights.bias), 0))
 
-    def _attend(self, value, packed, offsets, logits, reference_points, input_spatial_shapes, input_level_start_index, out_dtype):
+    def _attend(self, value, packed, offsets, logits, reference_points, input_spatial_shapes, input_level_start_index, out_dtype,
+                value_token=None):
         N, S = value.shape[:2]
         M, L, P = self.n_heads, self.n_levels, self.n_points
         Lq = (packed if packed is not None else offsets).shape[1]
@@ -125,7 +128,7 @@
                 locations = ref[..., :2] + offsets / P * extent * 0.5
 
         out = MSDeformAttnFunction.apply(value, input_spatial_shapes, input_level_start_index,
-                                         locations, weights, self.im2col_step)
+                                         locations, weights, self.im2col_step, value_token)
         out = _cut.at("msda", out, when_armed=True)
         if out.dtype != out_dtype and out_dtype == torch.bfloat16:
             out = out.to(out_dtype)
diff --git a/monodetr_amd/msda_ext.py b/monodetr_amd/msda_ext.py
--- a/monodetr_amd/msda_ext.py
+++ b/monodetr_amd/msda_ext.py
@@ -7,6 +7,7 @@
 _NAMES5 = ("value", "spatial_shapes", "level_start_index", "sampling_loc", "attn_weight")
 
 _ALLOW_CPU = False
+GRAD_VALUE_DTYPE = True
 
 
 def allow_cpu(on=True):
@@ -73,6 +74,28 @@
     return W.get("msda", device, nbytes, zero=True)
 
 
+def _backward_to(code, value, spatial_shapes, level_start_index, sampling_loc, attn_weight, grad_output, dims, grad_value_dtype):
+    B, S, M, D, L, Lq, P = dims
+    if B * Lq == 0 or D != 32:
+        return None
+    lib = _capi.lib()
+    sh_h, st_h = _geometry_on_host(spatial_shapes, level_start_index)
+    ws_bytes = lib.mdetr_msda_backward_workspace_bytes(_capi.MDETR_F32, sh_h.data_ptr(), st_h.data_ptr(), B, S, M, D, L, Lq, P)
+    if ws_bytes <= 0:
+        return None
+    ws = _workspace(value.device, ws_bytes)
+    grad_value = torch.empty(value.shape, dtype=grad_value_dtype, device=value.device)
+    grad_loc, grad_attn = torch.empty_like(sampling_loc), torch.empty_like(attn_weight)
+    rc = lib.mdetr_msda_backward_to(code, _capi.MDETR_BF16 if grad_value_dtype == torch.bfloat16 else _capi.MDETR_F32, value.data_ptr(),
+                                    sampling_loc.data_ptr(), attn_weight.data_ptr(), grad_output.data_ptr(), grad_value.data_ptr(),
+                                    grad_loc.data_ptr(), grad_attn.data_ptr(), B, S, M, D, L, Lq, P, sh_h.data_ptr(), st_h.data_ptr(),
+                                    ws.data_ptr(), ws_bytes, value.device.index, _stream(value.device))
+    if rc == _capi.MDETR_E_UNSUPPORTED:
+        return None
+    _capi.check(rc, "mdetr_msda_backward_to")
+    return [grad_value, grad_loc, grad_attn]
+
+
 def ms_deform_attn_forward(value, spatial_shapes, level_start_index, sampling_loc, attn_weight, im2col_step):
     args = (value, spatial_shapes, level_start_index, sampling_loc, attn_weight)
     if _ALLOW_CPU and not value.is_cuda:
@@ -91,7 +114,7 @@
     return out
 
 
-def ms_deform_attn_backward(value, spatial_shapes, level_start_index, sampling_loc, attn_weight, grad_output, im2col_step):
+def ms_deform_attn_backward(value, spatial_shapes, level_start_index, sampling_loc, attn_weight, grad_output, im2col_step, grad_value_dtype=None):
     args = (value, spatial_shapes, level_start_index, sampling_loc, attn_weight)
     if _ALLOW_CPU and not value.is_cuda:
         return _backward_cpu(*args, grad_output, im2col_step)
@@ -101,6 +124,14 @@
         raise RuntimeError("grad_output must be [B,Lq,M*D] of value's dtype")
     code = _capi.dtype_code(value)
     value, sampling_loc, attn_weight, grad_output = (_aligned(t) for t in (value, sampling_loc, attn_weight, grad_output))
+    if grad_value_dtype is not None and grad_value_dtype != value.dtype:
+        if grad_value_dtype != torch.bfloat16 or code != _capi.MDETR_F32:
+            raise RuntimeError("grad_value_dtype: torch.bfloat16 beside float32 tensors only")
+        got = _backward_to(code, value, spatial_shapes, level_start_index, sampling_loc, attn_weight, grad_output, (B, S, M, D, L, Lq, P), grad_value_dtype)
+        if got is None:
+            got = ms_deform_attn_backward(value, spatial_shapes, level_start_index, sampling_loc, attn_weight, grad_output, im2col_step)
+            got[0] = got[0].to(grad_value_dtype)
+        return got
     grad_value = torch.empty_like(value)
     grad_loc = torch.empty_like(sampling_loc)
     grad_attn = torch.empty_like(attn_weight)
@@ -198,13 +229,21 @@
     return out
 
 
-def ms_deform_attn_backward_bf16(value, spatial_shapes, level_start_index, sampling_loc, attn_weight, grad_output):
+def ms_deform_attn_backward_bf16(value, spatial_shapes, level_start_index, sampling_loc, attn_weight, grad_output, grad_value_dtype=torch.float32):
     args = (value, spatial_shapes, level_start_index, sampling_loc, attn_weight)
     _check_inputs(args + (grad_output,), _NAMES5 + ("grad_output",))
     B, S, M, D, L, Lq, P = _dims_mixed(*args)
     if grad_output.dtype != torch.bfloat16 or grad_output.numel() != B * Lq * M * D:
         raise RuntimeError("grad_output must be bfloat16 [B,Lq,M*D]")
     value, sampling_loc, attn_weight, grad_output = (_aligned(t) for t in (value, sampling_loc, attn_weight, grad_output))
+    if grad_value_dtype != torch.float32:
+        if grad_value_dtype != torch.bfloat16:
+            raise RuntimeError("grad_value_dtype must be torch.float32 or torch.bfloat16")
+        got = _backward_to(_capi.MDETR_BF16, value, spatial_shapes, level_start_index, sampling_loc, attn_weight, grad_output, (B, S, M, D, L, Lq, P), grad_value_dtype)
+        if got is None:
+            got = ms_deform_attn_backward_bf16(value, spatial_shapes, level_start_index, sampling_loc, attn_weight, grad_output)
+            got[0] = got[0].to(grad_value_dtype)
+        return got
     grad_value = torch.empty(value.shape, dtype=torch.float32, device=value.device)
     grad_loc = torch.empty_like(sampling_loc)
     grad_attn = torch.empty_like(attn_weight)
```

New measurement: 498.7 images/sec, median of 6. 1.8% higher.
